# oceanusxiv/pathtracer-rs

Hardware: AMD Instinct MI355X
Metric: Mray/s, Cornell Box 1024x1024, 256 spp, depth 15 (Msample/s in config) (higher is better)
Workload: dtype f32

## Files before the change

include/ptrs.h:

```cpp
#ifndef PTRS_H
#define PTRS_H

#include <stdint.h>

#ifdef __cplusplus
extern "C" {
#endif

#define PTRS_ABI_VERSION 4

enum {
    PTRS_OK = 0,
    PTRS_ERR_INVALID = -1,
    PTRS_ERR_UNSUPPORTED = -2,
    PTRS_ERR_DEVICE = -3,
    PTRS_ERR_IO = -4
};

enum { PTRS_TEX_CONSTANT = 0, PTRS_TEX_CHECKER = 1, PTRS_TEX_IMAGE = 2 };
enum { PTRS_WRAP_REPEAT = 0, PTRS_WRAP_BLACK = 1, PTRS_WRAP_CLAMP = 2 };

typedef struct PtrsTexture {
    int32_t kind;
    int32_t channels;
// ... 104 lines not shown
    uint32_t flags;
    int32_t sampler;
    int32_t n_sampled_dimensions;
} PtrsRenderParams;
enum { PTRS_SAMPLER_SOBOL = 0, PTRS_SAMPLER_STRATIFIED = 1 };

enum {
    PTRS_FLAG_COUNTERS = 1u,
    PTRS_FLAG_TIMING = 2u,
    PTRS_FLAG_FILM_ZERO = 4u
};

typedef struct PtrsFilmPixel {
    float rgb[3];
    float weight;
} PtrsFilmPixel;

typedef struct PtrsStats {
    uint64_t samples;
    uint64_t rays_extension;
    uint64_t rays_shadow;
    uint64_t rays_mis;
    uint64_t nodes_visited;
    uint64_t tris_tested;
    uint64_t passes;
    uint64_t kernel_launches;
    uint64_t trace_launches;
    double ms_total;
    double ms_trace;
    double ms_shade;
    double ms_film;
    uint64_t bvh_nodes;
    uint64_t bvh_max_depth;
    uint64_t device_bytes;
    double ms_extend;
    double ms_connect;
    double ms_shade_kernels;
    double ms_aux;
    uint64_t extend_launches, connect_launches, shade_launches, aux_launches, film_launches;
    uint64_t error_flags;
    uint64_t node_steps_x64, node_visits, tri_steps_x64;
    uint64_t debug[12];
    uint64_t queue_segments;
    uint64_t grid_wgs[4];
    uint64_t resident_wgs_per_cu[4];
    uint64_t lanes;
    uint64_t grid_pct;
    double ms_enqueue;
    double ms_tail;
    uint64_t tail_launches;
    uint64_t tail_round;
    uint64_t stack_lds;
    uint64_t lds_form_v4;
} PtrsStats;

enum {
    PTRS_ERRFLAG_SOBOL_DIM = 1u,
    PTRS_ERRFLAG_NULL_SKIPS = 2u
};

typedef struct PtrsScene PtrsScene;

int ptrs_set_option(const char *name, int64_t value);
int ptrs_get_option(const char *name, int64_t *value);
int ptrs_scene_set_option(PtrsScene *scene, const char *name, int64_t value);

int ptrs_abi_version(void);
const char *ptrs_build_id(void);
int ptrs_abi_sizeof(int which);
const char *ptrs_last_error(void);

int ptrs_scene_create(const PtrsSceneDesc *desc, int32_t device, PtrsScene **out);
void ptrs_scene_destroy(PtrsScene *scene);
int ptrs_scene_info(PtrsScene *scene, uint64_t *n_nodes, uint64_t *max_depth, uint64_t *n_tris);

int ptrs_render(PtrsScene *scene, const PtrsCamera *camera, const PtrsRenderParams *params,
                PtrsFilmPixel *film_inout, PtrsStats *stats);

typedef void (*PtrsProgressFn)(void *user, uint32_t passes_done, uint32_t passes_total, int32_t row_begin, int32_t row_end);
int ptrs_render_progressive(PtrsScene *scene, const PtrsCamera *camera, const PtrsRenderParams *params,
                            PtrsFilmPixel *film_inout, PtrsProgressFn fn, void *user, PtrsStats *stats);

int ptrs_plan_bands(int32_t height, uint32_t n, const float *row_cost, int32_t *bounds_out );
int ptrs_render_row_cost(PtrsScene *scene, const PtrsCamera *camera, const PtrsRenderParams *params, float *row_cost_out, PtrsStats *stats);
int ptrs_render_multi(PtrsScene *const *scenes, uint32_t n, const PtrsCamera *camera,
                      const PtrsRenderParams *params, const int32_t *band_bounds,
                      PtrsFilmPixel *film_inout, PtrsStats *stats_per_scene);

int ptrs_render_device(PtrsScene *scene, const PtrsCamera *camera, const PtrsRenderParams *params,
                       void *film_inout_device, void *hip_stream, PtrsStats *stats);

int ptrs_render_samples(PtrsScene *scene, const PtrsCamera *camera, const PtrsRenderParams *params,
                        PtrsFilmPixel *film_inout, float *sample_rgb, PtrsStats *stats);

enum { PTRS_AOV_ALBEDO = 1u, PTRS_AOV_NORMAL = 2u, PTRS_AOV_DEPTH = 4u };
#define PTRS_AOV_PLANES 3
#define PTRS_AOV_SAMPLE_FLOATS 12
int ptrs_render_aov(PtrsScene *scene, const PtrsCamera *camera, const PtrsRenderParams *params, uint32_t planes,
                    PtrsFilmPixel *const planes_inout[PTRS_AOV_PLANES], float *sample_aov, PtrsStats *stats);
int ptrs_render_aov_device(PtrsScene *scene, const PtrsCamera *camera, const PtrsRenderParams *params, uint32_t planes,
                           void *const planes_inout_device[PTRS_AOV_PLANES], float *sample_aov_device, void *hip_stream, PtrsStats *stats);

#define PTRS_DENOISE_MAX_ITERATIONS 8
enum {
    PTRS_DENOISE_DEMODULATE = 1u,
    PTRS_DENOISE_TIMING = 2u
// ... 80 lines not shown
```

pathtracer-rs_amd/abi.py:

```python
import ctypes as C

import numpy as np

PTRS_OK = 0
TEX_CONSTANT, TEX_CHECKER, TEX_IMAGE = 0, 1, 2
WRAP_REPEAT, WRAP_BLACK, WRAP_CLAMP = 0, 1, 2
MAT_MATTE, MAT_METAL, MAT_MIRROR, MAT_GLASS, MAT_DISNEY, MAT_SUBSTRATE, MAT_NORMAL = range(7)
LIGHT_POINT, LIGHT_DIRECTIONAL, LIGHT_AREA, LIGHT_INFINITE = range(4)
FLAG_COUNTERS, FLAG_TIMING, FLAG_FILM_ZERO = 1, 2, 4
SAMPLER_SOBOL, SAMPLER_STRATIFIED = 0, 1
PtrsAovAlbedo, PtrsAovNormal, PtrsAovDepth = 1, 2, 4
PtrsAovPlanes, PtrsAovSampleFloats = 3, 12
PtrsAovNames = ("albedo", "normal", "depth")
(MATH_SIN, MATH_COS, MATH_SINCOS, MATH_TAN, MATH_LOG, MATH_LOG2, MATH_EXP, MATH_POW, MATH_ATAN2, MATH_ACOS, MATH_DIV, MATH_SQRT,
 MATH_ROUND, MATH_MINMAX, MATH_MINMAX_NZ, MATH_U2F, MATH_INT, MATH_NEXT, MATH_SOLVE, MATH_FRAME, MATH_SPAWN, MATH_SEARCH, MATH_NUM_OPS) = range(23)
PROBE_MATH_WIDTH = 16
PROBE_MATH_ARGTYPES = [C.c_int32, C.c_uint32, C.c_uint32, C.c_void_p, C.c_void_p]

f32p = C.POINTER(C.c_float)
u32p = C.POINTER(C.c_uint32)
i32p = C.POINTER(C.c_int32)


class PtrsTexture(C.Structure):
# ... 5 lines not shown
class PtrsMaterial(C.Structure):
    _fields_ = [("kind", C.c_int32), ("tex", C.c_int32 * 6), ("flags", C.c_int32), ("inner", C.c_int32)]


class PtrsMesh(C.Structure):
    _fields_ = [("n_verts", C.c_uint32), ("n_tris", C.c_uint32), ("pos", f32p), ("normal", f32p), ("tangent", f32p),
                ("uv", f32p), ("indices", u32p), ("material", C.c_int32), ("alpha_mask_tex", C.c_int32),
                ("reverse_orientation", C.c_int32), ("transform_swaps_handedness", C.c_int32)]


class PtrsLight(C.Structure):
    _fields_ = [("kind", C.c_int32), ("v", C.c_float * 3), ("c", C.c_float * 3), ("mesh", C.c_uint32), ("tri", C.c_uint32),
                ("ke_tex", C.c_int32), ("world_center", C.c_float * 3), ("world_radius", C.c_float), ("lmap_tex", C.c_int32),
                ("light_to_world", C.c_float * 16), ("world_to_light", C.c_float * 16), ("dist_nu", C.c_int32),
                ("dist_nv", C.c_int32), ("dist_func", f32p), ("dist_cdf", f32p), ("dist_func_int", f32p),
                ("marg_cdf", f32p), ("marg_func_int", C.c_float)]


class PtrsBvhNode(C.Structure):
    _fields_ = [("p_min", C.c_float * 3), ("p_max", C.c_float * 3), ("offset", C.c_uint32), ("num_prims", C.c_uint16),
                ("axis", C.c_uint8), ("pad", C.c_uint8)]


class PtrsSceneDesc(C.Structure):
    _fields_ = [("n_meshes", C.c_uint32), ("meshes", C.POINTER(PtrsMesh)), ("n_materials", C.c_uint32),
                ("materials", C.POINTER(PtrsMaterial)), ("n_textures", C.c_uint32), ("textures", C.POINTER(PtrsTexture)),
                ("n_lights", C.c_uint32), ("lights", C.POINTER(PtrsLight)), ("n_bvh_nodes", C.c_uint32),
                ("bvh_nodes", C.POINTER(PtrsBvhNode)), ("bvh_prims", u32p)]


class PtrsCamera(C.Structure):
    _fields_ = [("rot", C.c_float * 4), ("trans", C.c_float * 3), ("m00", C.c_float), ("m11", C.c_float), ("m22", C.c_float),
                ("m23", C.c_float), ("raster_to_screen", C.c_float * 16), ("dx_camera", C.c_float * 3), ("dy_camera", C.c_float * 3)]


class PtrsRenderParams(C.Structure):
    _fields_ = [("width", C.c_int32), ("height", C.c_int32), ("spp", C.c_int32), ("max_depth", C.c_int32),
                ("rr_threshold", C.c_float), ("rr_start_depth", C.c_int32), ("rr_enable", C.c_int32), ("row_begin", C.c_int32),
                ("row_end", C.c_int32), ("device", C.c_int32), ("paths_per_pass", C.c_uint32), ("flags", C.c_uint32), ("sampler", C.c_int32),
                ("n_sampled_dimensions", C.c_int32)]


class PtrsStats(C.Structure):
    _fields_ = [("samples", C.c_uint64), ("rays_extension", C.c_uint64), ("rays_shadow", C.c_uint64), ("rays_mis", C.c_uint64),
                ("nodes_visited", C.c_uint64), ("tris_tested", C.c_uint64), ("passes", C.c_uint64), ("kernel_launches", C.c_uint64),
                ("trace_launches", C.c_uint64), ("ms_total", C.c_double), ("ms_trace", C.c_double), ("ms_shade", C.c_double),
                ("ms_film", C.c_double), ("bvh_nodes", C.c_uint64), ("bvh_max_depth", C.c_uint64), ("device_bytes", C.c_uint64),
                ("ms_extend", C.c_double), ("ms_connect", C.c_double), ("ms_shade_kernels", C.c_double), ("ms_aux", C.c_double),
                ("extend_launches", C.c_uint64), ("connect_launches", C.c_uint64), ("shade_launches", C.c_uint64), ("aux_launches", C.c_uint64),
                ("film_launches", C.c_uint64), ("error_flags", C.c_uint64), ("node_steps_x64", C.c_uint64), ("node_visits", C.c_uint64),
                ("tri_steps_x64", C.c_uint64), ("debug", C.c_uint64 * 12), ("queue_segments", C.c_uint64), ("grid_wgs", C.c_uint64 * 4),
                ("resident_wgs_per_cu", C.c_uint64 * 4), ("lanes", C.c_uint64), ("grid_pct", C.c_uint64), ("ms_enqueue", C.c_double),
                ("ms_tail", C.c_double), ("tail_launches", C.c_uint64), ("tail_round", C.c_uint64),
                ("stack_lds", C.c_uint64), ("lds_form_v4", C.c_uint64)]

    def as_dict(self):
        return {n: getattr(self, n) for n, _ in self._fields_}

    @property
    def rays(self):
        return self.rays_extension + self.rays_shadow + self.rays_mis


class PtrsHit(C.Structure):
    _fields_ = [("prim", C.c_int32), ("t", C.c_float), ("b0", C.c_float), ("b1", C.c_float), ("b2", C.c_float)]


class PtrsDenoiseParams(C.Structure):
    _fields_ = [("iterations", C.c_int32), ("sigma_color", C.c_float), ("sigma_normal", C.c_float), ("sigma_depth", C.c_float), ("flags", C.c_uint32)]


PtrsDenoiseDemodulate, PtrsDenoiseTiming, PtrsDenoiseMaxIterations = 1, 2, 8


class PtrsTileError(C.Structure):
    _fields_ = [("error", C.c_float), ("valid", C.c_uint32)]


class PtrsFilmErrorSummary(C.Structure):
    _fields_ = [("max_tile_error", C.c_float), ("worst_tile", C.c_uint32), ("valid_pixels", C.c_uint64), ("tiles_x", C.c_uint32), ("tiles_y", C.c_uint32)]


PtrsErrorTile, PtrsConvergeMaxChecks = 16, 32


class PtrsConvergeCheck(C.Structure):
    _fields_ = [("spp", C.c_uint32), ("max_tile_error", C.c_float)]


class PtrsConvergeResult(C.Structure):
    _fields_ = [("spp_done", C.c_uint32), ("converged", C.c_uint32), ("n_checks", C.c_uint32), ("worst_tile", C.c_uint32), ("history", PtrsConvergeCheck * PtrsConvergeMaxChecks)]


HIT_DTYPE = np.dtype([("prim", "<i4"), ("t", "<f4"), ("b0", "<f4"), ("b1", "<f4"), ("b2", "<f4")])
FILM_DTYPE = np.dtype([("rgb", "<f4", 3), ("weight", "<f4")])
TILE_DTYPE = np.dtype([("error", "<f4"), ("valid", "<u4")])


def _f32(a):
    return np.ascontiguousarray(a, dtype=np.float32)


def _ptr(a, typ):
    return a.ctypes.data_as(typ) if a is not None else typ()


class SceneDescHolder:
# ... 82 lines not shown
```

pathtracer-rs_amd/csrc/pt_hip_queue.h:

```cpp
#pragma once

constexpr int BLOCK = 256, WAVES = BLOCK / 64;

__device__ inline uint32_t rfl(uint32_t v) { return (uint32_t)__builtin_amdgcn_readfirstlane((int)v); }
__device__ inline uint32_t lanes_below(unsigned long long m) { return __builtin_amdgcn_mbcnt_hi((uint32_t)(m >> 32), __builtin_amdgcn_mbcnt_lo((uint32_t)m, 0u)); }
__device__ inline uint32_t wave_push(uint32_t &count, bool pred) {
    const unsigned long long m = __ballot(pred);
    const uint32_t slot = count + lanes_below(m);
    count += (uint32_t)__popcll(m);
    return slot;
}
__device__ inline uint32_t wave_of_launch() { return blockIdx.x * WAVES + (threadIdx.x >> 6); }
enum : uint32_t { TK_SUB = 64, TK_SUB_STRIDE = 32, TK_LAUNCH_WORDS = TK_SUB * TK_SUB_STRIDE };
__device__ inline uint32_t seg_next(uint32_t *ticket, uint32_t G) {
    const uint32_t per = (G + TK_SUB - 1u) / TK_SUB;
    const uint32_t home = wave_of_launch() & (TK_SUB - 1u);
    for (;;) {
        uint32_t tmp; unsigned long long open;
        asm volatile("v_mbcnt_lo_u32_b32 %0, -1, 0\n\tv_mbcnt_hi_u32_b32 %0, -1, %0\n\tv_lshlrev_b32 %0, 7, %0\n\tglobal_load_dword %0, %0, %2 sc1\n\ts_waitcnt vmcnt(0)\n\tv_cmp_gt_u32 %1, %3, %0"
                     : "=&v"(tmp), "=s"(open) : "s"(ticket), "s"(per) : "memory");
        static_assert(TK_SUB_STRIDE * 4u == 128u, "the asm above shifts the lane id by 7");
        if (open == 0ull) return 0xffffffffu;
        const unsigned long long rot = home ? ((open >> home) | (open << (64u - home))) : open;
        const uint32_t c = (home + (uint32_t)__ffsll((long long)rot) - 1u) & (TK_SUB - 1u);
        uint32_t t = 0;
        if (__lane_id() == 0) t = atomicAdd(ticket + c * TK_SUB_STRIDE, 1u);
        t = rfl(t);
        const uint32_t s = c * per + t;
        if (t < per && s < G) return s;
    }
}
__device__ inline uint32_t *seg_count(const DQueues &Q, uint32_t row, int q, uint32_t G, uint32_t s) { return Q.counts + ((size_t)row * Q_STRIDE + (size_t)q) * G + s; }
enum { TK_EXTEND = 0, TK_CONNECT = 1, TK_SHADE0 = 2, TK_EPILOGUE = 9, TK_RESOLVE = 10, TK_PRESAMPLE = 11, TK_TAIL = 12 };
__device__ inline bool round_is_dead(const DQueues &Q, uint32_t it) { return it > 0u && rfl(Q.alive[it]) == 0u; }
```

pathtracer-rs_amd/csrc/pt_items.h:

```cpp
#pragma once
#include "pt_bvh.h"
#include "pt_light.h"
#include "pt_sobol.h"
#include "pt_stratified.h"

namespace pt {

struct CamRay { f3 o, d, rx_d, ry_d; };

PT_HD CamRay camera_ray(const DCamera &C, f2 pf, float diff_scale) {
    const float *m = C.r2s;
    f3 s = mk3(m[0] * pf.x + m[1] * pf.y + m[2] * 0.0f + m[3], m[4] * pf.x + m[5] * pf.y + m[6] * 0.0f + m[7], m[8] * pf.x + m[9] * pf.y + m[10] * 0.0f + m[11]);
    float inv_denom = C.m23 / (s.z + C.m22);
    f3 pc = mk3(s.x * inv_denom / C.m00, s.y * inv_denom / C.m11, -inv_denom);
    CamRay r;
    r.o = quat_rotate(C.rot, splat3(0.0f)) + ld3(C.trans);
    f3 wd = quat_rotate(C.rot, pc);
    r.d = normalize(wd);
    f3 rxd = normalize(quat_rotate(C.rot, pc + ld3(C.dxc)));
    f3 ryd = normalize(quat_rotate(C.rot, pc + ld3(C.dyc)));
    r.rx_d = r.d + (rxd - r.d) * diff_scale;
    r.ry_d = r.d + (ryd - r.d) * diff_scale;
    return r;
}
// ... 47 lines not shown
template <int FEAT>
PT_HD int extension_epilogue(const DParams &R, const DScene &sc, const DPaths &P, uint32_t par, uint32_t pid, uint32_t e, const HitRec &h) {
    const v4 rdv = pslot(P.ray_d[par], e);
    const uint32_t stz = f2u(rdv.w);
    const int32_t prim = h.prim;
    const int32_t bounces = st_bounces(stz);
    if (bounces == 0 || (stz & ST_SPECULAR)) {
        if (prim >= 0) {
            if (h.flags & TRI_IS_LIGHT) {
                const TriRegs T = load_tri_regs(sc.shade + prim);
                f3 d = xyz(rdv);
                Surface s = tri_surface(T, prim, h.b0, h.b1, h.b2, -d);
                f3 le = surface_le<FEAT>(sc, T, s, -d);
                v4 Lv = pslot(P.L, pid);
                f3 L = xyz(Lv) + xyz(pslot(P.beta[par], e)) * le;
                pslot(P.L, pid) = mkv4(L, Lv.w);
            }
        } else if ((FEAT & FEAT_INFINITE) && sc.n_inf > 0) {
            f3 d = xyz(rdv);
            v4 Lv = pslot(P.L, pid);
            f3 L = xyz(Lv), beta = xyz(pslot(P.beta[par], e));
            for (uint32_t i = 0; i < sc.n_inf; ++i) L = L + beta * light_le<FEAT>(sc, sc.lights[sc.inf_lights[i]], d);
            pslot(P.L, pid) = mkv4(L, Lv.w);
        }
    }
    if (prim < 0 || bounces >= R.max_depth) return -1;
    return (int)((h.flags >> TRI_BUCKET_SHIFT) & 7u);
}

PT_HD uint32_t hit_pack(int32_t prim, uint32_t flags) {
    return prim < 0 ? 0xffffffffu : ((uint32_t)prim | (((flags >> TRI_BUCKET_SHIFT) & 7u) << 27) | ((flags & TRI_IS_LIGHT) ? 1u << 30 : 0u));
}
PT_HD int32_t hit_prim(uint32_t x) { return x == 0xffffffffu ? -1 : (int32_t)(x & REF_FIRST_MASK); }
PT_HD uint32_t hit_flags(uint32_t x) { return x == 0xffffffffu ? 0u : ((((x >> 27) & 7u) << TRI_BUCKET_SHIFT) | (((x >> 30) & 1u) ? (uint32_t)TRI_IS_LIGHT : 0u)); }

#if defined(PTRS_STAMPS) && defined(__HIPCC__)
#define PT_STAMP_PARAMS , unsigned long long *stamp_acc, unsigned long long &stamp_last
#if defined(__HIP_DEVICE_COMPILE__)
#define PT_STAMP(k, dep) { unsigned long long t_; const uint32_t d_ = (dep); asm volatile("s_memtime %0\n\ts_waitcnt lgkmcnt(0)" : "=s"(t_) : "v"(d_) : "memory"); stamp_acc[k] += t_ - stamp_last; stamp_last = t_; }
#else
#define PT_STAMP(k, dep)
#endif
#else
#define PT_STAMP_PARAMS
#if defined(PTRS_SCHED_BARRIERS) && defined(__HIP_DEVICE_COMPILE__)
#define PT_STAMP(k, dep) __builtin_amdgcn_sched_barrier(0);
#else
#define PT_STAMP(k, dep)
#endif
#endif

struct VertexDraws { float u_nee[5], u_tail[3]; uint32_t after_cont, after_rr; bool err_cont, err_rr; };
template <class CTX>
PT_HD void draw_vertex(const CTX &X, const DSampler &S, const u4 &stv, bool nee, VertexDraws &D) {
    const uint32_t field = stv.z & ST_DIM_MASK;
    for (int k = 0; k < 5; ++k) D.u_nee[k] = 0.0f;
    if (S.kind == PTRS_SAMPLER_STRATIFIED) {
        uint32_t d1 = field & 63u, d2 = (field >> 6) & 63u;
        const uint32_t nd = S.strat_dims, pixel = stv.x, sidx = stv.y;
        auto t1 = [&](uint32_t d) { return S.strat1[((size_t)pixel * nd + (d < nd ? d : nd - 1u)) * S.spp + sidx]; };
        auto t2 = [&](uint32_t d, int c) { return S.strat2[(((size_t)pixel * nd + (d < nd ? d : nd - 1u)) * S.spp + sidx) * 2u + (uint32_t)c]; };
        bool err = false;
        if (nee) {
            D.u_nee[0] = t2(d2, 0); D.u_nee[1] = t2(d2, 1); D.u_nee[2] = t2(d2 + 1u, 0); D.u_nee[3] = t2(d2 + 1u, 1); D.u_nee[4] = t1(d1);
            err = d2 + 1u >= nd || d1 >= nd;
            d2 += 2u; d1 += 1u;
        }
        D.u_tail[0] = t2(d2, 0); D.u_tail[1] = t2(d2, 1);
        err = err || d2 >= nd;
        d2 += 1u;
        D.u_tail[2] = t1(d1);
        D.after_cont = strat_pack(d1, d2); D.err_cont = err;
        D.after_rr = strat_pack(d1 + 1u, d2); D.err_rr = err || d1 >= nd;
        return;
    }
    const uint64_t index = (uint64_t)stv.x | ((uint64_t)stv.y << 32);
    const VertexDims V = vertex_dims(field, nee);
    const uint32_t dt[3] = {V.cont[0], V.cont[1], V.rr};
    if (nee) {
        const uint32_t dn[8] = {V.nee[0], V.nee[1], V.nee[2], V.nee[3], V.nee[4], dt[0], dt[1], dt[2]};
        float u8[8];
        X.template sobol<8>(S, index, dn, stv.w, u8);
        for (int k = 0; k < 5; ++k) D.u_nee[k] = u8[k];
        D.u_tail[0] = u8[5]; D.u_tail[1] = u8[6]; D.u_tail[2] = u8[7];
    } else X.template sobol<3>(S, index, dt, stv.w, D.u_tail);
    D.after_cont = V.after_cont; D.err_cont = V.after_cont > 1024u;
    D.after_rr = V.after_cont + 1u; D.err_rr = V.after_cont + 1u > 1024u;
}

struct ShadeCtx {
    static constexpr bool inf_fallback = true;
    PT_MEM TriRegs tri(const DScene &sc, int32_t prim, bool want_dp) const { return load_tri_regs(sc.shade + prim, want_dp); }
    PT_MEM void light(const DScene &sc, uint32_t li, DLight &out) const { out = sc.lights[li]; }
    PT_MEM const InfMarginal *inf_marginal(uint32_t) const { return nullptr; }
    PT_MEM bool presampled(uint32_t) const { return false; }
    template <int N> PT_MEM void sobol(const DSampler &S, uint64_t index, const uint32_t (&dim)[N], uint32_t scramble, float (&out)[N]) const { sobol_batch<N>(S, index, dim, scramble, out); }
    PT_MEM void before_stores() const {}
};

struct ShadeResult {
    bool next; bool nee; bool shadow; bool mis; bool err_dim;
    v4 ro, rd, beta;
    v4 sh_o, sh_d, mis_o, mis_d, nee0, nee1; u4 nee2; float pre_z;
    PT_MEM uint32_t nee_entry(uint32_t pid) const { return pid | (shadow ? (uint32_t)NEE_Q_SHADOW : 0u) | (mis ? (uint32_t)NEE_Q_MIS : (uint32_t)NEE_Q_PRE); }
};
PT_HD void store_shade_out(const DPaths &P, uint32_t par_next, const ShadeResult &r, uint32_t e_next, uint32_t f) {
    if (r.shadow) { pstore(P.sh_o, f, r.sh_o); pstore(P.sh_d, f, r.sh_d); }
    if (r.mis) { pstore(P.mis_o, f, r.mis_o); pstore(P.mis_d, f, r.mis_d); pstore(P.nee0, f, r.nee0); pstore(P.nee1, f, r.nee1); pstore(P.nee2, f, r.nee2); }
    else if (r.nee) pstore(P.pre_z, f, r.pre_z);
    if (r.next) { pstore(P.ray_o[par_next], e_next, r.ro); pstore(P.ray_d[par_next], e_next, r.rd); pstore(P.beta[par_next], e_next, r.beta); }
}

struct PathIn { v4 ro, rd, beta; u4 st, hit; v4 pre0, pre1; };
PT_HD PathIn load_path_in(const DPaths &P, uint32_t par, uint32_t pid, uint32_t e) { PathIn p; p.ro = pslot(P.ray_o[par], e); p.rd = pslot(P.ray_d[par], e); p.beta = pslot(P.beta[par], e); p.st = pslot(P.st, pid); p.hit = pslot(P.hit, e); p.pre0 = p.pre1 = mkv4(splat3(0.0f), 0.0f); return p; }

template <int MAT, int FEAT, class CTX = ShadeCtx>
PT_HD ShadeResult shade_item(const DParams &R, const DSampler &S, const DCamera &C, const DScene &sc, const DPaths &P, uint32_t pid, const PathIn &in, const CTX &X PT_STAMP_PARAMS) {
    ShadeResult out; out.next = false; out.nee = false; out.shadow = false; out.mis = false; out.err_dim = false; out.pre_z = 0.0f;
    const v4 rov = in.ro, rdv = in.rd;
    v4 bv = in.beta;
    u4 stv = in.st; stv.z = f2u(rdv.w);
    const u4 h = in.hit;
    const f3 ro = xyz(rov), rd = xyz(rdv);
    f3 beta = xyz(bv);
    float eta_scale = bv.w;
    const int32_t prim = hit_prim(h.x);
    int32_t bounces = st_bounces(stv.z);
    const uint32_t dim0 = stv.z & ST_DIM_MASK;
    PT_STAMP(0, h.x + stv.z + f2u(rov.x) + f2u(rdv.x) + f2u(bv.x))
    constexpr bool NEE_KIND = MAT != PTRS_MAT_MIRROR && MAT != PTRS_MAT_GLASS;
    const bool nee_guess = NEE_KIND && sc.n_lights > 0;
    const TriRegs T = X.tri(sc, prim, (FEAT & FEAT_IMAGE) != 0);
    VertexDraws D;
    draw_vertex(X, S, stv, nee_guess, D);
    float (&u_nee)[5] = D.u_nee; float (&u_tail)[3] = D.u_tail;
    PT_STAMP(1, f2u(T.ng.x) + f2u(T.p0.x) + f2u(T.n0.x) + f2u(T.uv0.x) + f2u(u_tail[2]) + f2u(u_nee[4]) + T.flags)
    uint32_t li = 0;
    if (nee_guess) {
        const float fl = floor_(u_nee[4] * (float)sc.n_lights);
        li = fl > 0.0f ? (uint32_t)fl : 0u;
        if (li > sc.n_lights - 1u) li = sc.n_lights - 1u;
    }
    PT_STAMP(2, li)
    const f3 wo = -rd;
    Surface s = tri_surface(T, prim, u2f(h.y), u2f(h.z), u2f(h.w), wo);
    if ((FEAT & FEAT_IMAGE) && (stv.z & ST_HAS_DIFF)) {
        const f2a pf = pslot(P.pfilm, pid);
        CamRay cr = camera_ray(C, mk2(pf.x, pf.y), R.inv_sqrt_spp);
        surface_differentials(s, ro, cr.rx_d, ro, cr.ry_d);
    }
    v4 &w_sh_o = out.sh_o, &w_sh_d = out.sh_d, &w_mis_o = out.mis_o, &w_mis_d = out.mis_d, &w_nee0 = out.nee0, &w_nee1 = out.nee1, &w_ro = out.ro, &w_rd = out.rd, &w_beta = out.beta; u4 &w_nee2 = out.nee2; uint32_t w_stz = stv.z; float &w_cz = out.pre_z;
    bool w_skip = false;
    w_sh_o = w_sh_d = w_mis_o = w_mis_d = w_nee0 = w_nee1 = w_ro = w_rd = w_beta = mkv4(splat3(0.0f), 0.0f); w_nee2.x = w_nee2.y = w_nee2.z = w_nee2.w = 0;
    BsdfT<MatLobes<MAT>::N> bsdf;
    if (!make_bsdf<MAT, FEAT>(sc, T.material, s, bsdf)) {
        f3 o2 = spawn_origin(s.p, s.p_error, s.n, rd);
        w_ro = mkv4(o2, PT_INF);
        w_stz = st_pack(dim0, stv.z & ST_SPECULAR, bounces - 1);
        w_skip = true;
    } else {
    PT_STAMP(3, f2u(bsdf.ss.x) + f2u(bsdf.ts.y) + f2u(s.p.x) + f2u(s.p_error.x))
    const SpawnPair sp = spawn_pair(s.p, s.p_error, s.n);
    const uint32_t NS = BSDF_ALL & ~BSDF_SPECULAR;
#if defined(PTRS_ABL_SHADE_HALF) && PTRS_ABL_SHADE_HALF == 2
    const bool do_nee = false;
#else
    const bool do_nee = bsdf_num(bsdf, NS) > 0 && sc.n_lights > 0;
#endif
    if (do_nee != nee_guess) draw_vertex(X, S, stv, false, D);
    if (do_nee) {
        DLight Lt;
        X.light(sc, li, Lt);
        const f2 u_light = mk2(u_nee[0], u_nee[1]), u_scat = mk2(u_nee[2], u_nee[3]);
        const bool delta = light_is_delta(Lt);
        LightSample ls;
        if ((FEAT & FEAT_INFINITE) && X.presampled(li)) {
            ls.p1_err = splat3(0.0f); ls.p1_n = splat3(0.0f);
            ls.wi = xyz(in.pre0); ls.pdf = in.pre0.w; ls.li = xyz(in.pre1);
            ls.p1 = f2u(in.pre1.w) ? s.p + ls.wi * (2.0f * Lt.world_radius) : s.p;
        } else light_sample_li<FEAT, CTX::inf_fallback>(sc, Lt, s.p, sp, u_light, ls, X.inf_marginal(li));
        PT_STAMP(4, f2u(ls.pdf) + f2u(ls.wi.x) + f2u(ls.li.x) + f2u(ls.p1.x))
        f3 A = splat3(0.0f);
        float spdf = 0.0f;
        f3 wi = ls.wi;
        if (ls.pdf > 0.0f && !is_black(ls.li)) {
            f3 f = bsdf_f(bsdf, wo, wi, NS) * fabs_(dot(wi, s.ns));
            spdf = bsdf_pdf(bsdf, wo, wi, NS);
            if (!is_black(f)) {
                f3 origin = spawn_from(sp, ls.p1 - s.p);
                f3 target = offset_ray_origin(ls.p1, ls.p1_err, ls.p1_n, origin - ls.p1);
                w_sh_o = mkv4(origin, PT_SHADOW_TMAX);
                w_sh_d = mkv4(target - origin, 0.0f);
                A = delta ? f * ls.li / ls.pdf : f * ls.li * power_heuristic(ls.pdf, spdf) / ls.pdf;
                out.shadow = true;
            }
        }
        PT_STAMP(5, f2u(A.x) + f2u(spdf) + (out.shadow ? 1u : 0u))
        f3 fB = splat3(0.0f); float wB = 1.0f;
        if (!delta) {
            uint32_t sampled = BSDF_ALL;
            fB = bsdf_sample_f(bsdf, wo, wi, u_scat, spdf, NS, sampled);
            fB = fB * fabs_(dot(wi, s.ns));
            if (!is_black(fB) && spdf > 0.0f) {
                bool ok = true;
                if (!(sampled & BSDF_SPECULAR)) {
                    float lpdf = light_pdf_li<FEAT>(sc, Lt, s.p, sp, wi);
                    if (lpdf == 0.0f) ok = false;
                    else wB = power_heuristic(spdf, lpdf);
                }
                if (ok) {
                    w_mis_o = mkv4(spawn_from(sp, wi), PT_INF);
                    w_mis_d = mkv4(wi, 0.0f);
                    out.mis = true;
                }
            }
        }
        PT_STAMP(6, f2u(fB.x) + f2u(wB) + (out.mis ? 1u : 0u))
        if (out.shadow || out.mis) {
            out.nee = true;
            w_nee0 = mkv4(A, wB);
            w_nee1 = mkv4(fB, spdf);
            w_nee2.x = f2u(beta.x); w_nee2.y = f2u(beta.y); w_nee2.z = f2u(beta.z);
            w_nee2.w = li | ((out.shadow ? NEE_SHADOW : 0u) | (out.mis ? NEE_MIS : 0u)) << 24;
            if (!out.mis) {
                f3 ld = splat3(0.0f);
                ld = ld + A;
                const f3 c = beta * ((float)sc.n_lights * ld);
                w_sh_d.w = c.x; w_sh_o.w = c.y; w_cz = c.z;
            }
        }
    }

    uint32_t dim = D.after_cont;
    f3 wi = splat3(0.0f);
    float pdf = 0.0f; uint32_t flags = 0;
#if defined(PTRS_ABL_SHADE_HALF) && PTRS_ABL_SHADE_HALF == 1
    f3 f = splat3(0.0f);
#else
    f3 f = bsdf_sample_f(bsdf, wo, wi, mk2(u_tail[0], u_tail[1]), pdf, BSDF_ALL, flags);
#endif
    bool alive = true;
    if (D.err_cont) { out.err_dim = true; alive = false; }
    if (is_black(f) || pdf == 0.0f) alive = false;
    if (alive) {
        beta = beta * (f * fabs_(dot(wi, s.ns)) / pdf);
        const bool spec = (flags & BSDF_SPECULAR) != 0;
        if (spec && (flags & BSDF_TRANSMISSION)) {
            float eta = bsdf.eta;
            eta_scale *= dot(wo, s.n) > 0.0f ? eta * eta : 1.0f / (eta * eta);
        }
        f3 o2 = spawn_from(sp, wi);
        if (R.rr_enable) {
            float mx = max_comp(beta * eta_scale);
            if (mx < R.rr_threshold && bounces > R.rr_start_depth) {
                float q = max_nz(0.05f, 1.0f - mx);
                dim = D.after_rr;
                if (D.err_rr) { out.err_dim = true; alive = false; }
                else if (u_tail[2] < q) alive = false;
                else beta = beta / (1.0f - q);
            }
        }
        if (alive) {
            PT_STAMP(7, f2u(beta.x) + f2u(o2.x) + f2u(wi.x))
            bounces += 1;
            w_ro = mkv4(o2, PT_INF);
            w_stz = st_pack(dim, spec ? ST_SPECULAR : 0u, bounces);
            w_rd = mkv4(wi, u2f(w_stz));
            w_beta = mkv4(beta, eta_scale);
            out.next = true;
        }
    }
    if (out.err_dim) { out.nee = false; out.shadow = false; out.mis = false; out.next = false; }
    }
    if (w_skip) { w_rd = mkv4(rd, u2f(w_stz)); w_beta = bv; out.next = true; }
    return out;
}

template <int FEAT>
PT_HD void resolve_item(const DScene &sc, const DPaths &P, uint32_t entry, uint32_t f, bool occluded, const HitRec &mh) {
    const uint32_t pid = entry & NEE_Q_PID;
    if (entry & NEE_Q_PRE) {
        if (!occluded) { const f3 c = mk3(pslot(P.sh_d, f).w, pslot(P.sh_o, f).w, pslot(P.pre_z, f)); const v4 Lv = pslot(P.L, pid); pslot(P.L, pid) = mkv4(xyz(Lv) + c, Lv.w); }
        return;
    }
    const u4 n2 = pslot(P.nee2, f);
    const uint32_t li = n2.w & 0xffffffu, fl = n2.w >> 24;
    const v4 n0 = pslot(P.nee0, f), n1 = pslot(P.nee1, f);
    f3 ld = splat3(0.0f);
    if ((fl & NEE_SHADOW) && !occluded) ld = ld + xyz(n0);
    if (fl & NEE_MIS) {
        const DLight &Lt = sc.lights[li];
        const f3 wi = xyz(pslot(P.mis_d, f));
        f3 l2 = splat3(0.0f);
        if (mh.prim >= 0) {
            const TriRegs T = load_tri_regs(sc.shade + mh.prim);
            if (T.light == (int32_t)li) {
                Surface s = tri_surface(T, mh.prim, mh.b0, mh.b1, mh.b2, -wi);
                l2 = surface_le<FEAT>(sc, T, s, -wi);
            }
        } else l2 = light_le<FEAT>(sc, Lt, wi);
        if (!is_black(l2)) ld = ld + xyz(n1) * l2 * splat3(1.0f) * n0.w / n1.w;
    }
    const f3 beta = mk3(u2f(n2.x), u2f(n2.y), u2f(n2.z));
    const v4 Lv = pslot(P.L, pid);
    const f3 L = xyz(Lv) + beta * ((float)sc.n_lights * ld);
    pslot(P.L, pid) = mkv4(L, Lv.w);
}

template <int FEAT, bool QUAD, class Stack, class Geom>
PT_HD void connect_item(const DScene &sc, const Geom &G, const DPaths &P, uint32_t entry, uint32_t f, Stack &stack, uint32_t &n_nodes, uint32_t &n_tris) {
    const uint32_t fl = ((entry & NEE_Q_SHADOW) ? (uint32_t)NEE_SHADOW : 0u) | ((entry & NEE_Q_MIS) ? (uint32_t)NEE_MIS : 0u) | ((entry & NEE_Q_PRE) ? (uint32_t)NEE_PRE : 0u);
    bool occluded = false;
    HitRec mh; mh.prim = -1; mh.t = 0.0f; mh.b0 = mh.b1 = mh.b2 = 0.0f; mh.flags = 0;
    if (fl & NEE_SHADOW) {
        const v4 o = pslot(P.sh_o, f), d = pslot(P.sh_d, f);
        HitRec h;
        occluded = bvh_trace_g<QUAD, true, (FEAT & FEAT_ALPHA) != 0>(G, sc, xyz(o), xyz(d), PT_SHADOW_TMAX, stack, h, n_nodes, n_tris);
    }
    if (fl & NEE_MIS) {
        const v4 o = pslot(P.mis_o, f);
        if (!bvh_trace_g<QUAD, false, (FEAT & FEAT_ALPHA) != 0>(G, sc, xyz(o), xyz(pslot(P.mis_d, f)), PT_INF, stack, mh, n_nodes, n_tris)) mh.prim = -1;
    }
    resolve_item<FEAT>(sc, P, entry, f, occluded, mh);
}

template <int FEAT>
// ... 55 lines not shown
```

pathtracer-rs_amd/csrc/pt_light.h:

```cpp
#pragma once
#include "pt_material.h"

namespace pt {

struct LightSample {
    f3 li;
    f3 wi;
    float pdf;
    f3 p1, p1_err, p1_n;
};

PT_HD void tri_sample(const TriRegs &T, f2 u, f3 &p, f3 &n, f3 &perr, f2 &uv, const float *n_fixed = nullptr) {
    float su0 = sqrt_(u.x);
    float b0 = 1.0f - su0, b1 = u.y * su0;
    f3 p0 = T.p0, p1 = T.p1, p2 = T.p2;
    float b2 = 1.0f - b0 - b1;
    p = (b0 * p0) + (b1 * p1) + b2 * p2;
    if (n_fixed) n = ld3(n_fixed);
    else {
        n = normalize(cross(p1 - p0, p2 - p0));
        if (T.flags & TRI_HAS_NORMAL) {
            f3 ns = (b0 * T.n0) + (b1 * T.n1) + b2 * T.n2;
            n = face_forward(n, ns);
        } else if (((T.flags & TRI_REVERSE) != 0) != ((T.flags & TRI_SWAPS) != 0)) n = n * -1.0f;
    }
    perr = gamma_err(6) * (abs3(b0 * p0) + abs3(b1 * p1) + abs3(b2 * p2));
    uv = mk2(b0 * T.uv0.x + b1 * T.uv1.x + b2 * T.uv2.x, b0 * T.uv0.y + b1 * T.uv1.y + b2 * T.uv2.y);
}

PT_HD void tri_point_normal(const TriRegs &T, float b0, float b1, float b2, f3 &p, f3 &n) {
    f3 p0 = T.p0, p1 = T.p1, p2 = T.p2;
    p = b0 * p0 + b1 * p1 + b2 * p2;
    n = T.ng;
    if (T.flags & (TRI_HAS_NORMAL | TRI_HAS_TANGENT)) {
        f3 ns;
        if (T.flags & TRI_HAS_NORMAL) {
            ns = b0 * T.n0 + b1 * T.n1 + b2 * T.n2;
            ns = len2(ns) > 0.0f ? normalize(ns) : n;
        } else ns = n;
        f3 ss;
        if (T.flags & TRI_HAS_TANGENT) {
            ss = b0 * T.s0 + b1 * T.s1 + b2 * T.s2;
            ss = len2(ss) > 0.0f ? normalize(ss) : T.ssn;
        } else ss = T.ssn;
        f3 ts = cross(ss, ns);
        if (len2(ts) > 0.0f) { ts = normalize(ts); ss = cross(ts, ns); }
        else coordinate_system(ns, ss, ts);
        if (T.flags & TRI_REVERSE) ts = -ts;
        n = face_forward(n, normalize(cross(ss, ts)));
    }
}

template <int FEAT>
PT_HD float tri_pdf_at_point(const DScene &sc, const TriRegs &T, float area, f3 ref_p, const SpawnPair &ref_sp, f3 wi, const float *n_fixed = nullptr) {
    f3 o = spawn_from(ref_sp, wi);
    TriHit h;
    if (!tri_test(o, wi, PT_INF, T.p0, T.p1, T.p2, h)) return 0.0f;
    if (T.flags & TRI_DEGENERATE) return 0.0f;
    if ((FEAT & FEAT_ALPHA) && (T.flags & TRI_HAS_ALPHA)) {
        const f2 uv = mk2(h.b0 * T.uv0.x + h.b1 * T.uv1.x + h.b2 * T.uv2.x, h.b0 * T.uv0.y + h.b1 * T.uv1.y + h.b2 * T.uv2.y);
        if (tex_eval<FEAT>(sc, T.alpha_tex, uv, 0.0f, 0.0f, 0.0f, 0.0f).x == 0.0f) return 0.0f;
    }
    f3 p, n;
    if (n_fixed) { p = h.b0 * T.p0 + h.b1 * T.p1 + h.b2 * T.p2; n = ld3(n_fixed); }
    else tri_point_normal(T, h.b0, h.b1, h.b2, p, n);
    return len2(ref_p - p) / (fabs_(dot(n, -wi)) * area);
}

PT_HD f3 env_lookup(const DScene &sc, const DLight &L, f2 st) { return tex_lookup_width(sc, sc.texs[L.lmap_tex], st, 0.0f); }
PT_HD float spherical_theta(f3 v) { return pt_acosf(clamp_(v.z, -1.0f, 1.0f)); }
PT_HD float spherical_phi(f3 v) { float p = pt_atan2f(v.y, v.x); return p < 0.0f ? p + 2.0f * PT_PI : p; }

PT_HD float dist1d_sample(const float *func, const float *cdf, float func_int, uint32_t n, float u, float &pdf, uint32_t &off, const float *guide = nullptr, uint32_t g = 0) {
    off = g ? find_interval_cdf_guided(cdf, n + 1, u, guide, g) : find_interval_cdf(cdf, n + 1, u);
    float du = u - cdf[off];
    if ((cdf[off + 1] - cdf[off]) > 0.0f) du /= cdf[off + 1] - cdf[off];
    pdf = func_int > 0.0f ? func[off] / func_int : 0.0f;
    return ((float)off + du) / (float)n;
}

struct InfMarginal { const float *func, *cdf, *guide; };

PT_HD bool inf_light_sample(const DScene &sc, const DLight &L, f2 u, f3 &wi, float &pdf, f3 &li, const InfMarginal *im = nullptr) {
    const float *D = sc.distdata;
    float pdf_v, pdf_u; uint32_t v, dummy;
    const float *mf = im ? im->func : D + L.fint_off, *mc = im ? im->cdf : D + L.mcdf_off, *mg = im ? im->guide : D + L.mguide_off;
    float d1 = dist1d_sample(mf, mc, L.marg_int, (uint32_t)L.nv, u.y, pdf_v, v, mg, L.guide_v);
    float d0 = dist1d_sample(D + L.func_off + (uint64_t)v * (uint32_t)L.nu, D + L.cdf_off + (uint64_t)v * ((uint32_t)L.nu + 1u), mf[v], (uint32_t)L.nu, u.x, pdf_u, dummy,
                             D + L.cguide_off + (uint64_t)v * (L.guide_u + 1u), L.guide_u);
    float map_pdf = pdf_u * pdf_v;
    f3 li_ = splat3(0.0f), wi_ = splat3(0.0f); float pdf_ = 0.0f;
    const bool ok = map_pdf != 0.0f;
    if (ok) {
        float theta = d1 * PT_PI, phi = d0 * 2.0f * PT_PI;
        float ct, st, sp, cp; pt_sincosf(theta, &st, &ct); pt_sincosf(phi, &sp, &cp);
        wi_ = xform_vec(L.l2w, mk3(st * cp, st * sp, ct));
        pdf_ = st == 0.0f ? 0.0f : map_pdf / (2.0f * PT_PI * PT_PI * st);
        li_ = env_lookup(sc, L, mk2(d0, d1));
    }
    li = li_; pdf = pdf_; wi = wi_;
    return ok;
}

template <int FEAT, bool INF = true>
PT_HD bool light_sample_li(const DScene &sc, const DLight &L, f3 ref_p, const SpawnPair &ref_sp, f2 u, LightSample &o, const InfMarginal *im = nullptr) {
    f3 li = splat3(0.0f), wi = splat3(0.0f), p1 = ref_p, p1_err = splat3(0.0f), p1_n = splat3(0.0f);
    float pdf = 0.0f;
    bool ok = true;
    if (L.kind == 0) {
        f3 pl = ld3(L.v);
        wi = normalize(pl - ref_p); pdf = 1.0f; p1 = pl;
        li = ld3(L.c) / len2(pl - ref_p);
    } else if (L.kind == 1) {
        f3 w = ld3(L.v);
        wi = w; pdf = 1.0f; p1 = ref_p + w * (2.0f * L.world_radius);
        li = ld3(L.c);
    } else if (L.kind == 2) {
        const TriRegs T = load_tri_regs(&L.T);
        f3 p, n, perr; f2 uv;
        tri_sample(T, u, p, n, perr, uv, L.n_ok ? L.n_sample : nullptr);
        wi = normalize(p - ref_p);
        pdf = tri_pdf_at_point<FEAT>(sc, T, L.area, ref_p, ref_sp, wi, L.n_ok ? L.n_point : nullptr);
        p1 = p; p1_err = perr; p1_n = n;
        f3 w = -wi;
        li = dot(n, w) > 0.0f ? (L.ke_const ? ld3(L.c) : tex_eval<FEAT>(sc, L.ke_tex, uv, 0.0f, 0.0f, 0.0f, 0.0f)) : splat3(0.0f);
    } else if (!(FEAT & FEAT_INFINITE) || !INF) { ok = false;
    } else {
        ok = inf_light_sample(sc, L, u, wi, pdf, li, im);
        p1 = ok ? ref_p + wi * (2.0f * L.world_radius) : ref_p;
    }
    o.li = li; o.wi = wi; o.pdf = pdf; o.p1 = p1; o.p1_err = p1_err; o.p1_n = p1_n;
    return ok;
}

template <int FEAT>
PT_HD float light_pdf_li(const DScene &sc, const DLight &L, f3 ref_p, const SpawnPair &ref_sp, f3 w) {
    if (L.kind == 2) return tri_pdf_at_point<FEAT>(sc, load_tri_regs(&L.T), L.area, ref_p, ref_sp, w, L.n_ok ? L.n_point : nullptr);
    if ((FEAT & FEAT_INFINITE) && L.kind == 3) {
        f3 wi = xform_vec(L.w2l, w);
        float theta = spherical_theta(wi), phi = spherical_phi(wi);
        float st = pt_sinf(theta);
        if (st == 0.0f) return 0.0f;
        float pu = phi * PT_INV_2PI, pv = theta * PT_INV_PI;
        uint32_t nu = (uint32_t)L.nu, nv = (uint32_t)L.nv;
        float fu = pu * (float)nu, fv = pv * (float)nv;
        uint32_t iu = (fu > 0.0f) ? (fu >= 4294967040.0f ? 0xffffffffu : (uint32_t)fu) : 0u;
        uint32_t iv = (fv > 0.0f) ? (fv >= 4294967040.0f ? 0xffffffffu : (uint32_t)fv) : 0u;
        if (iu > nu - 1u) iu = nu - 1u;
        if (iv > nv - 1u) iv = nv - 1u;
        const float *D = sc.distdata;
        return (D[L.func_off + (uint64_t)iv * nu + iu] / L.marg_int) / (2.0f * PT_PI * PT_PI * st);
    }
    return 0.0f;
}

template <int FEAT>
PT_HD f3 light_le(const DScene &sc, const DLight &L, f3 d) {
    if (!(FEAT & FEAT_INFINITE) || L.kind != 3) return splat3(0.0f);
    f3 w = normalize(xform_vec(L.w2l, d));
    return env_lookup(sc, L, mk2(spherical_phi(w) * PT_INV_2PI, spherical_theta(w) * PT_INV_PI));
}

template <int FEAT>
PT_HD f3 surface_le(const DScene &sc, const TriRegs &T, const Surface &s, f3 w) {
    if (T.light < 0) return splat3(0.0f);
    if (dot(s.n, w) > 0.0f) {
        const DLight &L = sc.lights[T.light];
        return L.ke_const ? ld3(L.c) : tex_eval<FEAT>(sc, L.ke_tex, s);
    }
    return splat3(0.0f);
}

PT_HD bool light_is_delta(const DLight &L) { return L.kind == 0 || L.kind == 1; }

}
```

pathtracer-rs_amd/csrc/pt_probe.h:

```cpp
#pragma once
#include "pt_light.h"
#include "pt_bvh.h"
#include "pt_host_scene.h"

namespace pt {

enum : uint32_t { PROBE_BSDF_IN = 8, PROBE_BSDF_OUT = 16, PROBE_LIGHT_IN = 5, PROBE_LIGHT_OUT = 16, PROBE_TEX_IN = 6, PROBE_TEX_OUT = 8,
                  PROBE_SURF_IN = 16, PROBE_SURF_OUT = 64, PROBE_MATH_IN = 16, PROBE_MATH_OUT = 16 };

PT_HD Surface probe_surface(const float *frame , f3 wo) {
    Surface s;
    s.p = splat3(0.0f); s.p_error = splat3(0.0f); s.wo = wo;
    s.n = mk3(frame[0], frame[1], frame[2]);
    s.ns = mk3(frame[3], frame[4], frame[5]);
    s.dpdu = mk3(frame[6], frame[7], frame[8]); s.dpdv = cross(s.ns, s.dpdu);
    s.s_dpdu = s.dpdu; s.s_dpdv = s.dpdv;
    s.uv = mk2(0.25f, 0.5f);
    s.dudx = s.dvdx = s.dudy = s.dvdy = 0.0f;
    s.prim = 0; s.ssn = s.dpdu; s.ssn_ok = false;
    return s;
}

template <int MAT>
PT_HD void bsdf_probe_mat(const DScene &sc, int32_t mat_id, const float *frame, const float *in, float *out) {
    const f3 wo = mk3(in[0], in[1], in[2]), wi = mk3(in[3], in[4], in[5]);
    const f2 u = mk2(in[6], in[7]);
    Surface s = probe_surface(frame, wo);
    BsdfT<MatLobes<MAT>::N> b;
    for (uint32_t k = 0; k < PROBE_BSDF_OUT; ++k) out[k] = 0.0f;
    if (!make_bsdf<MAT, 0>(sc, mat_id, s, b)) return;
    const f3 f = bsdf_f(b, wo, wi, BSDF_ALL);
    const float pdf = bsdf_pdf(b, wo, wi, BSDF_ALL);
    f3 swi = splat3(0.0f); float spdf = 0.0f; uint32_t sampled = 0;
    const f3 sf = bsdf_sample_f(b, wo, swi, u, spdf, BSDF_ALL, sampled);
    out[0] = f.x; out[1] = f.y; out[2] = f.z; out[3] = pdf;
    out[4] = sf.x; out[5] = sf.y; out[6] = sf.z; out[7] = spdf;
    out[8] = swi.x; out[9] = swi.y; out[10] = swi.z; out[11] = (float)sampled;
    out[12] = 1.0f;
}

PT_HD void bsdf_probe_row(const DScene &sc, int32_t mat_id, int32_t kind, const float *frame, const float *in, float *out) {
    switch (kind) {
        case 0: bsdf_probe_mat<0>(sc, mat_id, frame, in, out); break;
        case 1: bsdf_probe_mat<1>(sc, mat_id, frame, in, out); break;
        case 2: bsdf_probe_mat<2>(sc, mat_id, frame, in, out); break;
        case 3: bsdf_probe_mat<3>(sc, mat_id, frame, in, out); break;
        case 4: bsdf_probe_mat<4>(sc, mat_id, frame, in, out); break;
        default: bsdf_probe_mat<5>(sc, mat_id, frame, in, out); break;
    }
}

PT_HD void light_probe_row(const DScene &sc, int32_t light, const float *ref , const float *in, float *out) {
    const DLight &L = sc.lights[light];
    const f3 p = mk3(ref[0], ref[1], ref[2]), n = mk3(ref[3], ref[4], ref[5]);
    const SpawnPair sp = spawn_pair(p, splat3(0.0f), n);
    const f3 wq = mk3(in[2], in[3], in[4]);
    LightSample ls;
    const bool ok = light_sample_li<FEAT_IMG_ENV>(sc, L, p, sp, mk2(in[0], in[1]), ls);
    const float pq = light_pdf_li<FEAT_IMG_ENV>(sc, L, p, sp, wq);
    const f3 le = light_le<FEAT_IMG_ENV>(sc, L, wq);
    for (uint32_t k = 0; k < PROBE_LIGHT_OUT; ++k) out[k] = 0.0f;
    out[0] = ls.wi.x; out[1] = ls.wi.y; out[2] = ls.wi.z; out[3] = ls.pdf;
    out[4] = ls.li.x; out[5] = ls.li.y; out[6] = ls.li.z; out[7] = ok ? 1.0f : 0.0f;
    out[8] = pq; out[9] = le.x; out[10] = le.y; out[11] = le.z;
}

PT_HD void texture_probe_row(const DScene &sc, int32_t tex, const float *in, float *out) {
    const DTexture &T = sc.texs[tex];
    const f3 v = tex_eval<FEAT_FULL>(sc, tex, mk2(in[0], in[1]), in[2], in[3], in[4], in[5]);
    for (uint32_t k = 0; k < PROBE_TEX_OUT; ++k) out[k] = 0.0f;
    out[0] = v.x; out[1] = v.y; out[2] = v.z;
    if (T.kind == 2) {
        const float width = max_nz(max_nz(fabs_(T.su * in[2]), fabs_(T.sv * in[3])), max_nz(fabs_(T.su * in[4]), fabs_(T.sv * in[5])));
        out[3] = (float)T.n_levels - 1.0f + pt_log2f(max_nz(width, 1e-8f));
        out[4] = (width <= 1e-8f && T.n_levels <= 27) ? 1.0f : 0.0f;
        out[5] = T.su * in[0] + T.du; out[6] = T.sv * in[1] + T.dv;
    }
}

PT_HD void surface_probe_row(const DScene &sc, uint32_t prim, const float *in, float *out) {
    for (uint32_t k = 0; k < PROBE_SURF_OUT; ++k) out[k] = 0.0f;
    const f3 o = mk3(in[0], in[1], in[2]), d = mk3(in[3], in[4], in[5]);
    const float t_max = in[6];
    const TriRegs T = load_tri_regs(sc.shade + prim);
    const RayShear S = ray_shear(d);
    TriHit h{0.0f, 0.0f, 0.0f, 0.0f}, hs{0.0f, 0.0f, 0.0f, 0.0f};
    const bool hit = tri_test_s(o, S, t_max, T.p0, T.p1, T.p2, h);
    const bool hit_sel = tri_test_s_sel(o, S, t_max, T.p0, T.p1, T.p2, hs);
    out[0] = hit ? 1.0f : 0.0f;
    if (hit) { out[1] = h.t; out[2] = h.b0; out[3] = h.b1; out[4] = h.b2; }
    out[5] = hit_sel ? 1.0f : 0.0f;
    if (hit_sel) { out[6] = hs.t; out[7] = hs.b0; out[8] = hs.b1; out[9] = hs.b2; }
    if (!hit) return;
    Surface s = tri_surface(T, (int32_t)prim, h.b0, h.b1, h.b2, -d);
    surface_differentials(s, o, mk3(in[7], in[8], in[9]), o, mk3(in[10], in[11], in[12]));
    const DMaterial *mp = sc.mats + T.material;
    int steps = 0;
    for (; steps < 4 && mp->kind == 6; ++steps) {
        normal_mapping<FEAT_FULL>(sc, mp->tex[0], s);
        mp = sc.mats + mp->inner;
    }
    const f3 v[8] = {s.p, s.p_error, s.n, s.ns, s.dpdu, s.dpdv, s.s_dpdu, s.s_dpdv};
    for (int k = 0; k < 8; ++k) { out[10 + 3 * k] = v[k].x; out[11 + 3 * k] = v[k].y; out[12 + 3 * k] = v[k].z; }
    out[34] = s.uv.x; out[35] = s.uv.y;
    out[36] = s.dudx; out[37] = s.dvdx; out[38] = s.dudy; out[39] = s.dvdy;
    const SpawnPair sp = spawn_pair(s.p, s.p_error, s.n);
    const f3 ow = offset_ray_origin(s.p, s.p_error, s.n, mk3(in[13], in[14], in[15]));
    const f3 w[3] = {sp.plus, sp.minus, ow};
    for (int k = 0; k < 3; ++k) { out[40 + 3 * k] = w[k].x; out[41 + 3 * k] = w[k].y; out[42 + 3 * k] = w[k].z; }
    out[49] = (float)steps;
}

enum : uint32_t {
    MATH_SIN = 0, MATH_COS, MATH_SINCOS, MATH_TAN, MATH_LOG, MATH_LOG2, MATH_EXP, MATH_POW, MATH_ATAN2, MATH_ACOS,
    MATH_DIV,
    MATH_SQRT,
    MATH_ROUND,
// ... 96 lines not shown
```

pathtracer-rs_amd/csrc/pt_render.h:

```cpp
#pragma once
#include <algorithm>
#include <chrono>
#include <cmath>
#include <vector>

#include "pt_host_scene.h"
#include "pt_items.h"

namespace pt {

struct SobolTablesHost {
    std::vector<uint32_t> matrices;
    std::vector<uint64_t> vdc, vdc_inv;
    uint32_t stride = 52;
    bool ok = false;
};

inline bool load_sobol_tables(const char *path, SobolTablesHost &T) {
    FILE *f = std::fopen(path, "rb");
    if (!f) return false;
    char magic[8]; uint32_t hdr[6]; uint32_t lens[52];
    bool ok = std::fread(magic, 1, 8, f) == 8 && std::memcmp(magic, "PTRSSOB1", 8) == 0 && std::fread(hdr, 4, 6, f) == 6 && hdr[0] == 1024 && hdr[1] == 52;
    if (ok) {
        T.stride = hdr[4];
// ... 217 lines not shown
    uint64_t capacity = std::min<uint64_t>(1ull << 27, prm.paths_per_pass ? prm.paths_per_pass : be.auto_capacity(n_lanes, kinds_present));
    if (capacity < (uint64_t)g.NX) capacity = (uint64_t)g.NX;
    if (job.single_pixel) capacity = std::max<uint64_t>(capacity, (uint64_t)g.NX * ns);
    PassPlan plan;
    if (!plan_passes(band_rows, (uint64_t)g.NX, ns, capacity, n_lanes, prm.paths_per_pass != 0, plan)) { err = "pass too large"; return PTRS_ERR_INVALID; }
    const uint64_t rows_per_pass = plan.rows_per_pass, samples_per_pass = plan.samples_per_pass, max_paths = plan.max_paths;

    const uint32_t fixed_iters = (uint32_t)prm.max_depth + 1u;
    const uint32_t max_iters = fixed_iters + 64u;
    const int feat = scene_features(sc_host_feat), feat_trace = scene_trace_features(sc_host_feat);
    rc = be.begin(sc, u.S, u.C, (uint32_t)max_paths, max_iters + 1u, bvh_depth, prm.flags, feat, feat_trace, err);
    if (rc != PTRS_OK) return rc;

    PtrsStats st;
    std::memset(&st, 0, sizeof(st));
    std::vector<uint32_t> counts((size_t)(max_iters + 1u) * Q_STRIDE);
    const uint32_t n_passes_total = (uint32_t)(((band_rows + rows_per_pass - 1) / rows_per_pass) * ((ns + samples_per_pass - 1) / samples_per_pass));
    struct Pending { bool active = false, open = false; uint32_t it = 0, n_paths = 0, pass_no = 0; int32_t y0 = 0, y1 = 0; };
    std::vector<Pending> pending(n_lanes);
    bool null_skip_overrun = false;
    auto round = [&](uint32_t i) {
        be.extend(i);
        be.presample(i);
        for (int k = 0; k < 6; ++k) if (kinds_present[k]) be.shade(i, k);
        be.connect(i);
    };
    const uint32_t spare_rounds = kinds_present[PTRS_MAT_GLASS] ? 6u : 0u;
    auto close_pass = [&](uint32_t lane) {
        Pending &pd = pending[lane];
        if (!pd.active || !pd.open) return;
        be.select(lane);
        uint32_t it = pd.it;
        if (spare_rounds) {
            while (it < max_iters && be.read_count(it, Q_EXT) != 0) { round(it); ++it; }
            if (it == max_iters && be.read_count(it, Q_EXT) != 0) null_skip_overrun = true;
        }
        pd.it = it;
        if (pd.y1 > pd.y0 && job.film) be.film(job.film, pd.y0, pd.y1);
        if (pd.y1 > pd.y0 && job.film_half) be.film(job.film_half, pd.y0, pd.y1);
        if (job.samples_out) be.export_samples(job.samples_out);
        pd.open = false;
    };
    auto finish = [&](uint32_t lane) {
        Pending &pd = pending[lane];
        if (!pd.active) return;
        close_pass(lane);
        be.select(lane);
        be.read_counts(counts.data(), pd.it + 1u);
        be.learn(counts.data(), std::min(pd.it + 1u, max_iters + 1u), pd.n_paths);
        for (uint32_t i = 0; i <= pd.it && i < max_iters + 1u; ++i) {
            st.rays_extension += counts[(size_t)i * Q_STRIDE + Q_EXT];
            st.rays_shadow += counts[(size_t)i * Q_STRIDE + Q_SHADOW];
            st.rays_mis += counts[(size_t)i * Q_STRIDE + Q_MIS];
        }
        st.samples += pd.n_paths;
        st.passes += 1;
        if (job.progress && job.progress->fn && pd.y1 > pd.y0) { be.publish_rows(job.film, pd.y0, pd.y1); job.progress->fn(job.progress->user, pd.pass_no + 1u, n_passes_total, pd.y0, pd.y1); }
        pd.active = false;
    };
    uint32_t pass_no = 0;
    for (int32_t r0 = srow0; r0 < srow1; r0 += (int32_t)rows_per_pass) {
        const int32_t r1 = std::min<int32_t>(srow1, r0 + (int32_t)rows_per_pass);
        for (uint32_t s0 = sb; s0 < se; s0 += (uint32_t)samples_per_pass, ++pass_no) {
            const uint32_t s1 = (uint32_t)std::min<uint64_t>(se, (uint64_t)s0 + samples_per_pass);
            const uint32_t lane = pass_no % n_lanes;
            finish(lane);
            be.select(lane);
            R.row0 = r0; R.row1 = r1; R.s0 = s0; R.s1 = s1;
            R.n_paths = (uint32_t)(r1 - r0) * (uint32_t)g.NX * (s1 - s0);
            if (job.single_pixel) { R.pixel_mode = 1; R.pix_sx = job.single_pixel[0] - g.min_x; R.pix_sy = job.single_pixel[1] - g.min_y; R.n_paths = s1 - s0; }
            be.pass_begin(R);
            be.generate();
            uint32_t it = 0;
            if (job.dump) {
                for (; it < job.dump->round && it < max_iters; ++it) round(it);
                be.dump_rays(it, *job.dump);
                be.end(st);
                if (job.stats) *job.stats = st;
                return PTRS_OK;
            }
            const uint32_t n_rounds = std::min(fixed_iters + spare_rounds, max_iters);
            const uint32_t tail_from = spare_rounds ? 0xffffffffu : be.tail_round(R.n_paths, n_rounds);
            for (; it < n_rounds && it < tail_from; ++it) round(it);
            if (it < n_rounds) { be.tail(it, n_rounds); it = n_rounds; }
            const int32_t y0 = std::max(rb, g.min_y + r0 - 2), y1 = std::min(re, g.min_y + r1 - 1 + 2 + 1);
            pending[lane].active = true; pending[lane].it = it; pending[lane].n_paths = R.n_paths; pending[lane].pass_no = pass_no;
            pending[lane].y0 = (job.single_pixel || y1 <= y0) ? 0 : y0; pending[lane].y1 = (job.single_pixel || y1 <= y0) ? 0 : y1;
            pending[lane].open = true;
            if (!spare_rounds) close_pass(lane);
        }
    }
    st.ms_enqueue = std::chrono::duration<double, std::milli>(clock::now() - t_begin).count();
    for (uint32_t k = 0; k < n_lanes; ++k) finish((pass_no + k) % n_lanes);
    be.end(st);
    if (null_skip_overrun) st.error_flags |= PTRS_ERRFLAG_NULL_SKIPS;
    st.bvh_nodes = sc.n_nodes; st.bvh_max_depth = bvh_depth;
    st.ms_total = std::chrono::duration<double, std::milli>(clock::now() - t_begin).count();
    if (job.stats) *job.stats = st;
    if (st.error_flags & PTRS_ERRFLAG_SOBOL_DIM) {
        err = u.strat_dim ? "stratified sampler: a path drew past n_sampled_dimensions (null-BSDF skips lengthen paths beyond max_depth, Q7); the reference would continue from the tile's generator in path order, which a wavefront cannot reproduce"
                        : "sobol sampler can only sample up to 1024 dimensions (sobol.rs:177-183): max_depth is too large for this scene";
        return PTRS_ERR_UNSUPPORTED;
    }
    if (st.error_flags & PTRS_ERRFLAG_NULL_SKIPS) { err = "paths still alive after max_depth + 65 rounds of null-BSDF skips (integrator.rs:434-439)"; return PTRS_ERR_UNSUPPORTED; }
    return PTRS_OK;
}
// ... 10 lines not shown
```

pathtracer-rs_amd/csrc/pt_scene.h:

```cpp
#pragma once
#include "pt_vec.h"

namespace pt {

struct alignas(16) DNode {
    float pmin[3];
    float pmax0;
    float pmax1, pmax2;
    uint32_t offset;
    uint32_t meta;
};

struct alignas(16) DNode2 {
    float c0min[3]; float c0max0;
    float c0max1, c0max2, c1min0, c1min1;
    float c1min2; float c1max[3];
    uint32_t ref0, ref1, axis, pad;
};
static_assert(sizeof(DNode2) == 64, "node2");

struct alignas(16) DNode4 {
    float box[24];
    uint32_t ref[4];
    uint32_t axes, pad[3];
// ... 97 lines not shown
struct DCamera {
    float rot[4], trans[3];
    float m00, m11, m22, m23;
    float r2s[16];
    float dxc[3], dyc[3];
};

struct DParams {
    int32_t max_depth;
    float rr_threshold;
    int32_t rr_start_depth, rr_enable;
    int32_t NX, NY;
    int32_t W, H;
    float inv_sqrt_spp;
    int32_t row0, row1;
    uint32_t s0, s1;
    uint32_t n_paths;
    uint32_t counters_on;
    int32_t pixel_mode, pix_sx, pix_sy;
    uint32_t *row_cost;
};

struct alignas(16) v4 { float x, y, z, w; };
struct alignas(16) u4 { uint32_t x, y, z, w; };
struct alignas(8) f2a { float x, y; };

enum : uint32_t { ST_DIM_MASK = 0xfffu, ST_SPECULAR = 1u << 12, ST_HAS_DIFF = 1u << 13, ST_BOUNCE_SHIFT = 16 };
enum : uint32_t { NEE_Q_PID = 0x07ffffffu, NEE_Q_SHADOW = 0x20000000u, NEE_Q_MIS = 0x40000000u, NEE_Q_PRE = 0x80000000u };
enum : uint32_t { NEE_SHADOW = 1u, NEE_MIS = 2u,
                  NEE_PRE = 4u,
                  NEE_OCCLUDED = 0x80u };

struct DPaths {
    v4 *ray_o[2];
    v4 *ray_d[2];
    v4 *beta[2];
    u4 *hit;
    v4 *pre0;
    v4 *pre1;
    v4 *L;
    u4 *st;
    f2a *pfilm;
    v4 *nee0;
    v4 *nee1;
    u4 *nee2;
    v4 *sh_o;
    v4 *sh_d;
    float *pre_z;
    v4 *mis_o;
    v4 *mis_d;
    u4 *nhit;
};

enum { Q_EXT = 0, Q_SHADOW = 1, Q_MIS = 2, Q_NEE = 3, Q_MAT0 = 4, Q_NUM_MAT = 7, Q_STRIDE = 16 };
enum { CNT_EXT = 0, CNT_SHADOW = 1, CNT_MIS = 2, CNT_NODES = 3, CNT_TRIS = 4,
       CNT_NODE_STEPS = 5, CNT_NODE_VISITS = 6, CNT_TRI_STEPS = 7,
       CNT_ERR = 8,
       CNT_STAMP0 = 16,
       CNT_NUM = 32 };

struct alignas(8) MatEntry { uint32_t e, pid; };
struct DQueues {
    uint32_t *ext[2];
    MatEntry *mat[Q_NUM_MAT];
    uint32_t *nee;
    uint32_t *counts;
    uint32_t *tickets;
    uint32_t *alive;
    unsigned long long *stats;
};

template <class T> PT_HD T &pslot(T *base, uint32_t i) {
#if defined(__HIP_DEVICE_COMPILE__)
    return *reinterpret_cast<T *>(reinterpret_cast<char *>(base) + (size_t)(i * (uint32_t)sizeof(T)));
#else
    return base[i];
#endif
}
template <class T> PT_HD const T &pslot(const T *base, uint32_t i) {
#if defined(__HIP_DEVICE_COMPILE__)
    return *reinterpret_cast<const T *>(reinterpret_cast<const char *>(base) + (size_t)(i * (uint32_t)sizeof(T)));
#else
    return base[i];
#endif
}

template <class T> PT_HD void pstore(T *base, uint32_t i, const T &v) { pslot(base, i) = v; }

PT_HD uint32_t f2u(float f) { return ptf_bits(f); }
PT_HD float u2f(uint32_t u) { return ptf_from_bits(u); }
PT_HD v4 mkv4(f3 a, float w) { v4 r; r.x = a.x; r.y = a.y; r.z = a.z; r.w = w; return r; }
PT_HD f3 xyz(v4 a) { return mk3(a.x, a.y, a.z); }
PT_HD f3 ld3(const float *p) { return mk3(p[0], p[1], p[2]); }

struct TriRegs {
    f3 p0, p1, p2, n0, n1, n2, s0, s1, s2;
    f3 ng, ssn, dpdu, dpdv;
    f2 uv0, uv1, uv2;
    int32_t material, light, alpha_tex; uint32_t flags;
};
PT_HD TriRegs load_tri_regs(const DTriShade *rec, bool want_dp = true) {
    const v4 *q = reinterpret_cast<const v4 *>(rec);
    TriRegs t;
    const v4 k = q[10], l = q[11];
    t.ng = mk3(k.x, k.y, k.z); t.ssn = mk3(k.w, l.x, l.y);
    if (want_dp) { const v4 m = q[12]; t.dpdu = mk3(l.z, l.w, m.x); t.dpdv = mk3(m.y, m.z, m.w); }
    else { t.dpdu = t.dpdv = mk3(0.0f, 0.0f, 0.0f); }
    const v4 a = q[0], b = q[1], c = q[2];
    t.p0 = mk3(a.x, a.y, a.z); t.p1 = mk3(a.w, b.x, b.y); t.p2 = mk3(b.z, b.w, c.x);
    t.material = (int32_t)f2u(c.y); t.light = (int32_t)f2u(c.z); t.flags = f2u(c.w);
    const v4 d = q[3], e = q[4], f = q[5], g = q[6];
    t.n0 = mk3(d.x, d.y, d.z); t.n1 = mk3(d.w, e.x, e.y); t.n2 = mk3(e.z, e.w, f.x);
    t.alpha_tex = (int32_t)f2u(f.y); t.uv0 = mk2(f.z, f.w); t.uv1 = mk2(g.x, g.y); t.uv2 = mk2(g.z, g.w);
    if (t.flags & TRI_HAS_TANGENT) {
        const v4 h = q[7], i = q[8], j = q[9];
        t.s0 = mk3(h.x, h.y, h.z); t.s1 = mk3(h.w, i.x, i.y); t.s2 = mk3(i.z, i.w, j.x);
    } else { t.s0 = t.s1 = t.s2 = mk3(0.0f, 0.0f, 0.0f); }
    return t;
}

}
// ... 1 lines not shown
```

pathtracer-rs_amd/csrc/pt_tri.h:

```cpp
#pragma once
#include "pt_scene.h"

namespace pt {

struct TriHit { float t, b0, b1, b2; };

struct RayShear { int kz; float sx, sy, sz; };
PT_HD RayShear ray_shear(f3 d) {
    RayShear S;
    S.kz = max_dimension(abs3(d));
    int kx = S.kz + 1; if (kx == 3) kx = 0;
    int ky = kx + 1; if (ky == 3) ky = 0;
    const float dx = comp(d, kx), dy = comp(d, ky), dz = comp(d, S.kz);
    S.sx = -dx / dz; S.sy = -dy / dz; S.sz = 1.0f / dz;
    return S;
}

PT_HD bool tri_test_perm(f3 p0t, f3 p1t, f3 p2t, float sx, float sy, float sz, float t_max, TriHit &h) {
    p0t.x += sx * p0t.z; p0t.y += sy * p0t.z;
    p1t.x += sx * p1t.z; p1t.y += sy * p1t.z;
    p2t.x += sx * p2t.z; p2t.y += sy * p2t.z;
    float e0 = p1t.x * p2t.y - p1t.y * p2t.x;
    float e1 = p2t.x * p0t.y - p2t.y * p0t.x;
    float e2 = p0t.x * p1t.y - p0t.y * p1t.x;
    if (e0 == 0.0f || e1 == 0.0f || e2 == 0.0f) {
        e0 = (float)((double)p2t.y * (double)p1t.x - (double)p2t.x * (double)p1t.y);
        e1 = (float)((double)p0t.y * (double)p2t.x - (double)p0t.x * (double)p2t.y);
        e2 = (float)((double)p1t.y * (double)p0t.x - (double)p1t.x * (double)p0t.y);
    }
    const float det = e0 + e1 + e2;
    if ((((e0 < 0.0f) | (e1 < 0.0f) | (e2 < 0.0f)) & ((e0 > 0.0f) | (e1 > 0.0f) | (e2 > 0.0f))) | (det == 0.0f)) return false;
    p0t.z *= sz; p1t.z *= sz; p2t.z *= sz;
    const float t_scaled = e0 * p0t.z + e1 * p1t.z + e2 * p2t.z;
    const float lim = t_max * det;
    if (((det < 0.0f) & ((t_scaled >= 0.0f) | (t_scaled < lim))) | ((det > 0.0f) & ((t_scaled <= 0.0f) | (t_scaled > lim)))) return false;
    float inv_det = 1.0f / det;
    float t = t_scaled * inv_det;
    float max_z = max_nz(max_nz(fabs_(p0t.z), fabs_(p1t.z)), fabs_(p2t.z));
    float delta_z = gamma_err(3) * max_z;
    float max_x = max_nz(max_nz(fabs_(p0t.x), fabs_(p1t.x)), fabs_(p2t.x));
    float max_y = max_nz(max_nz(fabs_(p0t.y), fabs_(p1t.y)), fabs_(p2t.y));
    float delta_x = gamma_err(5) * (max_x + max_z);
    float delta_y = gamma_err(5) * (max_y + max_z);
    float delta_e = 2.0f * (gamma_err(2) * max_x * max_y + delta_y * max_x + delta_x * max_y);
    float max_e = max_nz(max_nz(fabs_(e0), fabs_(e1)), fabs_(e2));
    float delta_t = 3.0f * (gamma_err(3) * max_e * max_z + delta_e * max_z + delta_z * max_e) * fabs_(inv_det);
    if (t <= delta_t) return false;
    h.t = t; h.b0 = e0 * inv_det; h.b1 = e1 * inv_det; h.b2 = e2 * inv_det;
    return true;
}
PT_HD bool tri_test_perm_sel(f3 p0t, f3 p1t, f3 p2t, float sx, float sy, float sz, float t_max, TriHit &h) {
    p0t.x += sx * p0t.z; p0t.y += sy * p0t.z;
    p1t.x += sx * p1t.z; p1t.y += sy * p1t.z;
    p2t.x += sx * p2t.z; p2t.y += sy * p2t.z;
    float e0 = p1t.x * p2t.y - p1t.y * p2t.x;
    float e1 = p2t.x * p0t.y - p2t.y * p0t.x;
    float e2 = p0t.x * p1t.y - p0t.y * p1t.x;
    if (e0 == 0.0f || e1 == 0.0f || e2 == 0.0f) {
        e0 = (float)((double)p2t.y * (double)p1t.x - (double)p2t.x * (double)p1t.y);
        e1 = (float)((double)p0t.y * (double)p2t.x - (double)p0t.x * (double)p2t.y);
        e2 = (float)((double)p1t.y * (double)p0t.x - (double)p1t.x * (double)p0t.y);
    }
    const float det = e0 + e1 + e2;
    const bool rej_sign = (((e0 < 0.0f) | (e1 < 0.0f) | (e2 < 0.0f)) & ((e0 > 0.0f) | (e1 > 0.0f) | (e2 > 0.0f))) | (det == 0.0f);
    p0t.z *= sz; p1t.z *= sz; p2t.z *= sz;
    const float t_scaled = e0 * p0t.z + e1 * p1t.z + e2 * p2t.z;
    const float lim = t_max * det;
    const bool rej_range = ((det < 0.0f) & ((t_scaled >= 0.0f) | (t_scaled < lim))) | ((det > 0.0f) & ((t_scaled <= 0.0f) | (t_scaled > lim)));
    float inv_det = 1.0f / det;
    float t = t_scaled * inv_det;
    float max_z = max_nz(max_nz(fabs_(p0t.z), fabs_(p1t.z)), fabs_(p2t.z));
    float delta_z = gamma_err(3) * max_z;
    float max_x = max_nz(max_nz(fabs_(p0t.x), fabs_(p1t.x)), fabs_(p2t.x));
    float max_y = max_nz(max_nz(fabs_(p0t.y), fabs_(p1t.y)), fabs_(p2t.y));
    float delta_x = gamma_err(5) * (max_x + max_z);
    float delta_y = gamma_err(5) * (max_y + max_z);
    float delta_e = 2.0f * (gamma_err(2) * max_x * max_y + delta_y * max_x + delta_x * max_y);
    float max_e = max_nz(max_nz(fabs_(e0), fabs_(e1)), fabs_(e2));
    float delta_t = 3.0f * (gamma_err(3) * max_e * max_z + delta_e * max_z + delta_z * max_e) * fabs_(inv_det);
    h.t = t; h.b0 = e0 * inv_det; h.b1 = e1 * inv_det; h.b2 = e2 * inv_det;
    return !(rej_sign | rej_range) & !(t <= delta_t);
}
PT_HD bool tri_test_s(f3 o, const RayShear &S, float t_max, f3 p0, f3 p1, f3 p2, TriHit &h) {
    f3 p0t = p0 - o, p1t = p1 - o, p2t = p2 - o;
    const int kz = S.kz;
    int kx = kz + 1; if (kx == 3) kx = 0;
    int ky = kx + 1; if (ky == 3) ky = 0;
    p0t = mk3(comp(p0t, kx), comp(p0t, ky), comp(p0t, kz));
    p1t = mk3(comp(p1t, kx), comp(p1t, ky), comp(p1t, kz));
    p2t = mk3(comp(p2t, kx), comp(p2t, ky), comp(p2t, kz));
    return tri_test_perm(p0t, p1t, p2t, S.sx, S.sy, S.sz, t_max, h);
}
PT_HD bool tri_test_s_sel(f3 o, const RayShear &S, float t_max, f3 p0, f3 p1, f3 p2, TriHit &h) {
    f3 p0t = p0 - o, p1t = p1 - o, p2t = p2 - o;
    const int kz = S.kz;
    int kx = kz + 1; if (kx == 3) kx = 0;
    int ky = kx + 1; if (ky == 3) ky = 0;
    p0t = mk3(comp(p0t, kx), comp(p0t, ky), comp(p0t, kz));
    p1t = mk3(comp(p1t, kx), comp(p1t, ky), comp(p1t, kz));
    p2t = mk3(comp(p2t, kx), comp(p2t, ky), comp(p2t, kz));
    return tri_test_perm_sel(p0t, p1t, p2t, S.sx, S.sy, S.sz, t_max, h);
}
PT_HD RayShear ray_shear_inv(f3 d, f3 inv) {
    RayShear S;
    S.kz = max_dimension(abs3(d));
    int kx = S.kz + 1; if (kx == 3) kx = 0;
    int ky = kx + 1; if (ky == 3) ky = 0;
    const float dx = comp(d, kx), dy = comp(d, ky), dz = comp(d, S.kz);
    S.sx = -dx / dz; S.sy = -dy / dz; S.sz = comp(inv, S.kz);
    return S;
}
PT_HD bool tri_test(f3 o, f3 d, float t_max, f3 p0, f3 p1, f3 p2, TriHit &h) { return tri_test_s(o, ray_shear(d), t_max, p0, p1, p2, h); }

PT_HD bool tri_dpduv(f3 p0, f3 p1, f3 p2, f2 uv0, f2 uv1, f2 uv2, f3 &dpdu, f3 &dpdv) {
    f2 duv02 = mk2(uv0.x - uv2.x, uv0.y - uv2.y), duv12 = mk2(uv1.x - uv2.x, uv1.y - uv2.y);
    f3 dp02 = p0 - p2, dp12 = p1 - p2;
    float determinant = duv02.x * duv12.y - duv02.y * duv12.x;
    bool degenerate_uv = fabs_(determinant) < 1e-8f;
    dpdu = splat3(0.0f); dpdv = splat3(0.0f);
    if (!degenerate_uv) {
        float invdet = 1.0f / determinant;
        dpdu = (duv12.y * dp02 - duv02.y * dp12) * invdet;
        dpdv = (-duv12.x * dp02 + duv02.x * dp12) * invdet;
    }
    if (degenerate_uv || len2(cross(dpdu, dpdv)) == 0.0f) {
        f3 ng = cross(p2 - p0, p1 - p0);
        if (len2(ng) == 0.0f) return false;
        coordinate_system(normalize(ng), dpdu, dpdv);
    }
    return true;
}

struct Surface {
    f3 p, p_error, wo;
    f3 n;
    f3 ns;
    f3 dpdu, dpdv;
    f3 s_dpdu, s_dpdv;
    f2 uv;
    float dudx, dvdx, dudy, dvdy;
    int32_t prim;
    f3 ssn;
    bool ssn_ok;
};

PT_HD Surface tri_surface(const TriRegs &T, int32_t prim, float b0, float b1, float b2, f3 wo) {
    Surface s;
    f3 p0 = T.p0, p1 = T.p1, p2 = T.p2;
    f2 uv0 = T.uv0, uv1 = T.uv1, uv2 = T.uv2;
    s.dpdu = T.dpdu; s.dpdv = T.dpdv;
    float xs = fabs_(b0 * p0.x) + fabs_(b1 * p1.x) + fabs_(b2 * p2.x);
    float ys = fabs_(b0 * p0.y) + fabs_(b1 * p1.y) + fabs_(b2 * p2.y);
    float zs = fabs_(b0 * p0.z) + fabs_(b1 * p1.z) + fabs_(b2 * p2.z);
    s.p_error = gamma_err(7) * mk3(xs, ys, zs);
    s.p = b0 * p0 + b1 * p1 + b2 * p2;
    s.uv = mk2(b0 * uv0.x + b1 * uv1.x + b2 * uv2.x, b0 * uv0.y + b1 * uv1.y + b2 * uv2.y);
    s.wo = wo;
    s.prim = prim;
    s.dudx = s.dvdx = s.dudy = s.dvdy = 0.0f;
    s.n = T.ng;
    s.ns = s.n;
    s.s_dpdu = s.dpdu; s.s_dpdv = s.dpdv;
    s.ssn = T.ssn; s.ssn_ok = true;
    if (T.flags & (TRI_HAS_NORMAL | TRI_HAS_TANGENT)) {
        f3 ns;
// ... 52 lines not shown
```

pathtracer-rs_amd/csrc/ptrs_hip.hip:

```cpp
#include <hip/hip_runtime.h>

#include <cstdio>
#include <cstdlib>
#include <cstring>
#include <map>
#include <memory>
#include <mutex>
#include <new>
#include <string>
#include <thread>
#include <vector>

#include "pt_render.h"
#include "pt_aov.h"
#include "pt_denoise.h"
#include "pt_converge.h"
#include "pt_probe.h"

using namespace pt;

static const unsigned char k_sobol_blob[] = {
#include "sobol_tables_data.inc"
};

namespace {

thread_local std::string g_err;

struct Options {
    int lanes = 0;
    int refill = -1;
    int refill_connect = -1;
    int stack_lds = 8;
    int grid_mult = 0;
    int grid_pct = 0;
    int whole_rounds = 0;
    int persist = 1;
    int node_form = 0;
    int node_order = 0;
    int vote = -1;
    int fused_epilogue = 1;
    int fused_resolve = 1;
    int shade_lds = 1;
    int env_presample = 1;
    int peer_copy = 1;
    int deal = 0;
    int tail = 1;
    int tail_at = -1;
    int tail_paths = 0;
    int workspace_pct = 40;
    int aov_fused_film = 1;
    int denoise_lds = -1;
};
Options g_opt;
std::mutex g_opt_mu;
Options options() { std::lock_guard<std::mutex> lk(g_opt_mu); return g_opt; }
struct OptionDesc { const char *name; int Options::*field; int lo, hi; };
const OptionDesc k_options[] = {
    {"lanes", &Options::lanes, 0, 8}, {"refill", &Options::refill, -1, 64}, {"refill_connect", &Options::refill_connect, -1, 64}, {"stack_lds", &Options::stack_lds, 8, 16},
    {"grid_mult", &Options::grid_mult, 0, 64}, {"persist", &Options::persist, 0, 1}, {"whole_rounds", &Options::whole_rounds, 0, 1}, {"grid_pct", &Options::grid_pct, 0, 100}, {"node_form", &Options::node_form, 0, 2}, {"node_order", &Options::node_order, 0, 1}, {"vote", &Options::vote, -1, 2}, {"shade_lds", &Options::shade_lds, 0, 1}, {"fused_epilogue", &Options::fused_epilogue, 0, 1}, {"fused_resolve", &Options::fused_resolve, 0, 1}, {"workspace_pct", &Options::workspace_pct, 1, 90}, {"peer_copy", &Options::peer_copy, 0, 1}, {"env_presample", &Options::env_presample, 0, 1}, {"deal", &Options::deal, 0, 1}, {"tail", &Options::tail, 0, 1}, {"tail_at", &Options::tail_at, -1, 64}, {"tail_paths", &Options::tail_paths, 0, 1 << 20}, {"aov_fused_film", &Options::aov_fused_film, 0, 1}, {"denoise_lds", &Options::denoise_lds, -1, 1},
};

#define HIPCHK(expr)                                                                                             \
    do {                                                                                                          \
        hipError_t e_ = (expr);                                                                                   \
        if (e_ != hipSuccess) {                                                                                   \
            g_err = std::string(#expr) + ": " + hipGetErrorString(e_);                                            \
            return PTRS_ERR_DEVICE;                                                                               \
        }                                                                                                         \
    } while (0)

#include "pt_hip_queue.h"

typedef __attribute__((address_space(3))) const v4 lds_v4;
__device__ inline v4 lds_ld(lds_v4 *q) { v4 r; r.x = q->x; r.y = q->y; r.z = q->z; r.w = q->w; return r; }
enum : uint32_t { TOP_LDS_STRIDE = 9 };
struct GeomTop {
    lds_v4 *top; const v4 *nodesv; const DTri *tris; uint32_t ktop;
    __device__ inline void node8(uint32_t i, v4 *o) const {
        if (i < ktop) { lds_v4 *q = top + TOP_LDS_STRIDE * i; for (int k = 0; k < 8; ++k) o[k] = lds_ld(q + k); }
        else { const v4 *q = nodesv + 8u * i; for (int k = 0; k < 8; ++k) o[k] = q[k]; }
    }
    __device__ inline void quad_load(uint32_t i, uint32_t px, uint32_t py, uint32_t pz, v4 &xn, v4 &xf, v4 &yn, v4 &yf, v4 &zn, v4 &zf, v4 &refs, v4 &meta) const {
        if (i < ktop) {
            typedef __attribute__((address_space(3))) const char lds_c;
            lds_c *b = (lds_c *)top + i * (TOP_LDS_STRIDE * 16u);
            xn = lds_ld((lds_v4 *)(b + px)); xf = lds_ld((lds_v4 *)(b + (px ^ 16u)));
            yn = lds_ld((lds_v4 *)(b + py)); yf = lds_ld((lds_v4 *)(b + (py ^ 16u)));
            zn = lds_ld((lds_v4 *)(b + pz)); zf = lds_ld((lds_v4 *)(b + (pz ^ 16u)));
            refs = lds_ld((lds_v4 *)(b + 96u)); meta = lds_ld((lds_v4 *)(b + 112u));
        } else {
            const char *b = reinterpret_cast<const char *>(nodesv);
            const uint32_t off = i * 128u;
            xn = *reinterpret_cast<const v4 *>(b + (size_t)(off + px)); xf = *reinterpret_cast<const v4 *>(b + (size_t)((off + px) ^ 16u));
            yn = *reinterpret_cast<const v4 *>(b + (size_t)(off + py)); yf = *reinterpret_cast<const v4 *>(b + (size_t)((off + py) ^ 16u));
            zn = *reinterpret_cast<const v4 *>(b + (size_t)(off + pz)); zf = *reinterpret_cast<const v4 *>(b + (size_t)((off + pz) ^ 16u));
            refs = *reinterpret_cast<const v4 *>(b + (size_t)(off + 96u)); meta = *reinterpret_cast<const v4 *>(b + (size_t)(off + 112u));
        }
    }
    __device__ inline void node(uint32_t, v4 &, v4 &, v4 &, v4 &) const {}
    __device__ inline void tri(uint32_t k, v4 &a, v4 &b, v4 &c) const { const v4 *q = reinterpret_cast<const v4 *>(tris + k); a = q[0]; b = q[1]; c = q[2]; }
};

struct StackSpill { unsigned long long *p; uint32_t stride; };
template <int D, bool OVF>
struct LdsStack {
    unsigned long long *col, *ovf; uint32_t ovf_stride;
    int n;
    __device__ inline void init(unsigned long long *lds, const StackSpill &sp) { col = lds + threadIdx.x; ovf = OVF ? sp.p + (size_t)blockIdx.x * BLOCK + threadIdx.x : nullptr; ovf_stride = sp.stride; n = 0; }
    __device__ inline void push(uint32_t v, float t) {
        const unsigned long long e = (unsigned long long)v | ((unsigned long long)f2u(t) << 32);
        if (!OVF || n < D) col[n * BLOCK] = e; else ovf[(size_t)(n - D) * ovf_stride] = e;
        ++n;
// ... 490 lines not shown
template <int FEAT>
__device__ inline void epilogue_wave(const DParams &R, const DScene &sc, const DPaths &P, const DQueues &Q, uint32_t it, uint32_t kinds_mask, uint32_t seg_cap, uint32_t G, uint32_t s) {
    const uint32_t lane = __lane_id();
    const uint32_t e0 = s * seg_cap, par = it & 1u;
    const uint32_t n = rfl(*seg_count(Q, it, Q_EXT, G, s));
    uint32_t cnt[6] = {0u, 0u, 0u, 0u, 0u, 0u};
    for (uint32_t i0 = 0; i0 < n; i0 += 64u) {
        const uint32_t i = i0 + lane, e = e0 + i;
        int k = -1; uint32_t pid = 0;
        if (i < n) {
            pid = pslot(Q.ext[par], e);
            if (R.row_cost) atomicAdd(R.row_cost + sample_row_of(R, pid), 1u);
            const u4 r = pslot(P.hit, e);
            HitRec h; h.prim = hit_prim(r.x); h.t = 0.0f; h.b0 = u2f(r.y); h.b1 = u2f(r.z); h.b2 = u2f(r.w);
            h.flags = hit_flags(r.x);
            k = extension_epilogue<FEAT>(R, sc, P, par, pid, e, h);
        }
#pragma unroll
        for (int m = 0; m < 6; ++m) {
            if (!(kinds_mask & (1u << m))) continue;
            const uint32_t slot = wave_push(cnt[m], k == m);
            if (k == m) { MatEntry me; me.e = e; me.pid = pid; pslot(Q.mat[m], e0 + slot) = me; }
        }
    }
    if (lane == 0) {
#pragma unroll
        for (int m = 0; m < 6; ++m) if (kinds_mask & (1u << m)) *seg_count(Q, it, Q_MAT0 + m, G, s) = cnt[m];
    }
}

template <int FEAT>
__global__ __launch_bounds__(BLOCK) void k_epilogue(DParams R, DScene sc, DPaths P, DQueues Q, uint32_t it, uint32_t kinds_mask, uint32_t seg_cap, uint32_t Gn, uint32_t *ticket) {
    if (round_is_dead(Q, it)) return;
    for (uint32_t s = seg_next(ticket, Gn); s < Gn; s = seg_next(ticket, Gn)) epilogue_wave<FEAT>(R, sc, P, Q, it, kinds_mask, seg_cap, Gn, s);
}


#ifndef PTRS_SHADE_WAVES_MATTE
#define PTRS_SHADE_WAVES_MATTE 2
#endif
#ifndef PTRS_SHADE_WAVES_DISNEY_IMG
#define PTRS_SHADE_WAVES_DISNEY_IMG 2
#endif
template <int MAT, int FEAT> struct ShadeWaves { enum { N = (MAT == 0 && FEAT == FEAT_SIMPLE) ? PTRS_SHADE_WAVES_MATTE : ((MAT == 4 && FEAT == FEAT_IMG) ? PTRS_SHADE_WAVES_DISNEY_IMG : 2) }; };

#ifndef PTRS_SH_SOB_WORDS
#define PTRS_SH_SOB_WORDS 3200
#endif
#ifndef PTRS_SH_TRI_V4
#define PTRS_SH_TRI_V4 512
#endif
enum : uint32_t { SH_SOB_WORDS = PTRS_SH_SOB_WORDS, SH_TRI_V4 = PTRS_SH_TRI_V4, SH_LIGHTS = 16, SH_LIGHT_V4 = sizeof(DLight) / 16, SH_TRI_REC_V4 = sizeof(DTriShade) / 16 };
static_assert(sizeof(DLight) % 16 == 0 && sizeof(DTriShade) % 16 == 0, "records are staged as 16-byte vectors");
struct ShadeLdsCfg { uint32_t sob_lo, sob_n, sob_nib, tri_lds, n_lights_lds, marg_li, pre_li; };
enum : uint32_t { SH_MARG_N = 1024, SH_MARG_WORDS = 3 * SH_MARG_N + 8 };
typedef __attribute__((address_space(3))) const uint32_t lds_u32;
PT_HD uint32_t sob_stride(uint32_t nib) { return nib * 16u + 4u; }
template <bool ENVPRE = false>
struct ShadeCtxLds {
    static constexpr bool inf_fallback = !ENVPRE;
    lds_u32 *sob; lds_v4 *tris, *lights; ShadeLdsCfg cfg; InfMarginal marg;
    __device__ inline const InfMarginal *inf_marginal(uint32_t li) const { return li == cfg.marg_li ? &marg : nullptr; }
    __device__ inline bool presampled(uint32_t li) const { return li == cfg.pre_li; }
    __device__ inline v4 ld(lds_v4 *q) const { v4 r; r.x = q->x; r.y = q->y; r.z = q->z; r.w = q->w; return r; }
    __device__ inline TriRegs tri(const DScene &sc, int32_t prim, bool want_dp) const {
        if (!cfg.tri_lds) return load_tri_regs(sc.shade + prim, want_dp);
        v4 r[SH_TRI_REC_V4];
        lds_v4 *q = tris + (uint32_t)prim * SH_TRI_REC_V4;
#pragma unroll
        for (uint32_t k = 0; k < SH_TRI_REC_V4; ++k) r[k] = ld(q + k);
        return load_tri_regs(reinterpret_cast<const DTriShade *>(r), want_dp);
    }
    __device__ inline void before_stores() const { __builtin_amdgcn_s_waitcnt(0x0F70); }
    __device__ inline void light(const DScene &sc, uint32_t li, DLight &out) const {
        if (li >= cfg.n_lights_lds) { out = sc.lights[li]; return; }
        v4 *o = reinterpret_cast<v4 *>(&out);
        lds_v4 *q = lights + li * SH_LIGHT_V4;
#pragma unroll
        for (uint32_t k = 0; k < SH_LIGHT_V4; ++k) o[k] = ld(q + k);
    }
    template <int N> __device__ inline void sobol(const DSampler &S, uint64_t index, const uint32_t (&dim)[N], uint32_t scramble, float (&out)[N]) const {
        const uint32_t lo = (uint32_t)index, hi = (uint32_t)(index >> 32);
        bool in = cfg.sob_nib >= 13u || (hi == 0u && cfg.sob_nib >= 8u);
#pragma unroll
        for (int k = 0; k < N; ++k) in = in && dim[k] - cfg.sob_lo < cfg.sob_n;
        if (!in) { sobol_batch<N>(S, index, dim, scramble, out); return; }
        uint32_t v[N];
        bool run = cfg.sob_nib == 8u;
#pragma unroll
        for (int k = 1; k < N; ++k) run = run && dim[k] == dim[0] + (uint32_t)k;
        if (run) {
            constexpr uint32_t ST = 8u * 16u + 4u;
            lds_u32 *t = sob + (dim[0] - cfg.sob_lo) * ST;
            lds_u32 *t0 = t + (lo & 15u), *t1 = t + 16u + ((lo >> 4) & 15u), *t2 = t + 32u + ((lo >> 8) & 15u), *t3 = t + 48u + ((lo >> 12) & 15u), *t4 = t + 64u + ((lo >> 16) & 15u),
                    *t5 = t + 80u + ((lo >> 20) & 15u), *t6 = t + 96u + ((lo >> 24) & 15u), *t7 = t + 112u + (lo >> 28);
#pragma unroll
            for (int k = 0; k < N; ++k) v[k] = scramble ^ t0[k * ST] ^ t1[k * ST] ^ t2[k * ST] ^ t3[k * ST] ^ t4[k * ST] ^ t5[k * ST] ^ t6[k * ST] ^ t7[k * ST];
#pragma unroll
            for (int k = 0; k < N; ++k) out[k] = min_nz(PT_ONE_MINUS_EPS, (float)v[k] * 0x1p-32f);
            return;
        }
        const uint32_t stride = sob_stride(cfg.sob_nib);
#pragma unroll
        for (int k = 0; k < N; ++k) {
            lds_u32 *t = sob + (dim[k] - cfg.sob_lo) * stride;
            v[k] = scramble ^ t[lo & 15u] ^ t[16u + ((lo >> 4) & 15u)] ^ t[32u + ((lo >> 8) & 15u)] ^ t[48u + ((lo >> 12) & 15u)] ^ t[64u + ((lo >> 16) & 15u)] ^ t[80u + ((lo >> 20) & 15u)] ^
                   t[96u + ((lo >> 24) & 15u)] ^ t[112u + (lo >> 28)];
        }
        if (cfg.sob_nib > 8u) {
#pragma unroll
            for (int k = 0; k < N; ++k) {
                lds_u32 *t = sob + (dim[k] - cfg.sob_lo) * stride;
                v[k] ^= t[128u + (hi & 15u)] ^ t[144u + ((hi >> 4) & 15u)] ^ t[160u + ((hi >> 8) & 15u)] ^ t[176u + ((hi >> 12) & 15u)] ^ t[192u + ((hi >> 16) & 15u)];
            }
        }
#pragma unroll
        for (int k = 0; k < N; ++k) out[k] = min_nz(PT_ONE_MINUS_EPS, (float)v[k] * 0x1p-32f);
    }
};

template <int FEAT, bool ENVPRE> struct ShadeLdsSizes { enum : uint32_t { NPF = (FEAT & FEAT_INFINITE) ? 7u : 5u , MARG = ((FEAT & FEAT_INFINITE) && !ENVPRE) ? 1u : 0u  }; };
template <int FEAT, bool ENVPRE>
__device__ inline ShadeCtxLds<ENVPRE> stage_shade_tables(const DSampler &S, const DScene &sc, const ShadeLdsCfg &cfg, uint32_t *lds_sob, v4 *lds_tri, v4 *lds_light, float *lds_marg) {
    constexpr bool MARG = ShadeLdsSizes<FEAT, ENVPRE>::MARG != 0;
    {
        const uint32_t stride = sob_stride(cfg.sob_nib), nw = cfg.sob_nib * 16u;
        for (uint32_t i = threadIdx.x; i < cfg.sob_n * stride; i += BLOCK) { const uint32_t d = i / stride, w = i - d * stride; lds_sob[i] = w < nw ? S.nibtab[((size_t)(cfg.sob_lo + d) * SOBOL_NIBBLES) * 16u + w] : 0u; }
        if (cfg.tri_lds) { const v4 *g = reinterpret_cast<const v4 *>(sc.shade); for (uint32_t i = threadIdx.x; i < sc.n_prims * SH_TRI_REC_V4; i += BLOCK) lds_tri[i] = g[i]; }
        const v4 *gl = reinterpret_cast<const v4 *>(sc.lights);
        for (uint32_t i = threadIdx.x; i < cfg.n_lights_lds * SH_LIGHT_V4; i += BLOCK) lds_light[i] = gl[i];
        if (MARG && cfg.marg_li != 0xffffffffu) {
            const DLight &Le = sc.lights[cfg.marg_li];
            const uint32_t nv = (uint32_t)Le.nv, gv = Le.guide_v;
            for (uint32_t i = threadIdx.x; i < nv; i += BLOCK) lds_marg[i] = sc.distdata[Le.fint_off + i];
            for (uint32_t i = threadIdx.x; i < nv + 1u; i += BLOCK) lds_marg[SH_MARG_N + i] = sc.distdata[Le.mcdf_off + i];
            for (uint32_t i = threadIdx.x; i < gv + 1u; i += BLOCK) lds_marg[2u * SH_MARG_N + 1u + i] = sc.distdata[Le.mguide_off + i];
        }
    }
    ShadeCtxLds<ENVPRE> X; X.sob = (lds_u32 *)lds_sob; X.tris = (lds_v4 *)lds_tri; X.lights = (lds_v4 *)lds_light; X.cfg = cfg;
    if (!MARG) X.cfg.marg_li = 0xffffffffu;
    X.marg.func = lds_marg; X.marg.cdf = lds_marg + (MARG ? SH_MARG_N : 0); X.marg.guide = lds_marg + (MARG ? 2 * SH_MARG_N + 1 : 0);
    return X;
}

template <int MAT, int FEAT, bool ENVPRE>
__device__ inline void shade_segment(const DParams &R, const DSampler &S, const DCamera &C, const DScene &sc, const DPaths &P, const DQueues &Q, uint32_t it, uint32_t seg_cap, uint32_t Gn, uint32_t s,
                                     const ShadeCtxLds<ENVPRE> &X, v4 *lds_pf, bool &err_dim PT_STAMP_PARAMS) {
    const ShadeLdsCfg &cfg = X.cfg;
    const uint32_t wv = threadIdx.x >> 6, lane = threadIdx.x & 63u, par = it & 1u;
    auto dma = [&](const MatEntry &m) {
        typedef __attribute__((address_space(1))) const void gptr; typedef __attribute__((address_space(3))) void lptr;
        if (FEAT & FEAT_IMAGE) __builtin_amdgcn_global_load_lds((gptr *)&pslot(P.ray_o[par], m.e), (lptr *)(lds_pf + (0u * 4u + wv) * 64u), 16, 0, 0);
        __builtin_amdgcn_global_load_lds((gptr *)&pslot(P.ray_d[par], m.e), (lptr *)(lds_pf + (1u * 4u + wv) * 64u), 16, 0, 0);
        __builtin_amdgcn_global_load_lds((gptr *)&pslot(P.beta[par], m.e), (lptr *)(lds_pf + (2u * 4u + wv) * 64u), 16, 0, 0);
        __builtin_amdgcn_global_load_lds((gptr *)&pslot(P.st, m.pid), (lptr *)(lds_pf + (3u * 4u + wv) * 64u), 16, 0, 0);
        __builtin_amdgcn_global_load_lds((gptr *)&pslot(P.hit, m.e), (lptr *)(lds_pf + (4u * 4u + wv) * 64u), 16, 0, 0);
        if ((FEAT & FEAT_INFINITE) && cfg.pre_li != 0xffffffffu) {
            __builtin_amdgcn_global_load_lds((gptr *)&pslot(P.pre0, m.e), (lptr *)(lds_pf + (5u * 4u + wv) * 64u), 16, 0, 0);
            __builtin_amdgcn_global_load_lds((gptr *)&pslot(P.pre1, m.e), (lptr *)(lds_pf + (6u * 4u + wv) * 64u), 16, 0, 0);
        }
    };
    const MatEntry *__restrict__ queue = Q.mat[MAT] + (size_t)s * seg_cap;
    const uint32_t n = rfl(*seg_count(Q, it, Q_MAT0 + MAT, Gn, s));
    if (n == 0) return;
    const uint32_t next_base = rfl(*seg_count(Q, it + 1u, Q_EXT, Gn, s)), nee_base = rfl(*seg_count(Q, it, Q_NEE, Gn, s));
    const uint32_t e_next0 = s * seg_cap + next_base, f0 = s * seg_cap + nee_base;
    uint32_t c_next = 0, c_nee = 0, c_shadow = 0, c_mis = 0;
    uint32_t i = lane;
    MatEntry m, m1; m.e = m.pid = m1.e = m1.pid = 0;
    if (i < n) { m = pslot(queue, i); dma(m); }
    if (i + 64u < n) m1 = pslot(queue, i + 64u);
    __builtin_amdgcn_s_waitcnt(0x0F70);
    while (i < n) {
        PathIn in;
        {
            lds_v4 *q = (lds_v4 *)lds_pf + threadIdx.x;
            if (FEAT & FEAT_IMAGE) in.ro = X.ld(q); else in.ro = mkv4(splat3(0.0f), 0.0f);
            in.rd = X.ld(q + BLOCK); in.beta = X.ld(q + 2 * BLOCK);
            const v4 a = X.ld(q + 3 * BLOCK), c = X.ld(q + 4 * BLOCK);
            in.st.x = f2u(a.x); in.st.y = f2u(a.y); in.st.z = f2u(a.z); in.st.w = f2u(a.w);
            in.hit.x = f2u(c.x); in.hit.y = f2u(c.y); in.hit.z = f2u(c.z); in.hit.w = f2u(c.w);
            if ((FEAT & FEAT_INFINITE) && cfg.pre_li != 0xffffffffu) { in.pre0 = X.ld(q + 5 * BLOCK); in.pre1 = X.ld(q + 6 * BLOCK); } else in.pre0 = in.pre1 = mkv4(splat3(0.0f), 0.0f);
        }
        __builtin_amdgcn_s_waitcnt(0xC07F);
        const uint32_t i2 = i + 64u;
        if (i2 < n) dma(m1);
        MatEntry m2; m2.e = m2.pid = 0;
        if (i2 + 64u < n) m2 = pslot(queue, i2 + 64u);
#ifdef PTRS_STAMPS
        const ShadeResult r = shade_item<MAT, FEAT>(R, S, C, sc, P, m.pid, in, X, stamp_acc, stamp_last);
#else
        const ShadeResult r = shade_item<MAT, FEAT>(R, S, C, sc, P, m.pid, in, X);
#endif
        err_dim = err_dim || r.err_dim;
        const uint32_t e_next = e_next0 + wave_push(c_next, r.next), f = f0 + wave_push(c_nee, r.nee);
        X.before_stores();
        store_shade_out(P, par ^ 1u, r, e_next, f);
        if (r.next) pslot(Q.ext[par ^ 1u], e_next) = m.pid;
        if (r.nee) pslot(Q.nee, f) = r.nee_entry(m.pid);
#ifdef PTRS_STAMPS
        { const unsigned long long t_ = __builtin_amdgcn_s_memtime(); stamp_acc[8] += t_ - stamp_last; stamp_last = t_; stamp_acc[10] += 1; }
#endif
        c_shadow += (uint32_t)__popcll(__ballot(r.shadow));
        c_mis += (uint32_t)__popcll(__ballot(r.mis));
        if (R.row_cost && (r.shadow || r.mis)) atomicAdd(R.row_cost + sample_row_of(R, m.pid), (r.shadow ? 1u : 0u) + (r.mis ? 1u : 0u));
        i = i2; m = m1; m1 = m2;
    }
    if (lane == 0) {
        *seg_count(Q, it + 1u, Q_EXT, Gn, s) = next_base + c_next;
        if (c_next) Q.alive[it + 1u] = 1u;
        *seg_count(Q, it, Q_NEE, Gn, s) = nee_base + c_nee;
        *seg_count(Q, it, Q_SHADOW, Gn, s) += c_shadow;
        *seg_count(Q, it, Q_MIS, Gn, s) += c_mis;
    }
}

template <int MAT, int FEAT, bool ENVPRE>
__global__ __launch_bounds__(BLOCK, (ShadeWaves<MAT, FEAT>::N)) void k_shade(DParams R, DSampler S, DCamera C, DScene sc, DPaths P, DQueues Q, uint32_t it, uint32_t seg_cap, ShadeLdsCfg cfg, uint32_t Gn, uint32_t *ticket) {
    __shared__ v4 lds_pf[ShadeLdsSizes<FEAT, ENVPRE>::NPF * BLOCK];
    __shared__ uint32_t lds_sob[SH_SOB_WORDS];
    __shared__ v4 lds_tri[SH_TRI_V4];
    __shared__ v4 lds_light[SH_LIGHTS * SH_LIGHT_V4];
    __shared__ float lds_marg[ShadeLdsSizes<FEAT, ENVPRE>::MARG ? SH_MARG_WORDS : 1];
    static_assert(2u * lds_alloc((uint32_t)(sizeof(lds_pf) + sizeof(lds_sob) + sizeof(lds_tri) + sizeof(lds_light) + sizeof(lds_marg))) <= (uint32_t)PTRS_LDS_PER_CU, "two shade workgroups per CU");
    bool err_dim = false;
    if (round_is_dead(Q, it)) return;
    const ShadeCtxLds<ENVPRE> X = stage_shade_tables<FEAT, ENVPRE>(S, sc, cfg, lds_sob, lds_tri, lds_light, lds_marg);
    __syncthreads();
#ifdef PTRS_STAMPS
    unsigned long long stamp_acc[12] = {0, 0, 0, 0, 0, 0, 0, 0, 0, 0, 0, 0}, stamp_last = __builtin_amdgcn_s_memtime();
    for (uint32_t s = seg_next(ticket, Gn); s < Gn; s = seg_next(ticket, Gn)) shade_segment<MAT, FEAT, ENVPRE>(R, S, C, sc, P, Q, it, seg_cap, Gn, s, X, lds_pf, err_dim, stamp_acc, stamp_last);
#else
    for (uint32_t s = seg_next(ticket, Gn); s < Gn; s = seg_next(ticket, Gn)) shade_segment<MAT, FEAT, ENVPRE>(R, S, C, sc, P, Q, it, seg_cap, Gn, s, X, lds_pf, err_dim);
#endif
    if (err_dim) atomicOr(&Q.stats[CNT_ERR], (unsigned long long)PTRS_ERRFLAG_SOBOL_DIM);
#ifdef PTRS_STAMPS
    { const unsigned long long t_ = __builtin_amdgcn_s_memtime(); stamp_acc[11] += t_ - stamp_last; }
    if ((threadIdx.x & 63u) == 0) for (int k = 0; k < 12; ++k) atomicAdd(&Q.stats[CNT_STAMP0 + k], stamp_acc[k]);
#endif
}

constexpr bool tail_votes_connect(int geom) { return geom == 0; }
template <int MAT, int FEAT, int GEOM, bool OVF, int DEPTH = 8>
__global__ __launch_bounds__(BLOCK, 2) void k_tail(DParams R, DSampler S, DCamera C, DScene sc, StackSpill spill, DPaths P, DQueues Q, uint32_t it0, uint32_t it_end, uint32_t seg_cap, uint32_t thresh_e, uint32_t thresh_c,
                                                   uint32_t kinds_mask, ShadeLdsCfg cfg, uint32_t Gn, uint32_t *ticket) {
    constexpr int FEAT_T = FEAT_SIMPLE;
    constexpr bool VOTE_C = tail_votes_connect(GEOM);
    __shared__ unsigned long long lds_stack[DEPTH * BLOCK];
    __shared__ v4 lds_geom[TravLds<DEPTH, GEOM>::V4];
    __shared__ v4 lds_pf[ShadeLdsSizes<FEAT, false>::NPF * BLOCK];
    __shared__ uint32_t lds_sob[4];
    __shared__ v4 lds_tri[SH_TRI_V4];
    __shared__ v4 lds_light[SH_LIGHTS * SH_LIGHT_V4];
    __shared__ float lds_marg[ShadeLdsSizes<FEAT, false>::MARG ? SH_MARG_WORDS : 1];
    static_assert(2u * lds_alloc((uint32_t)(sizeof(lds_stack) + sizeof(lds_geom) + sizeof(lds_pf) + sizeof(lds_sob) + sizeof(lds_tri) + sizeof(lds_light) + sizeof(lds_marg))) <= (uint32_t)PTRS_LDS_PER_CU, "two tail workgroups per CU");
    if (round_is_dead(Q, it0)) return;
    GeomTop GG; LdsGeom LG;
    stage_geometry<DEPTH, GEOM>(sc, lds_geom, GG, LG);
    cfg.sob_n = 0;
    const ShadeCtxLds<false> X = stage_shade_tables<FEAT, false>(S, sc, cfg, lds_sob, lds_tri, lds_light, lds_marg);
    __syncthreads();
    LdsStack<DEPTH, OVF> stk; stk.init(lds_stack, spill);
    uint32_t nn = 0, nt = 0; StepCount stepc;
    bool err_dim = false;
#ifdef PTRS_STAMPS
    unsigned long long stamp_acc[12] = {0, 0, 0, 0, 0, 0, 0, 0, 0, 0, 0, 0}, stamp_last = __builtin_amdgcn_s_memtime();
#endif
    for (uint32_t s = seg_next(ticket, Gn); s < Gn; s = seg_next(ticket, Gn)) {
        for (uint32_t it = it0; it < it_end; ++it) {
            if (rfl(*(volatile uint32_t *)seg_count(Q, it, Q_EXT, Gn, s)) == 0u) break;
#ifdef PTRS_STAMPS_EXT
            { unsigned long long xs[12] = {0, 0, 0, 0, 0, 0, 0, 0, 0, 0, 0, 0}, xs_last = 0; extend_segment<FEAT_T, DEPTH, OVF, GEOM, true>(R, sc, P, Q, it, seg_cap, thresh_e, kinds_mask, Gn, s, GG, LG, stk, nn, nt, stepc PT_XS_ARGS); }
#else
            extend_segment<FEAT_T, DEPTH, OVF, GEOM, true>(R, sc, P, Q, it, seg_cap, thresh_e, kinds_mask, Gn, s, GG, LG, stk, nn, nt, stepc);
#endif
            __threadfence_block();
#ifdef PTRS_STAMPS
            shade_segment<MAT, FEAT, false>(R, S, C, sc, P, Q, it, seg_cap, Gn, s, X, lds_pf, err_dim, stamp_acc, stamp_last);
#else
            shade_segment<MAT, FEAT, false>(R, S, C, sc, P, Q, it, seg_cap, Gn, s, X, lds_pf, err_dim);
#endif
            __threadfence_block();
            connect_segment<FEAT_T, DEPTH, OVF, GEOM, VOTE_C>(sc, P, Q, it, seg_cap, thresh_c, 1u, Gn, s, GG, LG, stk, nn, nt, stepc);
            __threadfence_block();
        }
    }
    if (err_dim) atomicOr(&Q.stats[CNT_ERR], (unsigned long long)PTRS_ERRFLAG_SOBOL_DIM);
    flush_trav_counters(R, Q, nn, nt, stepc);
}

template <int FEAT>
__global__ __launch_bounds__(BLOCK) void k_env_presample(DSampler S, DScene sc, DPaths P, DQueues Q, uint32_t it, uint32_t seg_cap, uint32_t nee_kinds, uint32_t env_li, ShadeLdsCfg cfg, uint32_t Gn, uint32_t *ticket) {
    __shared__ float lds_marg[SH_MARG_WORDS];
    __shared__ uint32_t lds_sob[SH_SOB_WORDS];
    if (round_is_dead(Q, it)) return;
    const DLight &Le = sc.lights[env_li];
    {
        const uint32_t stride = sob_stride(cfg.sob_nib), nw = cfg.sob_nib * 16u;
        for (uint32_t i = threadIdx.x; i < cfg.sob_n * stride; i += BLOCK) { const uint32_t d = i / stride, w = i - d * stride; lds_sob[i] = w < nw ? S.nibtab[((size_t)(cfg.sob_lo + d) * SOBOL_NIBBLES) * 16u + w] : 0u; }
        const uint32_t nv = (uint32_t)Le.nv, gv = Le.guide_v;
        for (uint32_t i = threadIdx.x; i < nv; i += BLOCK) lds_marg[i] = sc.distdata[Le.fint_off + i];
        for (uint32_t i = threadIdx.x; i < nv + 1u; i += BLOCK) lds_marg[SH_MARG_N + i] = sc.distdata[Le.mcdf_off + i];
        for (uint32_t i = threadIdx.x; i < gv + 1u; i += BLOCK) lds_marg[2u * SH_MARG_N + 1u + i] = sc.distdata[Le.mguide_off + i];
    }
    __syncthreads();
    InfMarginal marg; marg.func = lds_marg; marg.cdf = lds_marg + SH_MARG_N; marg.guide = lds_marg + 2 * SH_MARG_N + 1;
    ShadeCtxLds<false> X; X.sob = (lds_u32 *)lds_sob; X.tris = nullptr; X.lights = nullptr; X.cfg = cfg; X.marg = marg;
    const uint32_t lane = __lane_id();
    for (uint32_t s = seg_next(ticket, Gn); s < Gn; s = seg_next(ticket, Gn)) {
        for (int m = 0; m < 6; ++m) {
            if (!(nee_kinds & (1u << m))) continue;
            const MatEntry *__restrict__ queue = Q.mat[m] + (size_t)s * seg_cap;
            const uint32_t n = rfl(*seg_count(Q, it, Q_MAT0 + m, Gn, s));
            for (uint32_t i = lane; i < n; i += 64u) {
                const MatEntry me = pslot(queue, i);
                const u4 stv = pslot(P.st, me.pid);
                const uint32_t field = f2u(pslot(P.ray_d[it & 1u], me.e).w) & ST_DIM_MASK;
                const VertexDims V = vertex_dims(field, true);
                const uint64_t index = (uint64_t)stv.x | ((uint64_t)stv.y << 32);
                const uint32_t dc[1] = {V.nee[4]};
                float uc[1];
                X.sobol<1>(S, index, dc, stv.w, uc);
                const float fl = floor_(uc[0] * (float)sc.n_lights);
                uint32_t li = fl > 0.0f ? (uint32_t)fl : 0u;
                if (li > sc.n_lights - 1u) li = sc.n_lights - 1u;
                if (li != env_li) continue;
                const uint32_t dn[2] = {V.nee[0], V.nee[1]};
                float u[2];
                X.sobol<2>(S, index, dn, stv.w, u);
                f3 wi, rgb; float pdf;
                const bool ok = inf_light_sample(sc, Le, mk2(u[0], u[1]), wi, pdf, rgb, &marg);
                pslot(P.pre0, me.e) = mkv4(wi, pdf);
                pslot(P.pre1, me.e) = mkv4(rgb, u2f(ok ? 1u : 0u));
            }
        }
    }
}

__global__ __launch_bounds__(BLOCK) void k_reduce_counts(const uint32_t *__restrict__ counts, uint32_t G, uint32_t *__restrict__ totals) {
    __shared__ uint32_t acc;
    if (threadIdx.x == 0) acc = 0;
    __syncthreads();
    uint32_t v = 0;
    for (uint32_t b = threadIdx.x; b < G; b += BLOCK) v += counts[(size_t)blockIdx.x * G + b];
    for (int off = 32; off > 0; off >>= 1) v += (uint32_t)__shfl_down((int)v, off);
    if ((threadIdx.x & 63) == 0) atomicAdd(&acc, v);
    __syncthreads();
    if (threadIdx.x == 0) totals[blockIdx.x] = acc;
}

struct FilmTile { int32_t tx0, ty0, lx, ly, x, y; bool live; uint32_t my_bits; };
__device__ inline FilmTile film_tile(const DParams &R, int32_t y0, int32_t y1, int32_t tiles_x) {
    const int32_t tx0 = (int32_t)(blockIdx.x % (uint32_t)tiles_x) * 16, ty0 = y0 + (int32_t)(blockIdx.x / (uint32_t)tiles_x) * 16;
    const int32_t lx = (int32_t)(threadIdx.x & 15u), ly = (int32_t)(threadIdx.x >> 4);
    return FilmTile{tx0, ty0, lx, ly, tx0 + lx, ty0 + ly, tx0 + lx < R.W && ty0 + ly < y1, (1u << (uint32_t)lx) | (1u << (16u + (uint32_t)ly))};
}
__device__ inline bool film_apron_pid(const DParams &R, const DSampler &S, const FilmTile &T, uint32_t e, uint32_t k, uint32_t npix, uint32_t &pid) {
    const int32_t sx = T.tx0 - 2 + (int32_t)(e % 20u) - S.min_x, sy = T.ty0 - 2 + (int32_t)(e / 20u) - S.min_y;
    pid = k * npix + (uint32_t)(sy - R.row0) * (uint32_t)R.NX + (uint32_t)sx;
    return sx >= 0 && sx < R.NX && sy >= R.row0 && sy < R.row1;
}
__device__ inline uint32_t film_footprint_mask(float pdx, float pdy, const FilmTile &T) {
    const int32_t p0x = (int32_t)ceil_(pdx - 2.0f), p0y = (int32_t)ceil_(pdy - 2.0f), p1x = (int32_t)(floor_(pdx + 2.0f) + 1.0f), p1y = (int32_t)(floor_(pdy + 2.0f) + 1.0f);
    auto span = [](int32_t lo, int32_t hi) {
        const uint32_t l = (uint32_t)(lo < 0 ? 0 : (lo > 16 ? 16 : lo)), h = (uint32_t)(hi < 0 ? 0 : (hi > 16 ? 16 : hi));
        return h > l ? ((1u << h) - 1u) & ~((1u << l) - 1u) : 0u;
    };
    return span(p0x - T.tx0, p1x - T.tx0) | (span(p0y - T.ty0, p1y - T.ty0) << 16);
}
__global__ __launch_bounds__(BLOCK) void k_film(DParams R, DSampler S, DPaths P, const float *__restrict__ table, v4 *film, int32_t y0, int32_t y1, int32_t tiles_x) {
    __shared__ float tab[256];
    __shared__ v4 s_a[400]; __shared__ float s_lb[400];
    __shared__ uint32_t s_m[400];
    tab[threadIdx.x] = table[threadIdx.x];
    const FilmTile T = film_tile(R, y0, y1, tiles_x);
    v4 acc; acc.x = acc.y = acc.z = acc.w = 0.0f;
    if (T.live) acc = film[(size_t)T.y * (size_t)R.W + (size_t)T.x];
    const uint32_t npix = (uint32_t)(R.row1 - R.row0) * (uint32_t)R.NX;
    const uint32_t ns = R.s1 - R.s0;
    for (uint32_t k = 0; k < ns; ++k) {
        __syncthreads();
        for (uint32_t e = threadIdx.x; e < 400u; e += BLOCK) {
// ... 214 lines not shown
};
std::mutex g_mu;
std::vector<SobolDevice *> g_sobol;

int get_sobol(int device, SobolDevice **out) {
    std::lock_guard<std::mutex> lk(g_mu);
    for (auto *s : g_sobol) if (s->device == device) { *out = s; return PTRS_OK; }
    const unsigned char *b = k_sobol_blob;
    if (sizeof(k_sobol_blob) < 32 || std::memcmp(b, "PTRSSOB1", 8) != 0) { g_err = "embedded sobol tables corrupt"; return PTRS_ERR_INVALID; }
    uint32_t hdr[6]; std::memcpy(hdr, b + 8, 24);
    const size_t nmat = (size_t)hdr[0] * hdr[1], stride = hdr[4];
    const unsigned char *pm = b + 32, *pv = pm + nmat * 4 + 52 * 4, *pvi = pv + (size_t)hdr[2] * stride * 8;
    std::unique_ptr<SobolDevice> s(new SobolDevice());
    s->device = device; s->stride = (uint32_t)stride;
    int rc;
    const size_t mat_pad = 16 * 52 * 4;
    if ((rc = s->matrices.ensure(nmat * 4 + mat_pad)) != PTRS_OK || (rc = s->vdc.ensure((size_t)hdr[2] * stride * 8)) != PTRS_OK || (rc = s->vdc_inv.ensure((size_t)hdr[3] * stride * 8)) != PTRS_OK) return rc;
    HIPCHK(hipMemset(s->matrices.p, 0, nmat * 4 + mat_pad));
    HIPCHK(hipMemcpy(s->matrices.p, pm, nmat * 4, hipMemcpyHostToDevice));
    HIPCHK(hipMemcpy(s->vdc.p, pv, (size_t)hdr[2] * stride * 8, hipMemcpyHostToDevice));
    HIPCHK(hipMemcpy(s->vdc_inv.p, pvi, (size_t)hdr[3] * stride * 8, hipMemcpyHostToDevice));
    SobolTablesHost T; T.matrices.resize(nmat); std::memcpy(T.matrices.data(), pm, nmat * 4);
    std::vector<uint32_t> bt; build_sobol_bytetab(T, bt);
    if ((rc = upload(s->bytetab, bt)) != PTRS_OK) return rc;
    std::vector<uint32_t> nt((size_t)1024 * SOBOL_NIBBLES * 16, 0u);
    for (uint32_t d = 0; d < 1024; ++d)
        for (uint32_t n = 0; n < (uint32_t)SOBOL_NIBBLES; ++n)
            for (uint32_t v = 0; v < 16; ++v) {
                uint32_t x = 0;
                for (uint32_t j = 0; j < 4; ++j) if ((v >> j) & 1u) { const uint32_t col = 4 * n + j; if (col < 52) x ^= T.matrices[(size_t)d * 52 + col]; }
                nt[((size_t)d * SOBOL_NIBBLES + n) * 16 + v] = x;
            }
    if ((rc = upload(s->nibtab, nt)) != PTRS_OK) return rc;
    g_sobol.push_back(s.get());
    *out = s.release();
    return PTRS_OK;
}

}

enum { MAX_LANES = 8 };
struct PtrsScene {
    int device = 0;
    HostScene H;
    DScene sc{};
    DevBuf nodes2, nodes4, nodes, tris, shade, mats, texs, levels, texdata, lights, distdata, inf;
    DevBuf stack_spill;
    StackSpill spill{nullptr, 0};
    size_t spill_lane_elems = 0;
    std::map<std::string, int> overrides;
    std::map<const void *, int> occupancy;
    uint32_t stack_lds = 16;
    std::vector<double> alive_frac;
    DevBuf ws[MAX_LANES][32];
    DevBuf counts[MAX_LANES], totals[MAX_LANES], tickets[MAX_LANES];
    DevBuf stats, table, film_tmp, samples_tmp, strat1, strat2, row_cost;
    DevBuf half_tmp, cv_tiles, cv_summary;
    DevBuf aov_film_tmp[AOV_PLANES], aov_samples_tmp;
    DevBuf aov_band[4], aov_band_pfilm;
    hipStream_t lane_stream[MAX_LANES] = {};
    hipEvent_t lane_ev[MAX_LANES] = {};
    std::vector<hipEvent_t> ev_pool;
    int n_cu = 256;
    ~PtrsScene() {
        for (auto st : lane_stream) if (st) (void)hipStreamDestroy(st);
        for (auto e : lane_ev) if (e) (void)hipEventDestroy(e);
        for (auto e : ev_pool) (void)hipEventDestroy(e);
    }
};

struct PtrsDenoiser {
    int device = 0;
    int32_t W = 0, H = 0;
    DevBuf ws;
    DevBuf stage[5];
};

namespace {

int require_spill(const PtrsScene *ps) {
    if (ps->spill_lane_elems == 0 || ps->spill.p) return PTRS_OK;
    g_err = "the scene has lost its traversal stack spill columns (an earlier allocation failed); a render allocates them again";
    return PTRS_ERR_DEVICE;
}

#define PTRS_K(...) (const void *)__VA_ARGS__
#define PTRS_TRAV_V(K, F, D, O, G) PTRS_K(K<F, D, O, G, true>), PTRS_K(K<F, D, O, G, false>)
#define PTRS_TRAV_O(K, F, D, G) PTRS_TRAV_V(K, F, D, true, G), PTRS_TRAV_V(K, F, D, false, G)
#define PTRS_TRAV_ALL(K, F) PTRS_TRAV_V(K, F, 9, false, LDS9_V4), PTRS_TRAV_O(K, F, 8, 640), PTRS_TRAV_O(K, F, 8, 1536), PTRS_TRAV_O(K, F, 8, 0), PTRS_TRAV_O(K, F, 16, 0)
#define PTRS_CONNECT_ALL(F) PTRS_TRAV_ALL(k_connect_rf, F), PTRS_K(k_resolve<F>)
#define PTRS_SHADE_ALL(F, E) PTRS_K(k_shade<0, F, E>), PTRS_K(k_shade<1, F, E>), PTRS_K(k_shade<2, F, E>), PTRS_K(k_shade<3, F, E>), PTRS_K(k_shade<4, F, E>), PTRS_K(k_shade<5, F, E>)
#define PTRS_TAIL_O(M, F, G) PTRS_K(k_tail<M, F, G, true>), PTRS_K(k_tail<M, F, G, false>)
[[maybe_unused]] const void *const k_code_object_order[] = {
    PTRS_K(k_epilogue<FEAT_FULL>), PTRS_K(k_epilogue<FEAT_IMG_ENV>), PTRS_K(k_epilogue<FEAT_SIMPLE>), PTRS_CONNECT_ALL(FEAT_FULL), PTRS_CONNECT_ALL(FEAT_IMG_ENV), PTRS_CONNECT_ALL(FEAT_SIMPLE),
    PTRS_SHADE_ALL(FEAT_SIMPLE, false), PTRS_SHADE_ALL(FEAT_IMG, false), PTRS_SHADE_ALL(FEAT_IMG_ENV, true), PTRS_SHADE_ALL(FEAT_IMG_ENV, false), PTRS_SHADE_ALL(FEAT_FULL, true), PTRS_SHADE_ALL(FEAT_FULL, false),
    PTRS_K(k_env_presample<FEAT_IMG_ENV>), PTRS_K(k_env_presample<FEAT_FULL>), PTRS_K(k_tail<PTRS_MAT_MATTE, FEAT_SIMPLE, LDS9_V4, false, 9>), PTRS_TAIL_O(PTRS_MAT_MATTE, FEAT_SIMPLE, 640), PTRS_TAIL_O(PTRS_MAT_MATTE, FEAT_SIMPLE, 1536),
    PTRS_TAIL_O(PTRS_MAT_MATTE, FEAT_SIMPLE, 0), PTRS_TAIL_O(PTRS_MAT_DISNEY, FEAT_IMG, 0), PTRS_K(k_aov<FEAT_SIMPLE>), PTRS_K(k_aov<FEAT_FULL>),
    PTRS_K(k_dn_iter_lds<1>), PTRS_K(k_dn_iter_lds<2>), PTRS_K(k_dn_iter_lds<4>), PTRS_K(k_dn_iter_lds<8>), PTRS_K(k_dn_iter_lds<16>),
    PTRS_K(k_trace<true, 8, false>), PTRS_K(k_trace<true, 8, true>), PTRS_K(k_trace<true, 16, false>), PTRS_K(k_trace<true, 16, true>), PTRS_K(k_trace<false, 8, false>), PTRS_K(k_trace<false, 8, true>), PTRS_K(k_trace<false, 16, false>), PTRS_K(k_trace<false, 16, true>),
    PTRS_TRAV_ALL(k_extend_rf, FEAT_FULL), PTRS_TRAV_ALL(k_extend_rf, FEAT_IMG_ENV), PTRS_TRAV_ALL(k_extend_rf, FEAT_SIMPLE)};
#undef PTRS_K
#undef PTRS_TRAV_V
#undef PTRS_TRAV_O
#undef PTRS_TRAV_ALL
#undef PTRS_CONNECT_ALL
#undef PTRS_SHADE_ALL
#undef PTRS_TAIL_O

struct HipBackend {
    PtrsScene *ps; hipStream_t stream; SobolDevice *sob;
    DScene sc; DSampler S; DCamera C; DParams R; DPaths P; DQueues Q;
    uint32_t cap = 0, rows = 0, depth = 0, flags = 0, kinds_mask = 0;
    int feat = FEAT_FULL, feat_trace = FEAT_FULL;
    struct TravForm {
        int depth = 16, geom = 0;
        bool ovf = false;
        uint32_t v4 = 0;
        bool vote = true, vote_connect = true;
    } form;
    uint32_t G = 1, seg_cap = 0;
    struct Lane { hipStream_t stream; DParams R; DPaths P; DQueues Q; uint32_t G, seg_cap; };
    Lane lane_[MAX_LANES]; uint32_t n_lanes = 1, cur = 0;
    hipEvent_t film_prev = nullptr;
    Options opt;
    uint32_t lanes(uint64_t job_paths = 0, const bool * = nullptr, bool single_pixel = false, uint32_t spp = 0xffffffffu) {
        int want = opt.lanes;
        if (want == 0) want = (single_pixel || spp < 2u) ? 1 : (job_paths >= (4ull << 20) ? 4 : 2);
        if (share > 1 && opt.lanes == 0) want = std::max(1, want / share);
        n_lanes = (uint32_t)(want < 1 ? 1 : (want > MAX_LANES ? MAX_LANES : want));
        return n_lanes;
    }
    void plan_segments(uint64_t max_paths) {
        if (opt.grid_mult == 0) {
            opt.grid_mult = n_lanes > 1 ? 1 : 8;
            if (n_lanes > 1 && ps->sc.n_nodes4 != 0) {
                const uint64_t per_unit = (uint64_t)ps->n_cu * 8u * 10240u;
                const uint64_t k = (max_paths + per_unit / 2) / per_unit;
                opt.grid_mult = (int)(k < 1 ? 1 : (k > 4 ? 4 : k));
            }
            if (opt.grid_pct == 0) opt.grid_pct = 100;
        }
        if (opt.grid_pct == 0) opt.grid_pct = n_lanes > 1 ? 50 : 100;
    }
    void select(uint32_t l) {
        if (l == cur) return;
        lane_[cur] = Lane{stream, R, P, Q, G, seg_cap};
        cur = l; stream = lane_[l].stream; R = lane_[l].R; P = lane_[l].P; Q = lane_[l].Q; G = lane_[l].G; seg_cap = lane_[l].seg_cap;
    }
    uint64_t auto_capacity(uint32_t lanes_n, const bool *kinds) {
        size_t fr = 0, tot = 0;
        if (hipMemGetInfo(&fr, &tot) != hipSuccess) return 1ull << 27;
        size_t held = 0;
        for (auto &l : ps->ws) for (auto &b : l) held += b.bytes;
        held += ps->stack_spill.bytes;
        uint32_t nk = 0; for (int k = 0; k < 7; ++k) nk += kinds[k] ? 1u : 0u;
        const double per_path = (17.0 + (ps->H.inf_lights.empty() ? 0.0 : 2.0)) * 16.0 + 8.0 + 4.0 + 3.0 * 4.0 + nk * 8.0;
        const double budget = (double)(fr + held) * (double)opt.workspace_pct / 100.0 / (double)std::max(1, share);
        const double cap = budget / (per_path * (double)lanes_n);
        return cap < 65536.0 ? 65536ull : (uint64_t)cap;
    }
    int share = 1;
    int grid_max = 8192;
    uint32_t refill_connect = 16;
    uint32_t refill = 16;
    int rc = PTRS_OK;
    struct Span { int cat; hipEvent_t a, b; };
    std::vector<Span> spans; size_t ev_next = 0;
    uint64_t launches = 0, trace_launches = 0;

    const uint32_t *sobol_matrices() { return (const uint32_t *)sob->matrices.p; }
    const uint32_t *sobol_bytetab() { return (const uint32_t *)sob->bytetab.p; }
    const uint32_t *sobol_nibtab() { return (const uint32_t *)sob->nibtab.p; }
    const uint64_t *sobol_vdc(uint32_t row) { return (const uint64_t *)sob->vdc.p + (size_t)row * sob->stride; }
    const uint64_t *sobol_vdc_inv(uint32_t row) { return (const uint64_t *)sob->vdc_inv.p + (size_t)row * sob->stride; }
    int strat_tables(int32_t NX, int32_t NY, uint32_t dim_ps, uint32_t n_dims, const float **t1, const float **t2, std::string &err) {
        const size_t n = (size_t)NX * (size_t)NY * n_dims * dim_ps * dim_ps;
        size_t fr = 0, tot = 0;
        if (hipMemGetInfo(&fr, &tot) == hipSuccess && n * 12 > (fr + ps->strat1.bytes + ps->strat2.bytes) / 2) { err = "stratified sampler: the per-pixel tables (" + std::to_string(n * 12 >> 20) + " MiB) do not fit"; return PTRS_ERR_UNSUPPORTED; }
        int rc;
        if ((rc = ps->strat1.ensure(n * 4)) != PTRS_OK || (rc = ps->strat2.ensure(n * 8)) != PTRS_OK) { err = g_err; return rc; }
        const int32_t tiles = ((NX + 15) / 16) * ((NY + 15) / 16);
        hipLaunchKernelGGL(k_strat_tables, dim3((uint32_t)(tiles + 63) / 64), dim3(64), 0, stream, NX, NY, dim_ps, n_dims, (float *)ps->strat1.p, (float *)ps->strat2.p);
        if (hipStreamSynchronize(stream) != hipSuccess || hipGetLastError() != hipSuccess) { err = "stratified table kernel failed"; return PTRS_ERR_DEVICE; }
        *t1 = (const float *)ps->strat1.p; *t2 = (const float *)ps->strat2.p;
        return PTRS_OK;
    }

    hipEvent_t ev() {
        if (ev_next == ps->ev_pool.size()) { hipEvent_t e; if (hipEventCreate(&e) != hipSuccess) { rc = PTRS_ERR_DEVICE; return nullptr; } ps->ev_pool.push_back(e); }
        return ps->ev_pool[ev_next++];
    }
    enum { T_EXTEND = 0, T_AUX = 1, T_FILM = 2, T_CONNECT = 3, T_SHADE = 4, T_TAIL = 5, T_NUM = 6 };
    uint64_t cat_launches[T_NUM] = {0, 0, 0, 0, 0, 0};
    void t0(int cat) { if (flags & PTRS_FLAG_TIMING) { Span s; s.cat = cat; s.a = ev(); s.b = ev(); if (s.a) (void)hipEventRecord(s.a, stream); spans.push_back(s); } ++launches; ++cat_launches[cat]; if (cat == T_EXTEND || cat == T_CONNECT) ++trace_launches; }
    void t1() { if (flags & PTRS_FLAG_TIMING) { if (spans.back().b) (void)hipEventRecord(spans.back().b, stream); } }
    int grid_for(uint32_t n) const { uint32_t g = (n + BLOCK - 1) / BLOCK; if (g < 1) g = 1; const uint32_t gm = (uint32_t)ps->n_cu * 8u; return (int)(g > gm ? gm : g); }

    uint32_t last_grid[T_NUM] = {0, 0, 0, 0, 0, 0}, last_per_cu[T_NUM] = {0, 0, 0, 0, 0, 0};
    template <class F> int wgs_per_cu(F fn) {
        const void *key = reinterpret_cast<const void *>(fn);
        auto itr = ps->occupancy.find(key);
        if (itr != ps->occupancy.end()) return opt.persist ? itr->second : 8;
        int nb = 0;
        if (hipOccupancyMaxActiveBlocksPerMultiprocessor(&nb, fn, BLOCK, 0) != hipSuccess || nb < 1) { (void)hipGetLastError(); nb = 1; }
        hipFuncAttributes fa;
        if (hipFuncGetAttributes(&fa, key) == hipSuccess) { if (fa.sharedSizeBytes > 0) nb = std::max(1, std::min(nb, (int)lds_wgs_per_cu((uint32_t)fa.sharedSizeBytes))); } else (void)hipGetLastError();
        ps->occupancy[key] = nb > 8 ? 8 : nb;
        return opt.persist ? ps->occupancy[key] : 8;
    }
// ... 21 lines not shown
        form.depth = (int)ps->stack_lds; form.ovf = ps->spill_lane_elems != 0;
        form.v4 = pair ? LN_V4 * ps->sc.n_nodes2 + 9u * ps->sc.n_prims : 0u;
        form.geom = form.depth == 9 ? LDS9_V4 : (form.depth == 8 && pair && form.v4 <= 640u) ? 640 : (form.depth == 8 && pair && form.v4 <= 1536u) ? 1536 : 0;
        const bool vote = form.vote = opt.vote >= 0 ? opt.vote != 0 : true;
        const bool vote_connect = form.vote_connect = opt.vote >= 0 ? opt.vote == 1 : !pair;
        refill = (uint32_t)(opt.refill > 0 ? opt.refill : (opt.refill == 0 ? 64 : ((vote && feat_trace == FEAT_SIMPLE) ? 32 : 16)));
        refill_connect = (uint32_t)(opt.refill_connect > 0 ? opt.refill_connect : (opt.refill_connect == 0 ? 64 : ((vote_connect && feat_trace == FEAT_SIMPLE) ? 32 : 16)));
    }
    int begin(const DScene &sc_, const DSampler &S_, const DCamera &C_, uint32_t capacity, uint32_t count_rows, uint32_t bvh_depth, uint32_t flags_, int feat_, int feat_trace_, std::string &err) {
        sc = sc_; S = S_; C = C_; cap = capacity; rows = count_rows; depth = bvh_depth; flags = flags_; feat = feat_;
        plan_segments(capacity);
        traversal_policy(feat_trace_);
        for (int k = 0; k < 7; ++k) if (ps->H.kinds_present[k]) kinds_mask |= 1u << k;
        grid_max = ps->n_cu * 8 * (opt.grid_mult ? opt.grid_mult : 8);
        if (opt.persist && opt.whole_rounds) grid_max = (int)whole_rounds((uint32_t)grid_max);
        const size_t n16 = (size_t)cap * 16, n4 = ((size_t)cap + ((size_t)grid_max + 1) * 64) * 4;
        if ((rc = ps->stats.ensure(CNT_NUM * 8)) != PTRS_OK || (rc = ps->table.ensure(1024)) != PTRS_OK) { err = g_err; return rc; }
        if (ps->spill_lane_elems) {
            rc = ps->stack_spill.ensure(ps->spill_lane_elems * n_lanes * sizeof(unsigned long long));
            ps->spill.p = (unsigned long long *)ps->stack_spill.p;
            if (rc != PTRS_OK) { err = g_err + " (traversal stack spill columns)"; return rc; }
        }
        if ((rc = require_spill(ps)) != PTRS_OK) { err = g_err; return rc; }
        for (uint32_t l = 0; l < n_lanes && n_lanes > 1; ++l) {
            if (l > 0 && !ps->lane_stream[l] && hipStreamCreateWithFlags(&ps->lane_stream[l], hipStreamNonBlocking) != hipSuccess) { err = "cannot create a pipeline stream"; return PTRS_ERR_DEVICE; }
            if (!ps->lane_ev[l] && hipEventCreateWithFlags(&ps->lane_ev[l], hipEventDisableTiming) != hipSuccess) { err = "cannot create pipeline events"; return PTRS_ERR_DEVICE; }
        }
        const size_t nq = n4 / 4;
        const bool presampled = presample_li() != 0xffffffffu;
        for (uint32_t l = 0; l < n_lanes; ++l) {
            DPaths Pl; DQueues Ql;
            std::memset(&Pl, 0, sizeof(Pl));
            int w = 0;
            auto take = [&](size_t bytes, void **out, const char *what) -> int {
                int r = ps->ws[l][w].ensure(bytes);
                if (r != PTRS_OK) { err = g_err + " (" + what + " of pipeline lane " + std::to_string(l) + "; ptrs_set_option(\"lanes\", 1) or a smaller workspace_pct shrink the workspace)"; return r; }
                *out = ps->ws[l][w++].p;
                return PTRS_OK;
            };
            void **by_queue16[] = {(void **)&Pl.ray_o[0], (void **)&Pl.ray_o[1], (void **)&Pl.ray_d[0], (void **)&Pl.ray_d[1], (void **)&Pl.beta[0], (void **)&Pl.beta[1], (void **)&Pl.hit,
                                   (void **)&Pl.nee0, (void **)&Pl.nee1, (void **)&Pl.nee2, (void **)&Pl.sh_o, (void **)&Pl.sh_d, (void **)&Pl.mis_o, (void **)&Pl.mis_d, (void **)&Pl.nhit};
            for (auto sl : by_queue16) if ((rc = take(nq * 16, sl, "path state")) != PTRS_OK) return rc;
            void **by_slot16[] = {(void **)&Pl.L, (void **)&Pl.st};
            for (auto sl : by_slot16) if ((rc = take(n16, sl, "path state")) != PTRS_OK) return rc;
            if ((rc = take((size_t)cap * 8, (void **)&Pl.pfilm, "path state")) != PTRS_OK) return rc;
            if ((rc = take(nq * 4, (void **)&Pl.pre_z, "path state")) != PTRS_OK) return rc;
            if (presampled) { if ((rc = take(nq * 16, (void **)&Pl.pre0, "path state")) != PTRS_OK || (rc = take(nq * 16, (void **)&Pl.pre1, "path state")) != PTRS_OK) return rc; } else w += 2;
            void **slots4[] = {(void **)&Ql.ext[0], (void **)&Ql.ext[1], (void **)&Ql.nee};
            for (auto sl : slots4) if ((rc = take(n4, sl, "queues")) != PTRS_OK) return rc;
            for (int k = 0; k < Q_NUM_MAT; ++k) {
                Ql.mat[k] = nullptr;
                if (kinds_mask & (1u << k)) { if ((rc = take(nq * sizeof(MatEntry), (void **)&Ql.mat[k], "queues")) != PTRS_OK) return rc; } else ++w;
            }
            if ((rc = ps->counts[l].ensure((size_t)rows * Q_STRIDE * (size_t)grid_max * 4)) != PTRS_OK || (rc = ps->totals[l].ensure((size_t)rows * Q_STRIDE * 4)) != PTRS_OK ||
                (rc = ps->tickets[l].ensure(((size_t)rows * Q_STRIDE * TK_LAUNCH_WORDS + rows) * 4)) != PTRS_OK) { err = g_err; return rc; }
            Ql.counts = (uint32_t *)ps->counts[l].p; Ql.stats = (unsigned long long *)ps->stats.p; Ql.tickets = (uint32_t *)ps->tickets[l].p; Ql.alive = Ql.tickets + (size_t)rows * Q_STRIDE * TK_LAUNCH_WORDS;
            lane_[l] = Lane{l == 0 ? stream : ps->lane_stream[l], DParams{}, Pl, Ql, 1u, 0u};
        }
        cur = 0; P = lane_[0].P; Q = lane_[0].Q;
        float tab[256]; gaussian_filter_table(tab);
        if (hipMemcpyAsync(ps->table.p, tab, 1024, hipMemcpyHostToDevice, stream) != hipSuccess || hipMemsetAsync(Q.stats, 0, CNT_NUM * 8, stream) != hipSuccess || hipStreamSynchronize(stream) != hipSuccess) { err = "workspace initialisation failed"; return PTRS_ERR_DEVICE; }
        film_prev = nullptr;
        return PTRS_OK;
    }
    void pass_begin(const DParams &R_) {
        R = R_;
        const uint32_t chunks = (R.n_paths + 63u) / 64u;
        G = chunks < (uint32_t)grid_max ? chunks : (uint32_t)grid_max;
        if (G < 1) G = 1;
        seg_cap = ((chunks + G - 1) / G) * 64u;
        (void)hipMemsetAsync(Q.counts, 0, (size_t)rows * Q_STRIDE * G * 4, stream);
        (void)hipMemsetAsync(Q.tickets, 0, ((size_t)rows * Q_STRIDE * TK_LAUNCH_WORDS + rows) * 4, stream);
    }
    void generate() { t0(T_AUX); hipLaunchKernelGGL(k_generate, dim3((G + WAVES - 1) / WAVES), dim3(BLOCK), 0, stream, R, S, C, P, Q, seg_cap, G, (uint32_t)deal_by_region()); t1(); }
    int deal_by_region() const { return opt.deal; }

    typedef void (*TravFn)(DParams, DScene, StackSpill, DPaths, DQueues, uint32_t, uint32_t, uint32_t, uint32_t, uint32_t, uint32_t *);
#define PTRS_PICK(K, D, O, GE) (v ? (TravFn)K<FEAT, D, O, GE, true> : (TravFn)K<FEAT, D, O, GE, false>)
#define PTRS_PICK_OVF(K, D, GE) (form.ovf ? PTRS_PICK(K, D, true, GE) : PTRS_PICK(K, D, false, GE))
#define PTRS_PICK_ALL(K) (form.depth == 9 ? PTRS_PICK(K, 9, false, LDS9_V4) : form.depth == 8 ? (form.geom == 640 ? PTRS_PICK_OVF(K, 8, 640) : form.geom == 1536 ? PTRS_PICK_OVF(K, 8, 1536) : PTRS_PICK_OVF(K, 8, 0)) : PTRS_PICK_OVF(K, 16, 0))
    typedef void (*EpilogueFn)(DParams, DScene, DPaths, DQueues, uint32_t, uint32_t, uint32_t, uint32_t, uint32_t *);
    struct ConnectFns { TravFn connect; void (*resolve)(DScene, DPaths, DQueues, uint32_t, uint32_t, uint32_t, uint32_t *); };
    template <int FEAT> TravFn pick_extend_t() { const bool v = form.vote; return PTRS_PICK_ALL(k_extend_rf); }
    template <int FEAT> ConnectFns pick_connect_t() { const bool v = form.vote_connect; return ConnectFns{PTRS_PICK_ALL(k_connect_rf), k_resolve<FEAT>}; }
#undef PTRS_PICK_ALL
#undef PTRS_PICK_OVF
#undef PTRS_PICK
    EpilogueFn epilogue_fn() const {
        static const EpilogueFn by_feat[3] = {k_epilogue<FEAT_FULL>, k_epilogue<FEAT_IMG_ENV>, k_epilogue<FEAT_SIMPLE>};
        return by_feat[feat_trace == FEAT_FULL ? 0 : feat_trace == FEAT_IMG_ENV ? 1 : 2];
    }
    ConnectFns pick_connect() { return feat_trace == FEAT_FULL ? pick_connect_t<FEAT_FULL>() : feat_trace == FEAT_IMG_ENV ? pick_connect_t<FEAT_IMG_ENV>() : pick_connect_t<FEAT_SIMPLE>(); }
    TravFn pick_extend() { return feat_trace == FEAT_FULL ? pick_extend_t<FEAT_FULL>() : feat_trace == FEAT_IMG_ENV ? pick_extend_t<FEAT_IMG_ENV>() : pick_extend_t<FEAT_SIMPLE>(); }
    StackSpill lane_spill() { StackSpill sp = ps->spill; if (sp.p) sp.p += (size_t)cur * ps->spill_lane_elems; return sp; }

    void extend(uint32_t it) {
        t0(T_EXTEND);
        const StackSpill sp = lane_spill();
        const uint32_t epi_mask = opt.fused_epilogue ? kinds_mask : 0u;
        const TravFn fn = pick_extend();
        hipLaunchKernelGGL(fn, dim3(persistent_grid(fn, T_EXTEND)), dim3(BLOCK), 0, stream, R, sc, sp, P, Q, it, seg_cap, refill, epi_mask, G, ticket(it, TK_EXTEND));
        if (!epi_mask) {
            t1(); t0(T_AUX);
            const EpilogueFn ep = epilogue_fn();
            hipLaunchKernelGGL(ep, dim3(persistent_grid(ep, T_AUX)), dim3(BLOCK), 0, stream, R, sc, P, Q, it, kinds_mask, seg_cap, G, ticket(it, TK_EPILOGUE));
        }
        t1();
    }
    void connect(uint32_t it) {
        t0(T_CONNECT);
        const StackSpill sp = lane_spill();
        const uint32_t fused = (opt.fused_epilogue && opt.fused_resolve) ? 1u : 0u;
        const ConnectFns cf = pick_connect();
        const TravFn fn = cf.connect;
        hipLaunchKernelGGL(fn, dim3(persistent_grid(fn, T_CONNECT)), dim3(BLOCK), 0, stream, R, sc, sp, P, Q, it, seg_cap, refill_connect, fused, G, ticket(it, TK_CONNECT));
        if (!fused) {
            t1(); t0(T_AUX);
            hipLaunchKernelGGL(cf.resolve, dim3(persistent_grid(cf.resolve, T_AUX)), dim3(BLOCK), 0, stream, sc, P, Q, it, seg_cap, G, ticket(it, TK_RESOLVE));
        }
        t1();
    }
    ShadeLdsCfg shade_cfg(uint32_t it) const {
        ShadeLdsCfg c;
        c.sob_nib = (2u * S.log2_res + (31u - (uint32_t)__builtin_clz(S.spp)) <= 32u) ? 8u : (uint32_t)SOBOL_NIBBLES;
        const uint32_t cap = SH_SOB_WORDS / sob_stride(c.sob_nib), top = std::min<uint32_t>(1024u, 3u + 8u * it + 9u);
        c.sob_lo = top > cap ? top - cap : 0u; c.sob_n = top - c.sob_lo;
        c.tri_lds = (sc.n_prims * SH_TRI_REC_V4 <= SH_TRI_V4 && opt.shade_lds) ? 1u : 0u;
        c.n_lights_lds = opt.shade_lds ? std::min<uint32_t>(sc.n_lights, SH_LIGHTS) : 0u;
        if (!opt.shade_lds) c.sob_n = 0;
        c.pre_li = presample_li();
        c.marg_li = 0xffffffffu;
        if (opt.shade_lds && !ps->H.inf_lights.empty()) {
            const DLight &Le = ps->H.lights[ps->H.inf_lights[0]];
            if (Le.nv >= 1 && (uint32_t)Le.nv <= SH_MARG_N && Le.guide_v >= 1 && Le.guide_v <= SH_MARG_N) c.marg_li = ps->H.inf_lights[0];
        }
        return c;
    }
    typedef void (*ShadeFn)(DParams, DSampler, DCamera, DScene, DPaths, DQueues, uint32_t, uint32_t, ShadeLdsCfg, uint32_t, uint32_t *);
    template <int FEAT, bool ENVPRE> ShadeFn shade_fn_t(int kind) {
        switch (kind) {
            case 0: return k_shade<0, FEAT, ENVPRE>;
            case 1: return k_shade<1, FEAT, ENVPRE>;
            case 2: return k_shade<2, FEAT, ENVPRE>;
            case 3: return k_shade<3, FEAT, ENVPRE>;
            case 4: return k_shade<4, FEAT, ENVPRE>;
            default: return k_shade<5, FEAT, ENVPRE>;
        }
    }
    bool env_presampled_only() const { return presample_li() != 0xffffffffu && ps->H.inf_lights.size() == 1; }
    ShadeFn shade_fn(int kind) {
        if (feat == FEAT_SIMPLE) return shade_fn_t<FEAT_SIMPLE, false>(kind);
        if (feat == FEAT_IMG) return shade_fn_t<FEAT_IMG, false>(kind);
        if (feat == FEAT_IMG_ENV) return env_presampled_only() ? shade_fn_t<FEAT_IMG_ENV, true>(kind) : shade_fn_t<FEAT_IMG_ENV, false>(kind);
        return env_presampled_only() ? shade_fn_t<FEAT_FULL, true>(kind) : shade_fn_t<FEAT_FULL, false>(kind);
    }
    uint32_t presample_li() const {
        if (!opt.env_presample || !(feat & FEAT_INFINITE) || S.kind != PTRS_SAMPLER_SOBOL || ps->H.inf_lights.empty()) return 0xffffffffu;
        const DLight &Le = ps->H.lights[ps->H.inf_lights[0]];
        return (Le.nv >= 1 && (uint32_t)Le.nv <= SH_MARG_N && Le.guide_v >= 1 && Le.guide_v <= SH_MARG_N) ? ps->H.inf_lights[0] : 0xffffffffu;
    }
    void presample(uint32_t it) {
        const uint32_t li = presample_li();
        const uint32_t nee_kinds = kinds_mask & 0x3fu & ~((1u << PTRS_MAT_MIRROR) | (1u << PTRS_MAT_GLASS));
        if (li == 0xffffffffu || !nee_kinds) return;
        t0(T_AUX);
        void (*const fn)(DSampler, DScene, DPaths, DQueues, uint32_t, uint32_t, uint32_t, uint32_t, ShadeLdsCfg, uint32_t, uint32_t *) = feat == FEAT_IMG_ENV ? k_env_presample<FEAT_IMG_ENV> : k_env_presample<FEAT_FULL>;
        hipLaunchKernelGGL(fn, dim3(persistent_grid(fn, T_AUX)), dim3(BLOCK), 0, stream, S, sc, P, Q, it, seg_cap, nee_kinds, li, shade_cfg(it), G, ticket(it, TK_PRESAMPLE));
        t1();
    }
    typedef void (*TailFn)(DParams, DSampler, DCamera, DScene, StackSpill, DPaths, DQueues, uint32_t, uint32_t, uint32_t, uint32_t, uint32_t, uint32_t, ShadeLdsCfg, uint32_t, uint32_t *);
    enum : uint32_t { TAIL_PATHS_DEFAULT = 192 };
    TailFn tail_fn() {
        if (!opt.tail || !opt.fused_epilogue || !opt.fused_resolve || !opt.shade_lds || !opt.persist || form.depth == 16 || feat_trace != FEAT_SIMPLE || S.kind != PTRS_SAMPLER_SOBOL) return nullptr;
        if (!form.vote || form.vote_connect != tail_votes_connect(form.geom)) return nullptr;
        int kind = -1;
        for (int k = 0; k < 7; ++k) if (ps->H.kinds_present[k]) { if (kind >= 0) return nullptr; kind = k; }
#define PTRS_TAIL(M, F, GE) (form.ovf ? (TailFn)k_tail<M, F, GE, true> : (TailFn)k_tail<M, F, GE, false>)
        if (kind == PTRS_MAT_MATTE && feat == FEAT_SIMPLE)
            return form.depth == 9 ? (TailFn)k_tail<PTRS_MAT_MATTE, FEAT_SIMPLE, LDS9_V4, false, 9> : form.geom == 640 ? PTRS_TAIL(PTRS_MAT_MATTE, FEAT_SIMPLE, 640) : form.geom == 1536 ? PTRS_TAIL(PTRS_MAT_MATTE, FEAT_SIMPLE, 1536) : PTRS_TAIL(PTRS_MAT_MATTE, FEAT_SIMPLE, 0);
        if (kind == PTRS_MAT_DISNEY && feat == FEAT_IMG && form.geom == 0) return PTRS_TAIL(PTRS_MAT_DISNEY, FEAT_IMG, 0);
#undef PTRS_TAIL
        return nullptr;
    }
    uint32_t tail_round(uint32_t n_paths, uint32_t n_rounds) {
        if (!tail_fn()) return 0xffffffffu;
        if (opt.tail_at >= 0) return (uint32_t)opt.tail_at < n_rounds ? (uint32_t)opt.tail_at : 0xffffffffu;
        const double limit = (double)(opt.tail_paths > 0 ? (uint32_t)opt.tail_paths : (uint32_t)TAIL_PATHS_DEFAULT) * (double)G;
        const std::vector<double> &f = ps->alive_frac;
        for (uint32_t it = 0; it < n_rounds && it < f.size(); ++it) if (f[it] * (double)n_paths <= limit) return it;
        return 0xffffffffu;
    }
    uint32_t tail_at_last = 0xffffffffu;
    void tail(uint32_t it0, uint32_t it_end) {
        const TailFn fn = tail_fn();
        if (!fn) return;
        t0(T_TAIL);
        hipLaunchKernelGGL(fn, dim3(persistent_grid(fn, T_TAIL)), dim3(BLOCK), 0, stream, R, S, C, sc, lane_spill(), P, Q, it0, it_end, seg_cap, refill, refill_connect, kinds_mask & 0x3fu, shade_cfg(it0), G, ticket(it0, TK_TAIL));
        t1();
        tail_at_last = it0;
    }
    void learn(const uint32_t *counts, uint32_t n_rows, uint32_t n_paths) {
        if (!n_paths || n_paths < 4096u) return;
        std::vector<double> f(n_rows);
        for (uint32_t i = 0; i < n_rows; ++i) f[i] = (double)counts[(size_t)i * Q_STRIDE + Q_EXT] / (double)n_paths;
        ps->alive_frac.swap(f);
    }
    void shade(uint32_t it, int kind) {
        t0(T_SHADE);
        if (kind > 5) kind = 5;
        const ShadeFn fn = shade_fn(kind);
        hipLaunchKernelGGL(fn, dim3(persistent_grid(fn, T_SHADE)), dim3(BLOCK), 0, stream, R, S, C, sc, P, Q, it, seg_cap, shade_cfg(it), G, ticket(it, TK_SHADE0 + kind));
        t1();
    }
    void reduce_counts(uint32_t n_rows) { hipLaunchKernelGGL(k_reduce_counts, dim3(n_rows * Q_STRIDE), dim3(BLOCK), 0, stream, (const uint32_t *)Q.counts, G, (uint32_t *)ps->totals[cur].p); }
    uint32_t read_count(uint32_t it, int q) {
        std::vector<uint32_t> seg(G);
        (void)hipMemcpyAsync(seg.data(), Q.counts + ((size_t)it * Q_STRIDE + (size_t)q) * G, (size_t)G * 4, hipMemcpyDeviceToHost, stream);
        if (hipStreamSynchronize(stream) != hipSuccess) { rc = PTRS_ERR_DEVICE; return 0; }
        uint64_t t = 0; for (uint32_t v : seg) t += v;
        return t > 0xffffffffull ? 0xffffffffu : (uint32_t)t;
    }
    void read_counts(uint32_t *dst, uint32_t n_rows) {
        reduce_counts(n_rows);
        (void)hipMemcpyAsync(dst, ps->totals[cur].p, (size_t)n_rows * Q_STRIDE * 4, hipMemcpyDeviceToHost, stream);
        if (hipStreamSynchronize(stream) != hipSuccess) rc = PTRS_ERR_DEVICE;
    }
    void film(v4 *film_px, int32_t y0, int32_t y1) {
        const int32_t tiles_x = (R.W + 15) / 16, tiles_y = (y1 - y0 + 15) / 16;
        if (n_lanes > 1 && film_prev) (void)hipStreamWaitEvent(stream, film_prev, 0);
        t0(T_FILM); hipLaunchKernelGGL(k_film, dim3((uint32_t)tiles_x * (uint32_t)tiles_y), dim3(BLOCK), 0, stream, R, S, P, (const float *)ps->table.p, film_px, y0, y1, tiles_x); t1();
        if (n_lanes > 1) { film_prev = ps->lane_ev[cur]; (void)hipEventRecord(film_prev, stream); }
    }
    PtrsFilmPixel *host_film = nullptr; int32_t film_w = 0;
    void publish_rows(v4 *film_px, int32_t y0, int32_t y1) {
        if (!host_film || hipStreamSynchronize(stream) != hipSuccess) { rc = host_film ? PTRS_ERR_DEVICE : rc; return; }
        const size_t off = (size_t)y0 * (size_t)film_w, cnt = (size_t)(y1 - y0) * (size_t)film_w;
        if (hipMemcpyAsync(host_film + off, film_px + off, cnt * sizeof(PtrsFilmPixel), hipMemcpyDeviceToHost, stream) != hipSuccess || hipStreamSynchronize(stream) != hipSuccess) rc = PTRS_ERR_DEVICE;
    }
    void dump_rays(uint32_t it, const RayDump &d) {
        DevBuf cnt;
        if (cnt.ensure(16) != PTRS_OK) { rc = PTRS_ERR_DEVICE; return; }
        (void)hipMemsetAsync(cnt.p, 0, 16, stream);
        hipLaunchKernelGGL(k_dump_rays, dim3((G + WAVES - 1) / WAVES), dim3(BLOCK), 0, stream, P, Q, it, seg_cap, G, d.max_rays, d.out, (uint32_t *)cnt.p);
        uint32_t n = 0;
        if (hipMemcpyAsync(&n, cnt.p, 4, hipMemcpyDeviceToHost, stream) != hipSuccess || hipStreamSynchronize(stream) != hipSuccess) rc = PTRS_ERR_DEVICE;
        *d.n_out = n < d.max_rays ? n : d.max_rays;
    }
    bool aov_band = false;
    int aov_band_begin(uint64_t n, std::string &err) {
        for (auto &b : ps->aov_band) if ((rc = b.ensure((size_t)n * 16)) != PTRS_OK) { err = g_err + " (feature-plane band arrays)"; return rc; }
        if ((rc = ps->aov_band_pfilm.ensure((size_t)n * 8)) != PTRS_OK) { err = g_err + " (feature-plane band arrays)"; return rc; }
        aov_band = true;
        return PTRS_OK;
    }
    DAov aov_arrays(bool depth_plane) const {
        DAov A;
        if (aov_band) { A.albedo = (v4 *)ps->aov_band[0].p; A.normal = (v4 *)ps->aov_band[1].p; A.pos = (v4 *)ps->aov_band[2].p; A.depthp = depth_plane ? (v4 *)ps->aov_band[3].p : nullptr; A.pfilm = (f2a *)ps->aov_band_pfilm.p; }
        else { A.albedo = P.sh_o; A.normal = P.sh_d; A.pos = P.mis_o; A.depthp = depth_plane ? P.mis_d : nullptr; A.pfilm = nullptr; }
        return A;
    }
    bool aov_depth_plane(uint32_t planes) const { return !opt.aov_fused_film && (planes & PTRS_AOV_DEPTH) != 0; }
    void aov(uint32_t planes, uint32_t off) {
// ... 969 lines not shown
```

Baseline: 13200.

## Split matte shading into hot kernel plus cold replay queue

Adds a hot variant of the matte shade kernel that compiles out rare paths, such as the double-precision triangle-edge fallback, and instead flags the item as cold. Flagged items are pushed to a replay queue and reprocessed by a generic replay kernel launched afterward. The aim is a leaner hot kernel with lower register pressure and higher occupancy for the common case. The cost is an extra launch per matte shade round, extra queue memory and bookkeeping, and some redundant work for replayed items.

```diff
diff --git a/include/ptrs.h b/include/ptrs.h
--- a/include/ptrs.h
+++ b/include/ptrs.h
@@ -180,6 +180,8 @@
     uint64_t tail_round;
     uint64_t stack_lds;
     uint64_t lds_form_v4;
+    uint64_t shade_items;
+    uint64_t shade_replayed;
 } PtrsStats;
 
 enum {
diff --git a/pathtracer-rs_amd/abi.py b/pathtracer-rs_amd/abi.py
--- a/pathtracer-rs_amd/abi.py
+++ b/pathtracer-rs_amd/abi.py
@@ -81,7 +81,7 @@
                 ("tri_steps_x64", C.c_uint64), ("debug", C.c_uint64 * 12), ("queue_segments", C.c_uint64), ("grid_wgs", C.c_uint64 * 4),
                 ("resident_wgs_per_cu", C.c_uint64 * 4), ("lanes", C.c_uint64), ("grid_pct", C.c_uint64), ("ms_enqueue", C.c_double),
                 ("ms_tail", C.c_double), ("tail_launches", C.c_uint64), ("tail_round", C.c_uint64),
-                ("stack_lds", C.c_uint64), ("lds_form_v4", C.c_uint64)]
+                ("stack_lds", C.c_uint64), ("lds_form_v4", C.c_uint64), ("shade_items", C.c_uint64), ("shade_replayed", C.c_uint64)]
 
     def as_dict(self):
         return {n: getattr(self, n) for n, _ in self._fields_}
diff --git a/pathtracer-rs_amd/csrc/pt_hip_queue.h b/pathtracer-rs_amd/csrc/pt_hip_queue.h
--- a/pathtracer-rs_amd/csrc/pt_hip_queue.h
+++ b/pathtracer-rs_amd/csrc/pt_hip_queue.h
@@ -31,5 +31,5 @@
     }
 }
 __device__ inline uint32_t *seg_count(const DQueues &Q, uint32_t row, int q, uint32_t G, uint32_t s) { return Q.counts + ((size_t)row * Q_STRIDE + (size_t)q) * G + s; }
-enum { TK_EXTEND = 0, TK_CONNECT = 1, TK_SHADE0 = 2, TK_EPILOGUE = 9, TK_RESOLVE = 10, TK_PRESAMPLE = 11, TK_TAIL = 12 };
+enum { TK_EXTEND = 0, TK_CONNECT = 1, TK_SHADE0 = 2, TK_EPILOGUE = 9, TK_RESOLVE = 10, TK_PRESAMPLE = 11, TK_TAIL = 12, TK_REPLAY = 13 };
 __device__ inline bool round_is_dead(const DQueues &Q, uint32_t it) { return it > 0u && rfl(Q.alive[it]) == 0u; }
diff --git a/pathtracer-rs_amd/csrc/pt_items.h b/pathtracer-rs_amd/csrc/pt_items.h
--- a/pathtracer-rs_amd/csrc/pt_items.h
+++ b/pathtracer-rs_amd/csrc/pt_items.h
@@ -123,7 +123,7 @@
 
 struct VertexDraws { float u_nee[5], u_tail[3]; uint32_t after_cont, after_rr; bool err_cont, err_rr; };
 template <class CTX>
-PT_HD void draw_vertex(const CTX &X, const DSampler &S, const u4 &stv, bool nee, VertexDraws &D) {
+PT_HD void draw_vertex(const CTX &X, const DSampler &S, const u4 &stv, bool nee, VertexDraws &D, bool &cold) {
     const uint32_t field = stv.z & ST_DIM_MASK;
     for (int k = 0; k < 5; ++k) D.u_nee[k] = 0.0f;
     if (S.kind == PTRS_SAMPLER_STRATIFIED) {
@@ -151,25 +151,27 @@
     if (nee) {
         const uint32_t dn[8] = {V.nee[0], V.nee[1], V.nee[2], V.nee[3], V.nee[4], dt[0], dt[1], dt[2]};
         float u8[8];
-        X.template sobol<8>(S, index, dn, stv.w, u8);
+        X.template sobol<8>(S, index, dn, stv.w, u8, cold);
         for (int k = 0; k < 5; ++k) D.u_nee[k] = u8[k];
         D.u_tail[0] = u8[5]; D.u_tail[1] = u8[6]; D.u_tail[2] = u8[7];
-    } else X.template sobol<3>(S, index, dt, stv.w, D.u_tail);
+    } else X.template sobol<3>(S, index, dt, stv.w, D.u_tail, cold);
     D.after_cont = V.after_cont; D.err_cont = V.after_cont > 1024u;
     D.after_rr = V.after_cont + 1u; D.err_rr = V.after_cont + 1u > 1024u;
 }
 
 struct ShadeCtx {
+    static constexpr bool cold_inline = true;
     static constexpr bool inf_fallback = true;
     PT_MEM TriRegs tri(const DScene &sc, int32_t prim, bool want_dp) const { return load_tri_regs(sc.shade + prim, want_dp); }
     PT_MEM void light(const DScene &sc, uint32_t li, DLight &out) const { out = sc.lights[li]; }
     PT_MEM const InfMarginal *inf_marginal(uint32_t) const { return nullptr; }
     PT_MEM bool presampled(uint32_t) const { return false; }
-    template <int N> PT_MEM void sobol(const DSampler &S, uint64_t index, const uint32_t (&dim)[N], uint32_t scramble, float (&out)[N]) const { sobol_batch<N>(S, index, dim, scramble, out); }
+    template <int N> PT_MEM void sobol(const DSampler &S, uint64_t index, const uint32_t (&dim)[N], uint32_t scramble, float (&out)[N], bool &) const { sobol_batch<N>(S, index, dim, scramble, out); }
     PT_MEM void before_stores() const {}
 };
 
 struct ShadeResult {
+    bool cold;
     bool next; bool nee; bool shadow; bool mis; bool err_dim;
     v4 ro, rd, beta;
     v4 sh_o, sh_d, mis_o, mis_d, nee0, nee1; u4 nee2; float pre_z;
@@ -187,7 +189,7 @@
 
 template <int MAT, int FEAT, class CTX = ShadeCtx>
 PT_HD ShadeResult shade_item(const DParams &R, const DSampler &S, const DCamera &C, const DScene &sc, const DPaths &P, uint32_t pid, const PathIn &in, const CTX &X PT_STAMP_PARAMS) {
-    ShadeResult out; out.next = false; out.nee = false; out.shadow = false; out.mis = false; out.err_dim = false; out.pre_z = 0.0f;
+    ShadeResult out; out.cold = false; out.next = false; out.nee = false; out.shadow = false; out.mis = false; out.err_dim = false; out.pre_z = 0.0f;
     const v4 rov = in.ro, rdv = in.rd;
     v4 bv = in.beta;
     u4 stv = in.st; stv.z = f2u(rdv.w);
@@ -203,7 +205,8 @@
     const bool nee_guess = NEE_KIND && sc.n_lights > 0;
     const TriRegs T = X.tri(sc, prim, (FEAT & FEAT_IMAGE) != 0);
     VertexDraws D;
-    draw_vertex(X, S, stv, nee_guess, D);
+    bool cold = false;
+    draw_vertex(X, S, stv, nee_guess, D, cold);
     float (&u_nee)[5] = D.u_nee; float (&u_tail)[3] = D.u_tail;
     PT_STAMP(1, f2u(T.ng.x) + f2u(T.p0.x) + f2u(T.n0.x) + f2u(T.uv0.x) + f2u(u_tail[2]) + f2u(u_nee[4]) + T.flags)
     uint32_t li = 0;
@@ -238,7 +241,7 @@
 #else
     const bool do_nee = bsdf_num(bsdf, NS) > 0 && sc.n_lights > 0;
 #endif
-    if (do_nee != nee_guess) draw_vertex(X, S, stv, false, D);
+    if (do_nee != nee_guess) draw_vertex(X, S, stv, false, D, cold);
     if (do_nee) {
         DLight Lt;
         X.light(sc, li, Lt);
@@ -249,7 +252,7 @@
             ls.p1_err = splat3(0.0f); ls.p1_n = splat3(0.0f);
             ls.wi = xyz(in.pre0); ls.pdf = in.pre0.w; ls.li = xyz(in.pre1);
             ls.p1 = f2u(in.pre1.w) ? s.p + ls.wi * (2.0f * Lt.world_radius) : s.p;
-        } else light_sample_li<FEAT, CTX::inf_fallback>(sc, Lt, s.p, sp, u_light, ls, X.inf_marginal(li));
+        } else light_sample_li<FEAT, CTX::inf_fallback, CTX::cold_inline>(sc, Lt, s.p, sp, u_light, ls, X.inf_marginal(li), &cold);
         PT_STAMP(4, f2u(ls.pdf) + f2u(ls.wi.x) + f2u(ls.li.x) + f2u(ls.p1.x))
         f3 A = splat3(0.0f);
         float spdf = 0.0f;
@@ -275,7 +278,7 @@
             if (!is_black(fB) && spdf > 0.0f) {
                 bool ok = true;
                 if (!(sampled & BSDF_SPECULAR)) {
-                    float lpdf = light_pdf_li<FEAT>(sc, Lt, s.p, sp, wi);
+                    float lpdf = light_pdf_li<FEAT, CTX::cold_inline>(sc, Lt, s.p, sp, wi, &cold);
                     if (lpdf == 0.0f) ok = false;
                     else wB = power_heuristic(spdf, lpdf);
                 }
@@ -343,6 +346,7 @@
     }
     if (out.err_dim) { out.nee = false; out.shadow = false; out.mis = false; out.next = false; }
     }
+    out.cold = cold;
     if (w_skip) { w_rd = mkv4(rd, u2f(w_stz)); w_beta = bv; out.next = true; }
     return out;
 }
diff --git a/pathtracer-rs_amd/csrc/pt_light.h b/pathtracer-rs_amd/csrc/pt_light.h
--- a/pathtracer-rs_amd/csrc/pt_light.h
+++ b/pathtracer-rs_amd/csrc/pt_light.h
@@ -51,11 +51,11 @@
     }
 }
 
-template <int FEAT>
-PT_HD float tri_pdf_at_point(const DScene &sc, const TriRegs &T, float area, f3 ref_p, const SpawnPair &ref_sp, f3 wi, const float *n_fixed = nullptr) {
+template <int FEAT, bool COLD_INLINE = true>
+PT_HD float tri_pdf_at_point(const DScene &sc, const TriRegs &T, float area, f3 ref_p, const SpawnPair &ref_sp, f3 wi, const float *n_fixed = nullptr, bool *cold = nullptr) {
     f3 o = spawn_from(ref_sp, wi);
     TriHit h;
-    if (!tri_test(o, wi, PT_INF, T.p0, T.p1, T.p2, h)) return 0.0f;
+    if (!tri_test<COLD_INLINE>(o, wi, PT_INF, T.p0, T.p1, T.p2, h, cold)) return 0.0f;
     if (T.flags & TRI_DEGENERATE) return 0.0f;
     if ((FEAT & FEAT_ALPHA) && (T.flags & TRI_HAS_ALPHA)) {
         const f2 uv = mk2(h.b0 * T.uv0.x + h.b1 * T.uv1.x + h.b2 * T.uv2.x, h.b0 * T.uv0.y + h.b1 * T.uv1.y + h.b2 * T.uv2.y);
@@ -102,8 +102,8 @@
     return ok;
 }
 
-template <int FEAT, bool INF = true>
-PT_HD bool light_sample_li(const DScene &sc, const DLight &L, f3 ref_p, const SpawnPair &ref_sp, f2 u, LightSample &o, const InfMarginal *im = nullptr) {
+template <int FEAT, bool INF = true, bool COLD_INLINE = true>
+PT_HD bool light_sample_li(const DScene &sc, const DLight &L, f3 ref_p, const SpawnPair &ref_sp, f2 u, LightSample &o, const InfMarginal *im = nullptr, bool *cold = nullptr) {
     f3 li = splat3(0.0f), wi = splat3(0.0f), p1 = ref_p, p1_err = splat3(0.0f), p1_n = splat3(0.0f);
     float pdf = 0.0f;
     bool ok = true;
@@ -120,7 +120,7 @@
         f3 p, n, perr; f2 uv;
         tri_sample(T, u, p, n, perr, uv, L.n_ok ? L.n_sample : nullptr);
         wi = normalize(p - ref_p);
-        pdf = tri_pdf_at_point<FEAT>(sc, T, L.area, ref_p, ref_sp, wi, L.n_ok ? L.n_point : nullptr);
+        pdf = tri_pdf_at_point<FEAT, COLD_INLINE>(sc, T, L.area, ref_p, ref_sp, wi, L.n_ok ? L.n_point : nullptr, cold);
         p1 = p; p1_err = perr; p1_n = n;
         f3 w = -wi;
         li = dot(n, w) > 0.0f ? (L.ke_const ? ld3(L.c) : tex_eval<FEAT>(sc, L.ke_tex, uv, 0.0f, 0.0f, 0.0f, 0.0f)) : splat3(0.0f);
@@ -133,9 +133,9 @@
     return ok;
 }
 
-template <int FEAT>
-PT_HD float light_pdf_li(const DScene &sc, const DLight &L, f3 ref_p, const SpawnPair &ref_sp, f3 w) {
-    if (L.kind == 2) return tri_pdf_at_point<FEAT>(sc, load_tri_regs(&L.T), L.area, ref_p, ref_sp, w, L.n_ok ? L.n_point : nullptr);
+template <int FEAT, bool COLD_INLINE = true>
+PT_HD float light_pdf_li(const DScene &sc, const DLight &L, f3 ref_p, const SpawnPair &ref_sp, f3 w, bool *cold = nullptr) {
+    if (L.kind == 2) return tri_pdf_at_point<FEAT, COLD_INLINE>(sc, load_tri_regs(&L.T), L.area, ref_p, ref_sp, w, L.n_ok ? L.n_point : nullptr, cold);
     if ((FEAT & FEAT_INFINITE) && L.kind == 3) {
         f3 wi = xform_vec(L.w2l, w);
         float theta = spherical_theta(wi), phi = spherical_phi(wi);
diff --git a/pathtracer-rs_amd/csrc/pt_probe.h b/pathtracer-rs_amd/csrc/pt_probe.h
--- a/pathtracer-rs_amd/csrc/pt_probe.h
+++ b/pathtracer-rs_amd/csrc/pt_probe.h
@@ -63,6 +63,9 @@
     out[0] = ls.wi.x; out[1] = ls.wi.y; out[2] = ls.wi.z; out[3] = ls.pdf;
     out[4] = ls.li.x; out[5] = ls.li.y; out[6] = ls.li.z; out[7] = ok ? 1.0f : 0.0f;
     out[8] = pq; out[9] = le.x; out[10] = le.y; out[11] = le.z;
+    bool cold = false;
+    const float pq_hot = light_pdf_li<FEAT_IMG_ENV, false>(sc, L, p, sp, wq, &cold);
+    out[12] = cold ? 1.0f : 0.0f; out[13] = pq_hot;
 }
 
 PT_HD void texture_probe_row(const DScene &sc, int32_t tex, const float *in, float *out) {
diff --git a/pathtracer-rs_amd/csrc/pt_render.h b/pathtracer-rs_amd/csrc/pt_render.h
--- a/pathtracer-rs_amd/csrc/pt_render.h
+++ b/pathtracer-rs_amd/csrc/pt_render.h
@@ -293,6 +293,8 @@
             st.rays_extension += counts[(size_t)i * Q_STRIDE + Q_EXT];
             st.rays_shadow += counts[(size_t)i * Q_STRIDE + Q_SHADOW];
             st.rays_mis += counts[(size_t)i * Q_STRIDE + Q_MIS];
+            for (int k = 0; k < Q_NUM_MAT; ++k) st.shade_items += counts[(size_t)i * Q_STRIDE + Q_MAT0 + k];
+            st.shade_replayed += counts[(size_t)i * Q_STRIDE + Q_REPLAY];
         }
         st.samples += pd.n_paths;
         st.passes += 1;
diff --git a/pathtracer-rs_amd/csrc/pt_scene.h b/pathtracer-rs_amd/csrc/pt_scene.h
--- a/pathtracer-rs_amd/csrc/pt_scene.h
+++ b/pathtracer-rs_amd/csrc/pt_scene.h
@@ -173,7 +173,7 @@
     u4 *nhit;
 };
 
-enum { Q_EXT = 0, Q_SHADOW = 1, Q_MIS = 2, Q_NEE = 3, Q_MAT0 = 4, Q_NUM_MAT = 7, Q_STRIDE = 16 };
+enum { Q_EXT = 0, Q_SHADOW = 1, Q_MIS = 2, Q_NEE = 3, Q_MAT0 = 4, Q_NUM_MAT = 7, Q_REPLAY = 11, Q_STRIDE = 16 };
 enum { CNT_EXT = 0, CNT_SHADOW = 1, CNT_MIS = 2, CNT_NODES = 3, CNT_TRIS = 4,
        CNT_NODE_STEPS = 5, CNT_NODE_VISITS = 6, CNT_TRI_STEPS = 7,
        CNT_ERR = 8,
@@ -184,10 +184,12 @@
 struct DQueues {
     uint32_t *ext[2];
     MatEntry *mat[Q_NUM_MAT];
+    MatEntry *replay;
     uint32_t *nee;
     uint32_t *counts;
     uint32_t *tickets;
     uint32_t *alive;
+    uint32_t *replay_any;
     unsigned long long *stats;
 };
 
diff --git a/pathtracer-rs_amd/csrc/pt_tri.h b/pathtracer-rs_amd/csrc/pt_tri.h
--- a/pathtracer-rs_amd/csrc/pt_tri.h
+++ b/pathtracer-rs_amd/csrc/pt_tri.h
@@ -16,7 +16,8 @@
     return S;
 }
 
-PT_HD bool tri_test_perm(f3 p0t, f3 p1t, f3 p2t, float sx, float sy, float sz, float t_max, TriHit &h) {
+template <bool COLD_INLINE = true>
+PT_HD bool tri_test_perm(f3 p0t, f3 p1t, f3 p2t, float sx, float sy, float sz, float t_max, TriHit &h, bool *cold = nullptr) {
     p0t.x += sx * p0t.z; p0t.y += sy * p0t.z;
     p1t.x += sx * p1t.z; p1t.y += sy * p1t.z;
     p2t.x += sx * p2t.z; p2t.y += sy * p2t.z;
@@ -24,9 +25,11 @@
     float e1 = p2t.x * p0t.y - p2t.y * p0t.x;
     float e2 = p0t.x * p1t.y - p0t.y * p1t.x;
     if (e0 == 0.0f || e1 == 0.0f || e2 == 0.0f) {
-        e0 = (float)((double)p2t.y * (double)p1t.x - (double)p2t.x * (double)p1t.y);
-        e1 = (float)((double)p0t.y * (double)p2t.x - (double)p0t.x * (double)p2t.y);
-        e2 = (float)((double)p1t.y * (double)p0t.x - (double)p1t.x * (double)p0t.y);
+        if (COLD_INLINE) {
+            e0 = (float)((double)p2t.y * (double)p1t.x - (double)p2t.x * (double)p1t.y);
+            e1 = (float)((double)p0t.y * (double)p2t.x - (double)p0t.x * (double)p2t.y);
+            e2 = (float)((double)p1t.y * (double)p0t.x - (double)p1t.x * (double)p0t.y);
+        } else *cold = true;
     }
     const float det = e0 + e1 + e2;
     if ((((e0 < 0.0f) | (e1 < 0.0f) | (e2 < 0.0f)) & ((e0 > 0.0f) | (e1 > 0.0f) | (e2 > 0.0f))) | (det == 0.0f)) return false;
@@ -81,7 +84,8 @@
     h.t = t; h.b0 = e0 * inv_det; h.b1 = e1 * inv_det; h.b2 = e2 * inv_det;
     return !(rej_sign | rej_range) & !(t <= delta_t);
 }
-PT_HD bool tri_test_s(f3 o, const RayShear &S, float t_max, f3 p0, f3 p1, f3 p2, TriHit &h) {
+template <bool COLD_INLINE = true>
+PT_HD bool tri_test_s(f3 o, const RayShear &S, float t_max, f3 p0, f3 p1, f3 p2, TriHit &h, bool *cold = nullptr) {
     f3 p0t = p0 - o, p1t = p1 - o, p2t = p2 - o;
     const int kz = S.kz;
     int kx = kz + 1; if (kx == 3) kx = 0;
@@ -89,7 +93,7 @@
     p0t = mk3(comp(p0t, kx), comp(p0t, ky), comp(p0t, kz));
     p1t = mk3(comp(p1t, kx), comp(p1t, ky), comp(p1t, kz));
     p2t = mk3(comp(p2t, kx), comp(p2t, ky), comp(p2t, kz));
-    return tri_test_perm(p0t, p1t, p2t, S.sx, S.sy, S.sz, t_max, h);
+    return tri_test_perm<COLD_INLINE>(p0t, p1t, p2t, S.sx, S.sy, S.sz, t_max, h, cold);
 }
 PT_HD bool tri_test_s_sel(f3 o, const RayShear &S, float t_max, f3 p0, f3 p1, f3 p2, TriHit &h) {
     f3 p0t = p0 - o, p1t = p1 - o, p2t = p2 - o;
@@ -110,7 +114,8 @@
     S.sx = -dx / dz; S.sy = -dy / dz; S.sz = comp(inv, S.kz);
     return S;
 }
-PT_HD bool tri_test(f3 o, f3 d, float t_max, f3 p0, f3 p1, f3 p2, TriHit &h) { return tri_test_s(o, ray_shear(d), t_max, p0, p1, p2, h); }
+template <bool COLD_INLINE = true>
+PT_HD bool tri_test(f3 o, f3 d, float t_max, f3 p0, f3 p1, f3 p2, TriHit &h, bool *cold = nullptr) { return tri_test_s<COLD_INLINE>(o, ray_shear(d), t_max, p0, p1, p2, h, cold); }
 
 PT_HD bool tri_dpduv(f3 p0, f3 p1, f3 p2, f2 uv0, f2 uv1, f2 uv2, f3 &dpdu, f3 &dpdv) {
     f2 duv02 = mk2(uv0.x - uv2.x, uv0.y - uv2.y), duv12 = mk2(uv1.x - uv2.x, uv1.y - uv2.y);
diff --git a/pathtracer-rs_amd/csrc/ptrs_hip.hip b/pathtracer-rs_amd/csrc/ptrs_hip.hip
--- a/pathtracer-rs_amd/csrc/ptrs_hip.hip
+++ b/pathtracer-rs_amd/csrc/ptrs_hip.hip
@@ -50,6 +50,7 @@
     int tail_paths = 0;
     int workspace_pct = 40;
     int aov_fused_film = 1;
+    int shade_cold = 1;
     int denoise_lds = -1;
 };
 Options g_opt;
@@ -58,7 +59,7 @@
 struct OptionDesc { const char *name; int Options::*field; int lo, hi; };
 const OptionDesc k_options[] = {
     {"lanes", &Options::lanes, 0, 8}, {"refill", &Options::refill, -1, 64}, {"refill_connect", &Options::refill_connect, -1, 64}, {"stack_lds", &Options::stack_lds, 8, 16},
-    {"grid_mult", &Options::grid_mult, 0, 64}, {"persist", &Options::persist, 0, 1}, {"whole_rounds", &Options::whole_rounds, 0, 1}, {"grid_pct", &Options::grid_pct, 0, 100}, {"node_form", &Options::node_form, 0, 2}, {"node_order", &Options::node_order, 0, 1}, {"vote", &Options::vote, -1, 2}, {"shade_lds", &Options::shade_lds, 0, 1}, {"fused_epilogue", &Options::fused_epilogue, 0, 1}, {"fused_resolve", &Options::fused_resolve, 0, 1}, {"workspace_pct", &Options::workspace_pct, 1, 90}, {"peer_copy", &Options::peer_copy, 0, 1}, {"env_presample", &Options::env_presample, 0, 1}, {"deal", &Options::deal, 0, 1}, {"tail", &Options::tail, 0, 1}, {"tail_at", &Options::tail_at, -1, 64}, {"tail_paths", &Options::tail_paths, 0, 1 << 20}, {"aov_fused_film", &Options::aov_fused_film, 0, 1}, {"denoise_lds", &Options::denoise_lds, -1, 1},
+    {"grid_mult", &Options::grid_mult, 0, 64}, {"persist", &Options::persist, 0, 1}, {"whole_rounds", &Options::whole_rounds, 0, 1}, {"grid_pct", &Options::grid_pct, 0, 100}, {"node_form", &Options::node_form, 0, 2}, {"node_order", &Options::node_order, 0, 1}, {"vote", &Options::vote, -1, 2}, {"shade_lds", &Options::shade_lds, 0, 1}, {"fused_epilogue", &Options::fused_epilogue, 0, 1}, {"fused_resolve", &Options::fused_resolve, 0, 1}, {"workspace_pct", &Options::workspace_pct, 1, 90}, {"peer_copy", &Options::peer_copy, 0, 1}, {"env_presample", &Options::env_presample, 0, 1}, {"deal", &Options::deal, 0, 1}, {"tail", &Options::tail, 0, 1}, {"tail_at", &Options::tail_at, -1, 64}, {"tail_paths", &Options::tail_paths, 0, 1 << 20}, {"aov_fused_film", &Options::aov_fused_film, 0, 1}, {"denoise_lds", &Options::denoise_lds, -1, 1}, {"shade_cold", &Options::shade_cold, 0, 4},
 };
 
 #define HIPCHK(expr)                                                                                             \
@@ -655,12 +656,13 @@
 #endif
 enum : uint32_t { SH_SOB_WORDS = PTRS_SH_SOB_WORDS, SH_TRI_V4 = PTRS_SH_TRI_V4, SH_LIGHTS = 16, SH_LIGHT_V4 = sizeof(DLight) / 16, SH_TRI_REC_V4 = sizeof(DTriShade) / 16 };
 static_assert(sizeof(DLight) % 16 == 0 && sizeof(DTriShade) % 16 == 0, "records are staged as 16-byte vectors");
-struct ShadeLdsCfg { uint32_t sob_lo, sob_n, sob_nib, tri_lds, n_lights_lds, marg_li, pre_li; };
+struct ShadeLdsCfg { uint32_t sob_lo, sob_n, sob_nib, tri_lds, n_lights_lds, marg_li, pre_li, cold_mode; };
 enum : uint32_t { SH_MARG_N = 1024, SH_MARG_WORDS = 3 * SH_MARG_N + 8 };
 typedef __attribute__((address_space(3))) const uint32_t lds_u32;
 PT_HD uint32_t sob_stride(uint32_t nib) { return nib * 16u + 4u; }
-template <bool ENVPRE = false>
+template <bool ENVPRE = false, bool HOT = false>
 struct ShadeCtxLds {
+    static constexpr bool cold_inline = !HOT;
     static constexpr bool inf_fallback = !ENVPRE;
     lds_u32 *sob; lds_v4 *tris, *lights; ShadeLdsCfg cfg; InfMarginal marg;
     __device__ inline const InfMarginal *inf_marginal(uint32_t li) const { return li == cfg.marg_li ? &marg : nullptr; }
@@ -682,16 +684,41 @@
 #pragma unroll
         for (uint32_t k = 0; k < SH_LIGHT_V4; ++k) o[k] = ld(q + k);
     }
-    template <int N> __device__ inline void sobol(const DSampler &S, uint64_t index, const uint32_t (&dim)[N], uint32_t scramble, float (&out)[N]) const {
+    template <int N> __device__ inline void sobol(const DSampler &S, uint64_t index, const uint32_t (&dim)[N], uint32_t scramble, float (&out)[N], bool &cold) const {
         const uint32_t lo = (uint32_t)index, hi = (uint32_t)(index >> 32);
         bool in = cfg.sob_nib >= 13u || (hi == 0u && cfg.sob_nib >= 8u);
 #pragma unroll
         for (int k = 0; k < N; ++k) in = in && dim[k] - cfg.sob_lo < cfg.sob_n;
-        if (!in) { sobol_batch<N>(S, index, dim, scramble, out); return; }
+        if (!HOT && !in) { sobol_batch<N>(S, index, dim, scramble, out); return; }
         uint32_t v[N];
         bool run = cfg.sob_nib == 8u;
 #pragma unroll
         for (int k = 1; k < N; ++k) run = run && dim[k] == dim[0] + (uint32_t)k;
+        if constexpr (HOT) {
+            constexpr uint32_t ST = 8u * 16u + 4u;
+            const uint32_t gap = N > 2 ? dim[N > 2 ? 2 : 0] - dim[0] - 2u : 0u;
+            bool ok = in && cfg.sob_nib == 8u && gap <= 1u && (N < 2 || dim[N > 1 ? 1 : 0] == dim[0] + 1u);
+#pragma unroll
+            for (int k = 3; k < N; ++k) ok = ok && dim[k] == dim[0] + (uint32_t)k + gap;
+            if (!ok) {
+                cold = true;
+#pragma unroll
+                for (int k = 0; k < N; ++k) out[k] = 0.0f;
+                return;
+            }
+            lds_u32 *t = sob + (dim[0] - cfg.sob_lo) * ST;
+            lds_u32 *a[8] = {t + (lo & 15u), t + 16u + ((lo >> 4) & 15u), t + 32u + ((lo >> 8) & 15u), t + 48u + ((lo >> 12) & 15u), t + 64u + ((lo >> 16) & 15u),
+                             t + 80u + ((lo >> 20) & 15u), t + 96u + ((lo >> 24) & 15u), t + 112u + (lo >> 28)};
+#pragma unroll
+            for (int k = 0; k < N; ++k) {
+                v[k] = scramble;
+#pragma unroll
+                for (int j = 0; j < 8; ++j) v[k] ^= (k < 2 ? a[j] : a[j] + gap * ST)[k * ST];
+            }
+#pragma unroll
+            for (int k = 0; k < N; ++k) out[k] = min_nz(PT_ONE_MINUS_EPS, (float)v[k] * 0x1p-32f);
+            return;
+        }
         if (run) {
             constexpr uint32_t ST = 8u * 16u + 4u;
             lds_u32 *t = sob + (dim[0] - cfg.sob_lo) * ST;
@@ -723,8 +750,8 @@
 };
 
 template <int FEAT, bool ENVPRE> struct ShadeLdsSizes { enum : uint32_t { NPF = (FEAT & FEAT_INFINITE) ? 7u : 5u , MARG = ((FEAT & FEAT_INFINITE) && !ENVPRE) ? 1u : 0u  }; };
-template <int FEAT, bool ENVPRE>
-__device__ inline ShadeCtxLds<ENVPRE> stage_shade_tables(const DSampler &S, const DScene &sc, const ShadeLdsCfg &cfg, uint32_t *lds_sob, v4 *lds_tri, v4 *lds_light, float *lds_marg) {
+template <int FEAT, bool ENVPRE, bool HOT = false>
+__device__ inline ShadeCtxLds<ENVPRE, HOT> stage_shade_tables(const DSampler &S, const DScene &sc, const ShadeLdsCfg &cfg, uint32_t *lds_sob, v4 *lds_tri, v4 *lds_light, float *lds_marg) {
     constexpr bool MARG = ShadeLdsSizes<FEAT, ENVPRE>::MARG != 0;
     {
         const uint32_t stride = sob_stride(cfg.sob_nib), nw = cfg.sob_nib * 16u;
@@ -740,15 +767,86 @@
             for (uint32_t i = threadIdx.x; i < gv + 1u; i += BLOCK) lds_marg[2u * SH_MARG_N + 1u + i] = sc.distdata[Le.mguide_off + i];
         }
     }
-    ShadeCtxLds<ENVPRE> X; X.sob = (lds_u32 *)lds_sob; X.tris = (lds_v4 *)lds_tri; X.lights = (lds_v4 *)lds_light; X.cfg = cfg;
+    ShadeCtxLds<ENVPRE, HOT> X; X.sob = (lds_u32 *)lds_sob; X.tris = (lds_v4 *)lds_tri; X.lights = (lds_v4 *)lds_light; X.cfg = cfg;
     if (!MARG) X.cfg.marg_li = 0xffffffffu;
     X.marg.func = lds_marg; X.marg.cdf = lds_marg + (MARG ? SH_MARG_N : 0); X.marg.guide = lds_marg + (MARG ? 2 * SH_MARG_N + 1 : 0);
     return X;
 }
 
+enum { SHADE_GENERIC = 0, SHADE_HOT = 1, SHADE_REPLAY = 2 };
 template <int MAT, int FEAT, bool ENVPRE>
+__device__ inline void shade_segment_hot(const DParams &R, const DSampler &S, const DCamera &C, const DScene &sc, const DPaths &P, const DQueues &Q, uint32_t it, uint32_t seg_cap, uint32_t Gn, uint32_t s_,
+                                         const ShadeCtxLds<ENVPRE, true> &X, v4 *lds_pf) {
+    const uint32_t s = rfl(s_);
+    static_assert(!(FEAT & (FEAT_IMAGE | FEAT_INFINITE)), "the hot role is instantiated for scenes without image textures and environment lights");
+    const ShadeLdsCfg &cfg = X.cfg;
+    const uint32_t wv = rfl(threadIdx.x >> 6), lane = threadIdx.x & 63u, par = it & 1u;
+    auto dma = [&](const MatEntry &m) {
+        typedef __attribute__((address_space(1))) const void gptr; typedef __attribute__((address_space(3))) void lptr;
+        __builtin_amdgcn_global_load_lds((gptr *)&pslot(P.ray_d[par], m.e), (lptr *)(lds_pf + (1u * 4u + wv) * 64u), 16, 0, 0);
+        __builtin_amdgcn_global_load_lds((gptr *)&pslot(P.beta[par], m.e), (lptr *)(lds_pf + (2u * 4u + wv) * 64u), 16, 0, 0);
+        __builtin_amdgcn_global_load_lds((gptr *)&pslot(P.st, m.pid), (lptr *)(lds_pf + (3u * 4u + wv) * 64u), 16, 0, 0);
+        __builtin_amdgcn_global_load_lds((gptr *)&pslot(P.hit, m.e), (lptr *)(lds_pf + (4u * 4u + wv) * 64u), 16, 0, 0);
+    };
+    const uint32_t seg0 = s * seg_cap;
+    const MatEntry *__restrict__ queue = Q.mat[MAT] + seg0;
+    const uint32_t n = rfl(*seg_count(Q, it, Q_MAT0 + MAT, Gn, s));
+    if (n == 0) return;
+    const uint32_t next_base = rfl(*seg_count(Q, it + 1u, Q_EXT, Gn, s)), nee_base = rfl(*seg_count(Q, it, Q_NEE, Gn, s));
+    const uint32_t e_next0 = seg0 + next_base, f0 = seg0 + nee_base;
+    uint32_t c_next = 0, c_nee = 0, c_shadow = 0, c_mis = 0, c_replay = 0;
+    MatEntry m, m1; m.e = m.pid = m1.e = m1.pid = 0;
+    if (lane < n) { m = pslot(queue, lane); dma(m); }
+    if (lane + 64u < n) m1 = pslot(queue, lane + 64u);
+    __builtin_amdgcn_s_waitcnt(0x0F70);
+    for (uint32_t i0 = 0; i0 < n; i0 += 64u) {
+        const bool active = i0 + lane < n;
+        PathIn in;
+        {
+            lds_v4 *q = (lds_v4 *)lds_pf + threadIdx.x;
+            in.ro = mkv4(splat3(0.0f), 0.0f);
+            in.rd = X.ld(q + BLOCK); in.beta = X.ld(q + 2 * BLOCK);
+            const v4 a = X.ld(q + 3 * BLOCK), c = X.ld(q + 4 * BLOCK);
+            in.st.x = f2u(a.x); in.st.y = f2u(a.y); in.st.z = f2u(a.z); in.st.w = f2u(a.w);
+            in.hit.x = f2u(c.x); in.hit.y = f2u(c.y); in.hit.z = f2u(c.z); in.hit.w = f2u(c.w);
+            in.pre0 = in.pre1 = mkv4(splat3(0.0f), 0.0f);
+        }
+        __builtin_amdgcn_s_waitcnt(0xC07F);
+        if (i0 + 64u + lane < n) dma(m1);
+        MatEntry m2; m2.e = m2.pid = 0;
+        if (i0 + 128u + lane < n) m2 = pslot(queue + i0, lane + 128u);
+        const ShadeResult r = shade_item<MAT, FEAT>(R, S, C, sc, P, m.pid, in, X);
+        const bool cold = active && (r.cold || r.err_dim || cfg.cold_mode == 2u || (cfg.cold_mode == 3u && (((m.pid * 0x9E3779B1u) >> 16) & 1u)));
+        const bool live = active && !cold, next = live && r.next, nee = live && r.nee, shadow = live && r.shadow, mis = live && r.mis;
+        const uint32_t e_next = e_next0 + wave_push(c_next, next), f = f0 + wave_push(c_nee, nee), q = wave_push(c_replay, cold);
+        X.before_stores();
+        if (shadow) { pstore(P.sh_o, f, r.sh_o); pstore(P.sh_d, f, r.sh_d); }
+        if (mis) { pstore(P.mis_o, f, r.mis_o); pstore(P.mis_d, f, r.mis_d); pstore(P.nee0, f, r.nee0); pstore(P.nee1, f, r.nee1); pstore(P.nee2, f, r.nee2); }
+        else if (nee) pstore(P.pre_z, f, r.pre_z);
+        if (next) { pstore(P.ray_o[par ^ 1u], e_next, r.ro); pstore(P.ray_d[par ^ 1u], e_next, r.rd); pstore(P.beta[par ^ 1u], e_next, r.beta); pslot(Q.ext[par ^ 1u], e_next) = m.pid; }
+        if (nee) pslot(Q.nee, f) = r.nee_entry(m.pid);
+        c_shadow += (uint32_t)__popcll(__ballot(shadow));
+        c_mis += (uint32_t)__popcll(__ballot(mis));
+        if (cold) pslot(Q.replay + seg0, q) = m;
+        m = m1; m1 = m2;
+    }
+    uint32_t s2 = s;
+    asm volatile("" : "+s"(s2));
+    if (lane == 0) {
+        *seg_count(Q, it + 1u, Q_EXT, Gn, s2) = next_base + c_next;
+        if (c_next) Q.alive[it + 1u] = 1u;
+        *seg_count(Q, it, Q_NEE, Gn, s2) = nee_base + c_nee;
+        *seg_count(Q, it, Q_SHADOW, Gn, s2) += c_shadow;
+        *seg_count(Q, it, Q_MIS, Gn, s2) += c_mis;
+        if (c_replay) { *seg_count(Q, it, Q_REPLAY, Gn, s2) = c_replay; Q.replay_any[it] = 1u; }
+    }
+}
+
+
+template <int MAT, int FEAT, bool ENVPRE, int ROLE = SHADE_GENERIC>
 __device__ inline void shade_segment(const DParams &R, const DSampler &S, const DCamera &C, const DScene &sc, const DPaths &P, const DQueues &Q, uint32_t it, uint32_t seg_cap, uint32_t Gn, uint32_t s,
-                                     const ShadeCtxLds<ENVPRE> &X, v4 *lds_pf, bool &err_dim PT_STAMP_PARAMS) {
+                                     const ShadeCtxLds<ENVPRE, ROLE == SHADE_HOT> &X, v4 *lds_pf, bool &err_dim PT_STAMP_PARAMS) {
+    if constexpr (ROLE == SHADE_HOT) { shade_segment_hot<MAT, FEAT, ENVPRE>(R, S, C, sc, P, Q, it, seg_cap, Gn, s, X, lds_pf); return; }
     const ShadeLdsCfg &cfg = X.cfg;
     const uint32_t wv = threadIdx.x >> 6, lane = threadIdx.x & 63u, par = it & 1u;
     auto dma = [&](const MatEntry &m) {
@@ -763,8 +861,8 @@
             __builtin_amdgcn_global_load_lds((gptr *)&pslot(P.pre1, m.e), (lptr *)(lds_pf + (6u * 4u + wv) * 64u), 16, 0, 0);
         }
     };
-    const MatEntry *__restrict__ queue = Q.mat[MAT] + (size_t)s * seg_cap;
-    const uint32_t n = rfl(*seg_count(Q, it, Q_MAT0 + MAT, Gn, s));
+    const MatEntry *__restrict__ queue = (ROLE == SHADE_REPLAY ? Q.replay : Q.mat[MAT]) + (size_t)s * seg_cap;
+    const uint32_t n = rfl(*seg_count(Q, it, ROLE == SHADE_REPLAY ? (int)Q_REPLAY : Q_MAT0 + MAT, Gn, s));
     if (n == 0) return;
     const uint32_t next_base = rfl(*seg_count(Q, it + 1u, Q_EXT, Gn, s)), nee_base = rfl(*seg_count(Q, it, Q_NEE, Gn, s));
     const uint32_t e_next0 = s * seg_cap + next_base, f0 = s * seg_cap + nee_base;
@@ -818,8 +916,8 @@
     }
 }
 
-template <int MAT, int FEAT, bool ENVPRE>
-__global__ __launch_bounds__(BLOCK, (ShadeWaves<MAT, FEAT>::N)) void k_shade(DParams R, DSampler S, DCamera C, DScene sc, DPaths P, DQueues Q, uint32_t it, uint32_t seg_cap, ShadeLdsCfg cfg, uint32_t Gn, uint32_t *ticket) {
+template <int MAT, int FEAT, bool ENVPRE, int ROLE>
+__device__ __forceinline__ void shade_kernel(const DParams &R, const DSampler &S, const DCamera &C, const DScene &sc, const DPaths &P, const DQueues &Q, uint32_t it, uint32_t seg_cap, const ShadeLdsCfg &cfg, uint32_t Gn, uint32_t *ticket) {
     __shared__ v4 lds_pf[ShadeLdsSizes<FEAT, ENVPRE>::NPF * BLOCK];
     __shared__ uint32_t lds_sob[SH_SOB_WORDS];
     __shared__ v4 lds_tri[SH_TRI_V4];
@@ -828,13 +926,15 @@
     static_assert(2u * lds_alloc((uint32_t)(sizeof(lds_pf) + sizeof(lds_sob) + sizeof(lds_tri) + sizeof(lds_light) + sizeof(lds_marg))) <= (uint32_t)PTRS_LDS_PER_CU, "two shade workgroups per CU");
     bool err_dim = false;
     if (round_is_dead(Q, it)) return;
-    const ShadeCtxLds<ENVPRE> X = stage_shade_tables<FEAT, ENVPRE>(S, sc, cfg, lds_sob, lds_tri, lds_light, lds_marg);
+    if (ROLE == SHADE_REPLAY && rfl(Q.replay_any[it]) == 0u) return;
+    if (ROLE == SHADE_HOT) for (uint32_t i = threadIdx.x; i < ShadeLdsSizes<FEAT, ENVPRE>::NPF * BLOCK; i += BLOCK) lds_pf[i] = mkv4(splat3(0.0f), 0.0f);
+    const ShadeCtxLds<ENVPRE, ROLE == SHADE_HOT> X = stage_shade_tables<FEAT, ENVPRE, ROLE == SHADE_HOT>(S, sc, cfg, lds_sob, lds_tri, lds_light, lds_marg);
     __syncthreads();
 #ifdef PTRS_STAMPS
     unsigned long long stamp_acc[12] = {0, 0, 0, 0, 0, 0, 0, 0, 0, 0, 0, 0}, stamp_last = __builtin_amdgcn_s_memtime();
-    for (uint32_t s = seg_next(ticket, Gn); s < Gn; s = seg_next(ticket, Gn)) shade_segment<MAT, FEAT, ENVPRE>(R, S, C, sc, P, Q, it, seg_cap, Gn, s, X, lds_pf, err_dim, stamp_acc, stamp_last);
+    for (uint32_t s = seg_next(ticket, Gn); s < Gn; s = seg_next(ticket, Gn)) shade_segment<MAT, FEAT, ENVPRE, ROLE>(R, S, C, sc, P, Q, it, seg_cap, Gn, s, X, lds_pf, err_dim, stamp_acc, stamp_last);
 #else
-    for (uint32_t s = seg_next(ticket, Gn); s < Gn; s = seg_next(ticket, Gn)) shade_segment<MAT, FEAT, ENVPRE>(R, S, C, sc, P, Q, it, seg_cap, Gn, s, X, lds_pf, err_dim);
+    for (uint32_t s = seg_next(ticket, Gn); s < Gn; s = seg_next(ticket, Gn)) shade_segment<MAT, FEAT, ENVPRE, ROLE>(R, S, C, sc, P, Q, it, seg_cap, Gn, s, X, lds_pf, err_dim);
 #endif
     if (err_dim) atomicOr(&Q.stats[CNT_ERR], (unsigned long long)PTRS_ERRFLAG_SOBOL_DIM);
 #ifdef PTRS_STAMPS
@@ -842,6 +942,14 @@
     if ((threadIdx.x & 63u) == 0) for (int k = 0; k < 12; ++k) atomicAdd(&Q.stats[CNT_STAMP0 + k], stamp_acc[k]);
 #endif
 }
+#define PTRS_SHADE_ARGS DParams R, DSampler S, DCamera C, DScene sc, DPaths P, DQueues Q, uint32_t it, uint32_t seg_cap, ShadeLdsCfg cfg, uint32_t Gn, uint32_t *ticket
+template <int MAT, int FEAT, bool ENVPRE>
+__global__ __launch_bounds__(BLOCK, (ShadeWaves<MAT, FEAT>::N)) void k_shade(PTRS_SHADE_ARGS) { shade_kernel<MAT, FEAT, ENVPRE, SHADE_GENERIC>(R, S, C, sc, P, Q, it, seg_cap, cfg, Gn, ticket); }
+template <int MAT, int FEAT, bool ENVPRE>
+__global__ __launch_bounds__(BLOCK, (ShadeWaves<MAT, FEAT>::N)) void k_shade_hot(PTRS_SHADE_ARGS) { shade_kernel<MAT, FEAT, ENVPRE, SHADE_HOT>(R, S, C, sc, P, Q, it, seg_cap, cfg, Gn, ticket); }
+template <int MAT, int FEAT, bool ENVPRE>
+__global__ __launch_bounds__(BLOCK, (ShadeWaves<MAT, FEAT>::N)) void k_shade_replay(PTRS_SHADE_ARGS) { shade_kernel<MAT, FEAT, ENVPRE, SHADE_REPLAY>(R, S, C, sc, P, Q, it, seg_cap, cfg, Gn, ticket); }
+#undef PTRS_SHADE_ARGS
 
 constexpr bool tail_votes_connect(int geom) { return geom == 0; }
 template <int MAT, int FEAT, int GEOM, bool OVF, int DEPTH = 8>
@@ -923,14 +1031,15 @@
                 const uint64_t index = (uint64_t)stv.x | ((uint64_t)stv.y << 32);
                 const uint32_t dc[1] = {V.nee[4]};
                 float uc[1];
-                X.sobol<1>(S, index, dc, stv.w, uc);
+                bool cold_unused = false;
+                X.sobol<1>(S, index, dc, stv.w, uc, cold_unused);
                 const float fl = floor_(uc[0] * (float)sc.n_lights);
                 uint32_t li = fl > 0.0f ? (uint32_t)fl : 0u;
                 if (li > sc.n_lights - 1u) li = sc.n_lights - 1u;
                 if (li != env_li) continue;
                 const uint32_t dn[2] = {V.nee[0], V.nee[1]};
                 float u[2];
-                X.sobol<2>(S, index, dn, stv.w, u);
+                X.sobol<2>(S, index, dn, stv.w, u, cold_unused);
                 f3 wi, rgb; float pdf;
                 const bool ok = inf_light_sample(sc, Le, mk2(u[0], u[1]), wi, pdf, rgb, &marg);
                 pslot(P.pre0, me.e) = mkv4(wi, pdf);
@@ -1251,7 +1360,7 @@
     std::map<const void *, int> occupancy;
     uint32_t stack_lds = 16;
     std::vector<double> alive_frac;
-    DevBuf ws[MAX_LANES][32];
+    DevBuf ws[MAX_LANES][34];
     DevBuf counts[MAX_LANES], totals[MAX_LANES], tickets[MAX_LANES];
     DevBuf stats, table, film_tmp, samples_tmp, strat1, strat2, row_cost;
     DevBuf half_tmp, cv_tiles, cv_summary;
@@ -1292,7 +1401,7 @@
 #define PTRS_TAIL_O(M, F, G) PTRS_K(k_tail<M, F, G, true>), PTRS_K(k_tail<M, F, G, false>)
 [[maybe_unused]] const void *const k_code_object_order[] = {
     PTRS_K(k_epilogue<FEAT_FULL>), PTRS_K(k_epilogue<FEAT_IMG_ENV>), PTRS_K(k_epilogue<FEAT_SIMPLE>), PTRS_CONNECT_ALL(FEAT_FULL), PTRS_CONNECT_ALL(FEAT_IMG_ENV), PTRS_CONNECT_ALL(FEAT_SIMPLE),
-    PTRS_SHADE_ALL(FEAT_SIMPLE, false), PTRS_SHADE_ALL(FEAT_IMG, false), PTRS_SHADE_ALL(FEAT_IMG_ENV, true), PTRS_SHADE_ALL(FEAT_IMG_ENV, false), PTRS_SHADE_ALL(FEAT_FULL, true), PTRS_SHADE_ALL(FEAT_FULL, false),
+    PTRS_SHADE_ALL(FEAT_SIMPLE, false), PTRS_K(k_shade_hot<PTRS_MAT_MATTE, FEAT_SIMPLE, false>), PTRS_K(k_shade_replay<PTRS_MAT_MATTE, FEAT_SIMPLE, false>), PTRS_SHADE_ALL(FEAT_IMG, false), PTRS_SHADE_ALL(FEAT_IMG_ENV, true), PTRS_SHADE_ALL(FEAT_IMG_ENV, false), PTRS_SHADE_ALL(FEAT_FULL, true), PTRS_SHADE_ALL(FEAT_FULL, false),
     PTRS_K(k_env_presample<FEAT_IMG_ENV>), PTRS_K(k_env_presample<FEAT_FULL>), PTRS_K(k_tail<PTRS_MAT_MATTE, FEAT_SIMPLE, LDS9_V4, false, 9>), PTRS_TAIL_O(PTRS_MAT_MATTE, FEAT_SIMPLE, 640), PTRS_TAIL_O(PTRS_MAT_MATTE, FEAT_SIMPLE, 1536),
     PTRS_TAIL_O(PTRS_MAT_MATTE, FEAT_SIMPLE, 0), PTRS_TAIL_O(PTRS_MAT_DISNEY, FEAT_IMG, 0), PTRS_K(k_aov<FEAT_SIMPLE>), PTRS_K(k_aov<FEAT_FULL>),
     PTRS_K(k_dn_iter_lds<1>), PTRS_K(k_dn_iter_lds<2>), PTRS_K(k_dn_iter_lds<4>), PTRS_K(k_dn_iter_lds<8>), PTRS_K(k_dn_iter_lds<16>),
@@ -1353,7 +1462,7 @@
         for (auto &l : ps->ws) for (auto &b : l) held += b.bytes;
         held += ps->stack_spill.bytes;
         uint32_t nk = 0; for (int k = 0; k < 7; ++k) nk += kinds[k] ? 1u : 0u;
-        const double per_path = (17.0 + (ps->H.inf_lights.empty() ? 0.0 : 2.0)) * 16.0 + 8.0 + 4.0 + 3.0 * 4.0 + nk * 8.0;
+        const double per_path = (17.0 + (ps->H.inf_lights.empty() ? 0.0 : 2.0)) * 16.0 + 8.0 + 4.0 + 3.0 * 4.0 + nk * 8.0 + (kinds[0] ? 8.0 : 0.0);
         const double budget = (double)(fr + held) * (double)opt.workspace_pct / 100.0 / (double)std::max(1, share);
         const double cap = budget / (per_path * (double)lanes_n);
         return cap < 65536.0 ? 65536ull : (uint64_t)cap;
@@ -1481,9 +1590,11 @@
                 Ql.mat[k] = nullptr;
                 if (kinds_mask & (1u << k)) { if ((rc = take(nq * sizeof(MatEntry), (void **)&Ql.mat[k], "queues")) != PTRS_OK) return rc; } else ++w;
             }
+            Ql.replay = nullptr;
+            if (shade_hot()) { if ((rc = take(nq * sizeof(MatEntry), (void **)&Ql.replay, "queues")) != PTRS_OK) return rc; } else ++w;
             if ((rc = ps->counts[l].ensure((size_t)rows * Q_STRIDE * (size_t)grid_max * 4)) != PTRS_OK || (rc = ps->totals[l].ensure((size_t)rows * Q_STRIDE * 4)) != PTRS_OK ||
-                (rc = ps->tickets[l].ensure(((size_t)rows * Q_STRIDE * TK_LAUNCH_WORDS + rows) * 4)) != PTRS_OK) { err = g_err; return rc; }
-            Ql.counts = (uint32_t *)ps->counts[l].p; Ql.stats = (unsigned long long *)ps->stats.p; Ql.tickets = (uint32_t *)ps->tickets[l].p; Ql.alive = Ql.tickets + (size_t)rows * Q_STRIDE * TK_LAUNCH_WORDS;
+                (rc = ps->tickets[l].ensure(((size_t)rows * Q_STRIDE * TK_LAUNCH_WORDS + 2u * rows) * 4)) != PTRS_OK) { err = g_err; return rc; }
+            Ql.counts = (uint32_t *)ps->counts[l].p; Ql.stats = (unsigned long long *)ps->stats.p; Ql.tickets = (uint32_t *)ps->tickets[l].p; Ql.alive = Ql.tickets + (size_t)rows * Q_STRIDE * TK_LAUNCH_WORDS; Ql.replay_any = Ql.alive + rows;
             lane_[l] = Lane{l == 0 ? stream : ps->lane_stream[l], DParams{}, Pl, Ql, 1u, 0u};
         }
         cur = 0; P = lane_[0].P; Q = lane_[0].Q;
@@ -1499,7 +1610,7 @@
         if (G < 1) G = 1;
         seg_cap = ((chunks + G - 1) / G) * 64u;
         (void)hipMemsetAsync(Q.counts, 0, (size_t)rows * Q_STRIDE * G * 4, stream);
-        (void)hipMemsetAsync(Q.tickets, 0, ((size_t)rows * Q_STRIDE * TK_LAUNCH_WORDS + rows) * 4, stream);
+        (void)hipMemsetAsync(Q.tickets, 0, ((size_t)rows * Q_STRIDE * TK_LAUNCH_WORDS + 2u * rows) * 4, stream);
     }
     void generate() { t0(T_AUX); hipLaunchKernelGGL(k_generate, dim3((G + WAVES - 1) / WAVES), dim3(BLOCK), 0, stream, R, S, C, P, Q, seg_cap, G, (uint32_t)deal_by_region()); t1(); }
     int deal_by_region() const { return opt.deal; }
@@ -1558,6 +1669,7 @@
         c.n_lights_lds = opt.shade_lds ? std::min<uint32_t>(sc.n_lights, SH_LIGHTS) : 0u;
         if (!opt.shade_lds) c.sob_n = 0;
         c.pre_li = presample_li();
+        c.cold_mode = 0;
         c.marg_li = 0xffffffffu;
         if (opt.shade_lds && !ps->H.inf_lights.empty()) {
             const DLight &Le = ps->H.lights[ps->H.inf_lights[0]];
@@ -1634,9 +1746,29 @@
         for (uint32_t i = 0; i < n_rows; ++i) f[i] = (double)counts[(size_t)i * Q_STRIDE + Q_EXT] / (double)n_paths;
         ps->alive_frac.swap(f);
     }
+    bool shade_hot() const {
+#ifdef PTRS_STAMPS
+        return false;
+#else
+        return opt.shade_cold != 0 && opt.shade_lds && feat == FEAT_SIMPLE && ps->H.kinds_present[PTRS_MAT_MATTE];
+#endif
+    }
     void shade(uint32_t it, int kind) {
         t0(T_SHADE);
         if (kind > 5) kind = 5;
+        if (kind == PTRS_MAT_MATTE && shade_hot() && !R.row_cost && Q.replay) {
+            const ShadeFn hot = k_shade_hot<PTRS_MAT_MATTE, FEAT_SIMPLE, false>, replay = k_shade_replay<PTRS_MAT_MATTE, FEAT_SIMPLE, false>;
+            ShadeLdsCfg c = shade_cfg(it);
+            c.cold_mode = (uint32_t)opt.shade_cold;
+            ShadeLdsCfg ch = c;
+            if (opt.shade_cold == 4) ch.sob_n = 0;
+            const uint32_t g_replay = persistent_grid(replay, T_SHADE), g_hot = persistent_grid(hot, T_SHADE);
+            hipLaunchKernelGGL(hot, dim3(g_hot), dim3(BLOCK), 0, stream, R, S, C, sc, P, Q, it, seg_cap, ch, G, ticket(it, TK_SHADE0 + kind));
+            hipLaunchKernelGGL(replay, dim3(g_replay), dim3(BLOCK), 0, stream, R, S, C, sc, P, Q, it, seg_cap, c, G, ticket(it, TK_REPLAY));
+            ++launches;
+            t1();
+            return;
+        }
         const ShadeFn fn = shade_fn(kind);
         hipLaunchKernelGGL(fn, dim3(persistent_grid(fn, T_SHADE)), dim3(BLOCK), 0, stream, R, S, C, sc, P, Q, it, seg_cap, shade_cfg(it), G, ticket(it, TK_SHADE0 + kind));
         t1();
```

Measured after the change: 13280, median of 6. Within noise of the previous version (+0.6%).
